# OATML-Markslab/ProteinGym

Measured on AMD Instinct MI355X. Metric: mutants scored/sec (ESM-1v 650M masked-marginal), higher is better.
Workload: dtype f16x3 (fp32 operands split into 2 fp16 planes, 3 fp16 MFMAs per product, fp32 accumulate)

## Files before the change

### include/pgmi.h

```cpp
#ifndef PGMI_H
#define PGMI_H

#include <stddef.h>
#include <stdint.h>

#ifdef __cplusplus
extern "C" {
#endif

#define PGMI_ABI_VERSION 6

#define PGMI_OK 0
#define PGMI_EINVAL (-1)
#define PGMI_ENOMEM (-2)
#define PGMI_EHIP (-3)
#define PGMI_ENODEV (-4)
#define PGMI_EPARSE (-5)
#define PGMI_EOVERFLOW (-6)

#define PGMI_ARCH_ESM1B 1
#define PGMI_ARCH_ESM2 2
#define PGMI_ARCH_TRANCEPTION 3
#define PGMI_ARCH_MSA 4
#define PGMI_ARCH_PROGEN2 5
// ... 43 lines not shown
typedef struct pgmi_pppl pgmi_pppl;

int pgmi_abi_version(void);
int pgmi_device_count(void);
const char* pgmi_last_error(void);

int64_t pgmi_weight_count(const pgmi_config* cfg);

int pgmi_model_create(const pgmi_config* cfg, const float* weights, int64_t n_weights,
                      int device, pgmi_model** out);
void pgmi_model_destroy(pgmi_model* m);
int pgmi_model_device(const pgmi_model* m);

int pgmi_token_logprobs(pgmi_model* m, const int32_t* tokens, int B, int T, float* out);

int pgmi_masked_logprobs(pgmi_model* m, const int32_t* tokens, const int32_t* mask_pos,
                         int B, int T, float* out);

int pgmi_assay_create(pgmi_model* m, const int32_t* wt_tokens, int n_tok,
                      const int32_t* positions, int P, int window,
                      const int32_t* sub_pos, const int32_t* sub_wt, const int32_t* sub_mt,
                      const int64_t* mut_off, int64_t n_mut, pgmi_assay** out);
int pgmi_assay_run(pgmi_model* m, pgmi_assay* a, double* scores_host, float* table_host,
                   double* scores_dev);
void pgmi_assay_destroy(pgmi_assay* a);

int pgmi_pppl_create(pgmi_model* m, const uint8_t* tokens, const int64_t* seq_off, int64_t n_seq, pgmi_pppl** out);
int pgmi_pppl_run(pgmi_model* m, pgmi_pppl* lib, int64_t first, int64_t count, double* scores_host,
                  float* terms_host, double* scores_dev);
int64_t pgmi_pppl_rows(const pgmi_pppl* lib, int64_t first, int64_t count);
int pgmi_pppl_stats(const pgmi_pppl* lib, int64_t* rows, int64_t* batches, int64_t* tokens, int64_t* padded_tokens);
void pgmi_pppl_destroy(pgmi_pppl* lib);

int pgmi_parse_mutants(const char* text, const int64_t* str_off, int64_t n_mut,
                       const char* sequence, int seq_len, int offset_idx,
                       int32_t* sub_pos, int32_t* sub_wt, int32_t* sub_mt,
                       int64_t* mut_off, int64_t* n_sub);

int pgmi_score_mutants(const float* table, int n_rows, int vocab, const int32_t* sub_pos, const int32_t* sub_wt,
                       const int32_t* sub_mt, const int64_t* mut_off, int64_t n_mut, double* scores);

void pgmi_optimal_window(int position, int seq_len_with_special, int model_window,
                         int* start, int* end);

#define PGMI_K_EMBED 0
#define PGMI_K_LAYERNORM 1
#define PGMI_K_GEMM_QKV 2
#define PGMI_K_ATTENTION 3
#define PGMI_K_GEMM_OUT 4
#define PGMI_K_GEMM_FC1 5
#define PGMI_K_GEMM_FC2 6
#define PGMI_K_HEAD 7
#define PGMI_K_SCORE 8
#define PGMI_K_KEPT_ROWS 9
#define PGMI_K_MOE_ROUTE 10
#define PGMI_K_GEOM 11
#define PGMI_K_CROSS_ATTENTION 12
#define PGMI_K_COUNT 13
int pgmi_profile_enable(pgmi_model* m, int on);
int pgmi_profile_get(pgmi_model* m, int kernel_class, double* ms, int64_t* launches,
                     double* flops, double* bytes);
int pgmi_profile_reset(pgmi_model* m);
int pgmi_synchronize(pgmi_model* m);

int pgmi_set_option(const char* name, int64_t value);

int pgmi_op_layernorm(int device, const float* x, const float* w, const float* b,
                      int rows, int D, float eps, float* y);
int pgmi_op_gemm(int device, int precision, const float* A, const float* W, const float* bias,
                 const float* residual, int M, int N, int K, int epilogue ,
                 float* C);
int pgmi_op_qkln_prep(int device, const float* qkv, const float* q_w, const float* k_w, int B, int T, int H, int iters, float* qk,
                      float* v, double* ms);
int pgmi_op_attention(int device, int precision, const float* qkv, const int32_t* kv_len,
                      int B, int T, int H, int rotary, float* ctx);
int pgmi_op_causal_attention(int device, int lanes, const float* X, const float* W, const float* bias, int K, const float* qkv,
                             const float* conv, const float* rot_cos, const float* rot_sin, const float* slopes, int B, int T,
                             int heads, float* ctx);
int pgmi_op_prefix_attention(int device, const float* qkv, const int32_t* seg_off, int n_seg, const float* prefix_kv, int P, int heads,
                             int split, float* ctx);
int pgmi_op_cross_attention(int device, const float* q, const int32_t* seg_off, int n_seg, const float* mem_kv, int S, int heads,
                            int split, float* ctx);
int pgmi_op_packed_chunks(const int32_t* lens, int B, int drop_last, int same_length, int max_rows, int32_t* out_b1, int32_t* out_n);
int pgmi_op_rmsnorm(int device, const float* x, const float* w, int rows, int D, float eps, float* y);
int pgmi_op_geom_attention(int device, const float* proj, const float* rot, const float* trans, const int32_t* frame_mask,
                           int per_row_frames, const float* w_rot, const float* w_dist, int B, int S, int H, float* out);
int pgmi_op_geom_key_tile(int S);
int pgmi_op_moe(int device, const float* h, const float* gate, const float* w1, const float* w3, const float* w2, int M, int D, int F,
                int E, int top_k, int gated, float* out, int32_t* ids, float* weights);
int pgmi_op_tied_row_attention(int device, const float* qkv, int R, int C, int H, int splits, float* ctx, float* probs);
int pgmi_op_tied_row_splits(int R, int C, int H);
int pgmi_op_column_attention(int device, const float* X, const float* W, const float* bias, int K, int R, int C, int H, float* ctx);
int pgmi_op_vocab_logsoftmax(int device, const float* h, const float* E, const float* bias, int rows, int D, int V, float* out,
                             int32_t* nonfinite);
int pgmi_op_wide_logsoftmax(int device, const float* logits, int ldl, int rows, int V, const int32_t* tgt, float* out, int32_t* nonfinite);
int pgmi_op_group_logsoftmax(int device, const float* h, const float* E, const float* bias, int rows, int D, int V, int first, int groups,
                             int width, float* full, float* group, int32_t* nonfinite);
int pgmi_op_seq_loglik(int device, const float* lp, const int32_t* tokens, int B, int T, int V, const int32_t* lens, const int32_t* seq_off,
                       const int32_t* seq_p, const int32_t* seq_root, int n_lp_rows, const float* prior, int n_prior_rows,
                       const int32_t* a0, const int32_t* row0, const int32_t* n, const int32_t* flip, float alpha, const float* eve,
                       float beta, int eve_fallback, float* out);

int pgmi_tr_token_logprobs(pgmi_model* m, const int32_t* tokens, int B, int T, float* out);
int pgmi_tr_sequence_loglik(pgmi_model* m, const int32_t* tokens, const int32_t* lens, int B, int T,
                            const float* log_prior, int P, const int32_t* prior_a0, const int32_t* prior_row0,
                            const int32_t* prior_n, const int32_t* prior_flip, float alpha, float* out);
int pgmi_tr_sequence_loglik_shared(pgmi_model* m, const int32_t* tokens, const int32_t* ref, int B, int T,
                                   const float* log_prior, int P, const int32_t* prior_a0, const int32_t* prior_row0,
                                   const int32_t* prior_n, const int32_t* prior_flip, float alpha, float* out,
                                   float* token_logprobs, int64_t* rows_forwarded);
int pgmi_tr_sequence_loglik_eve(pgmi_model* m, const int32_t* tokens, const int32_t* lens, int B, int T,
                                const float* log_prior, int P, const int32_t* prior_a0, const int32_t* prior_row0,
                                const int32_t* prior_n, const int32_t* prior_flip, float alpha, const float* eve_log_prior, float beta,
                                int eve_fallback, float* out);
int pgmi_tr_sequence_loglik_shared_eve(pgmi_model* m, const int32_t* tokens, const int32_t* ref, int B, int T,
                                       const float* log_prior, int P, const int32_t* prior_a0, const int32_t* prior_row0,
                                       const int32_t* prior_n, const int32_t* prior_flip, float alpha, const float* eve_log_prior,
                                       float beta, int eve_fallback, float* out, float* token_logprobs, int64_t* rows_forwarded);

int pgmi_bench_gemm(int device, int precision, int M, int N, int K, int epilogue, int split_out,
                    int variant, int iters, double* ms_per_launch);
int pgmi_bench_gemm_ab(int device, int precision, int M, int N, int K, int epilogue, int split_out,
                       const int* variants, int n_variants, int rounds, int iters, double* ms_out);

int pgmi_pg2_model_create(const pgmi_config* cfg, int rotary_dim, const float* weights, int64_t n_weights, int device, pgmi_model** out);
int pgmi_pg2_token_logprobs(pgmi_model* m, const int32_t* tokens, int B, int T, float* out);
int pgmi_pg2_sequence_loglik(pgmi_model* m, const int32_t* tokens, int B, int L, float* out, int32_t* n_kept);

int64_t pgmi_gpt_weight_count(const pgmi_config* cfg, int pos_kind);
int pgmi_gpt_model_create(const pgmi_config* cfg, int pos_kind, const float* weights, int64_t n_weights, int device, pgmi_model** out);
int pgmi_gpt_token_logprobs(pgmi_model* m, const int32_t* tokens, int B, int T, float* out);
int pgmi_gpt_sequence_loglik(pgmi_model* m, const int32_t* tokens, const int32_t* lens, int B, int T, double* sum, int32_t* n_targets);

typedef struct pgmi_pg3_params {
    int32_t kv_heads;
    int32_t n_experts;
    int32_t top_k;
    int32_t gated;
    float rope_theta;
    float clip_qkv;
} pgmi_pg3_params;
int64_t pgmi_pg3_weight_count(const pgmi_config* cfg, const pgmi_pg3_params* params);
int pgmi_pg3_model_create(const pgmi_config* cfg, const pgmi_pg3_params* params, const float* weights, int64_t n_weights, int device,
                          pgmi_model** out);
int pgmi_pg3_token_logprobs(pgmi_model* m, const int32_t* tokens, int B, int T, float* out);
int pgmi_pg3_sequence_loglik(pgmi_model* m, const int32_t* tokens, const int32_t* lens, int B, int T, double* sum, int32_t* n_targets);
int pgmi_pg3_routing(pgmi_model* m, int layer, int rows, int32_t* ids, float* weights);


int64_t pgmi_esm3_weight_count(const pgmi_config* cfg, int v_heads);
int pgmi_esm3_model_create(const pgmi_config* cfg, int v_heads, const float* weights, int64_t n_weights, int device, pgmi_model** out);
int pgmi_esm3_set_structure(pgmi_model* m, const int32_t* structure_tokens, const int32_t* plddt, const float* rot, const float* trans,
                            const int32_t* frame_mask, int T);

int pgmi_saprot_model_create(const pgmi_config* cfg, int mask_id, const float* weights, int64_t n_weights, int device, pgmi_model** out);
int pgmi_saprot_token_logprobs(pgmi_model* m, const int32_t* tokens, int B, int T, float* out);
int pgmi_saprot_group_logprobs(pgmi_model* m, const int32_t* wt_tokens, int T, const int32_t* set_off, const int32_t* set_pos,
                               int n_sets, float* out);

#define PGMI_POET_TOK_GAP 20
#define PGMI_POET_TOK_START 21
#define PGMI_POET_TOK_STOP 22
#define PGMI_POET_TOK_MASK 23
int64_t pgmi_poet_weight_count(const pgmi_config* cfg, int final_norm);
int pgmi_poet_model_create(const pgmi_config* cfg, int final_norm, const float* weights, int64_t n_weights, int device, pgmi_model** out);
int pgmi_poet_set_prompt(pgmi_model* m, const int32_t* tokens, const int32_t* seg_len, int n_seg);
// ... 128 lines not shown
```

### proteingym_amd/_lib.py

```python
from __future__ import annotations

import ctypes as C
import os

import numpy as np

HERE = os.path.dirname(os.path.abspath(__file__))
LIB_PATH = os.path.join(HERE, "libpgmi.so")

ABI_VERSION = 6
ARCH_ESM1B, ARCH_ESM2, ARCH_TRANCEPTION = 1, 2, 3
ARCH_PROGEN2 = 5
ARCH_GPT = 6
ARCH_ESMC = 7
ARCH_SAPROT = 8
ARCH_POET = 9
ARCH_PROGEN3 = 10
ARCH_ESM3 = 11
ARCH_ESMIF1 = 12
GPT_POS_ROTARY, GPT_POS_LEARNED = 0, 1
PREC_FP32, PREC_BF16, PREC_F16X3 = 0, 1, 2
PRECISIONS = {"fp32": PREC_FP32, "bf16": PREC_BF16, "f16x3": PREC_F16X3}
K_NAMES = ["embed", "layernorm", "gemm_qkv", "attention", "gemm_out", "gemm_fc1", "gemm_fc2",
           "head", "score", "kept_rows", "moe_route", "geom", "cross_attention"]


EINVAL, ENOMEM, EHIP, ENODEV, EPARSE, EOVERFLOW = -1, -2, -3, -4, -5, -6


class PgmiError(RuntimeError):

    def __init__(self, message, code=None):
        super().__init__(message)
        self.code = code


class Config(C.Structure):
    _fields_ = [(n, C.c_int32) for n in (
        "abi_version", "arch", "layers", "embed_dim", "heads", "ffn_dim", "vocab",
        "max_positions", "token_dropout", "emb_layer_norm_before", "precision", "max_rows")] + [("ln_eps", C.c_float)]


class Pg3Params(C.Structure):
    _fields_ = [(n, C.c_int32) for n in ("kv_heads", "n_experts", "top_k", "gated")] + [("rope_theta", C.c_float), ("clip_qkv", C.c_float)]


_lib = None

_i32p = C.POINTER(C.c_int32)
_i64p = C.POINTER(C.c_int64)
_f32p = C.POINTER(C.c_float)
_f64p = C.POINTER(C.c_double)
_u8p = C.POINTER(C.c_uint8)

SIGNATURES = [
    ("pgmi_abi_version", C.c_int, []),
    ("pgmi_device_count", C.c_int, []),
    ("pgmi_last_error", C.c_char_p, []),
    ("pgmi_weight_count", C.c_int64, [C.POINTER(Config)]),
    ("pgmi_model_create", C.c_int, [C.POINTER(Config), _f32p, C.c_int64, C.c_int, C.POINTER(C.c_void_p)]),
    ("pgmi_model_destroy", None, [C.c_void_p]),
    ("pgmi_model_device", C.c_int, [C.c_void_p]),
    ("pgmi_token_logprobs", C.c_int, [C.c_void_p, _i32p, C.c_int, C.c_int, _f32p]),
    ("pgmi_masked_logprobs", C.c_int, [C.c_void_p, _i32p, _i32p, C.c_int, C.c_int, _f32p]),
    ("pgmi_assay_create", C.c_int, [C.c_void_p, _i32p, C.c_int, _i32p, C.c_int, C.c_int,
                                    _i32p, _i32p, _i32p, _i64p, C.c_int64, C.POINTER(C.c_void_p)]),
    ("pgmi_assay_run", C.c_int, [C.c_void_p, C.c_void_p, _f64p, _f32p, C.c_void_p]),
    ("pgmi_assay_destroy", None, [C.c_void_p]),
    ("pgmi_pppl_create", C.c_int, [C.c_void_p, C.POINTER(C.c_uint8), _i64p, C.c_int64, C.POINTER(C.c_void_p)]),
    ("pgmi_pppl_run", C.c_int, [C.c_void_p, C.c_void_p, C.c_int64, C.c_int64, _f64p, _f32p, C.c_void_p]),
    ("pgmi_pppl_rows", C.c_int64, [C.c_void_p, C.c_int64, C.c_int64]),
    ("pgmi_pppl_stats", C.c_int, [C.c_void_p, _i64p, _i64p, _i64p, _i64p]),
    ("pgmi_pppl_destroy", None, [C.c_void_p]),
    ("pgmi_parse_mutants", C.c_int, [C.c_char_p, _i64p, C.c_int64, C.c_char_p, C.c_int, C.c_int,
                                     _i32p, _i32p, _i32p, _i64p, _i64p]),
    ("pgmi_score_mutants", C.c_int, [_f32p, C.c_int, C.c_int, _i32p, _i32p, _i32p, _i64p, C.c_int64, _f64p]),
    ("pgmi_optimal_window", None, [C.c_int, C.c_int, C.c_int, _i32p, _i32p]),
    ("pgmi_profile_enable", C.c_int, [C.c_void_p, C.c_int]),
    ("pgmi_profile_get", C.c_int, [C.c_void_p, C.c_int, _f64p, _i64p, _f64p, _f64p]),
    ("pgmi_profile_reset", C.c_int, [C.c_void_p]),
    ("pgmi_synchronize", C.c_int, [C.c_void_p]),
    ("pgmi_set_option", C.c_int, [C.c_char_p, C.c_int64]),
    ("pgmi_op_layernorm", C.c_int, [C.c_int, _f32p, _f32p, _f32p, C.c_int, C.c_int, C.c_float, _f32p]),
    ("pgmi_op_gemm", C.c_int, [C.c_int, C.c_int, _f32p, _f32p, _f32p, _f32p, C.c_int, C.c_int, C.c_int, C.c_int, _f32p]),
    ("pgmi_tr_token_logprobs", C.c_int, [C.c_void_p, _i32p, C.c_int, C.c_int, _f32p]),
    ("pgmi_tr_sequence_loglik", C.c_int, [C.c_void_p, _i32p, _i32p, C.c_int, C.c_int, _f32p, C.c_int,
                                          _i32p, _i32p, _i32p, _i32p, C.c_float, _f32p]),
    ("pgmi_tr_sequence_loglik_shared", C.c_int, [C.c_void_p, _i32p, _i32p, C.c_int, C.c_int, _f32p, C.c_int,
                                                 _i32p, _i32p, _i32p, _i32p, C.c_float, _f32p, _f32p, _i64p]),
    ("pgmi_tr_sequence_loglik_eve", C.c_int, [C.c_void_p, _i32p, _i32p, C.c_int, C.c_int, _f32p, C.c_int,
                                              _i32p, _i32p, _i32p, _i32p, C.c_float, _f32p, C.c_float, C.c_int, _f32p]),
    ("pgmi_tr_sequence_loglik_shared_eve", C.c_int, [C.c_void_p, _i32p, _i32p, C.c_int, C.c_int, _f32p, C.c_int,
                                                     _i32p, _i32p, _i32p, _i32p, C.c_float, _f32p, C.c_float, C.c_int, _f32p, _f32p,
                                                     _i64p]),
    ("pgmi_pg2_model_create", C.c_int, [C.POINTER(Config), C.c_int, _f32p, C.c_int64, C.c_int, C.POINTER(C.c_void_p)]),
    ("pgmi_pg2_token_logprobs", C.c_int, [C.c_void_p, _i32p, C.c_int, C.c_int, _f32p]),
    ("pgmi_pg2_sequence_loglik", C.c_int, [C.c_void_p, _i32p, C.c_int, C.c_int, _f32p, _i32p]),
    ("pgmi_gpt_weight_count", C.c_int64, [C.POINTER(Config), C.c_int]),
    ("pgmi_gpt_model_create", C.c_int, [C.POINTER(Config), C.c_int, _f32p, C.c_int64, C.c_int, C.POINTER(C.c_void_p)]),
    ("pgmi_gpt_token_logprobs", C.c_int, [C.c_void_p, _i32p, C.c_int, C.c_int, _f32p]),
    ("pgmi_gpt_sequence_loglik", C.c_int, [C.c_void_p, _i32p, _i32p, C.c_int, C.c_int, _f64p, _i32p]),
    ("pgmi_saprot_model_create", C.c_int, [C.POINTER(Config), C.c_int, _f32p, C.c_int64, C.c_int, C.POINTER(C.c_void_p)]),
    ("pgmi_saprot_token_logprobs", C.c_int, [C.c_void_p, _i32p, C.c_int, C.c_int, _f32p]),
    ("pgmi_saprot_group_logprobs", C.c_int, [C.c_void_p, _i32p, C.c_int, _i32p, _i32p, C.c_int, _f32p]),
    ("pgmi_poet_weight_count", C.c_int64, [C.POINTER(Config), C.c_int]),
    ("pgmi_poet_model_create", C.c_int, [C.POINTER(Config), C.c_int, _f32p, C.c_int64, C.c_int, C.POINTER(C.c_void_p)]),
    ("pgmi_poet_set_prompt", C.c_int, [C.c_void_p, _i32p, _i32p, C.c_int]),
    ("pgmi_poet_prompt_logprobs", C.c_int, [C.c_void_p, _f32p]),
    ("pgmi_poet_token_logprobs", C.c_int, [C.c_void_p, _i32p, _i32p, C.c_int, C.c_int, _f32p]),
    ("pgmi_poet_sequence_loglik", C.c_int, [C.c_void_p, _i32p, _i32p, C.c_int, C.c_int, _f64p]),
    ("pgmi_esmif1_weight_count", C.c_int64, [C.POINTER(Config), C.c_int]),
    ("pgmi_esmif1_model_create", C.c_int, [C.POINTER(Config), C.c_int, _f32p, C.c_int64, C.c_int, C.POINTER(C.c_void_p)]),
    ("pgmi_esmif1_set_memory", C.c_int, [C.c_void_p, _f32p, C.c_int]),
    ("pgmi_esmif1_token_logprobs", C.c_int, [C.c_void_p, _i32p, _i32p, C.c_int, C.c_int, _f32p]),
    ("pgmi_esmif1_sequence_loglik", C.c_int, [C.c_void_p, _i32p, _i32p, C.c_int, C.c_int, _f64p]),
    ("pgmi_pg3_weight_count", C.c_int64, [C.POINTER(Config), C.POINTER(Pg3Params)]),
    ("pgmi_pg3_model_create", C.c_int, [C.POINTER(Config), C.POINTER(Pg3Params), _f32p, C.c_int64, C.c_int, C.POINTER(C.c_void_p)]),
    ("pgmi_pg3_token_logprobs", C.c_int, [C.c_void_p, _i32p, C.c_int, C.c_int, _f32p]),
    ("pgmi_pg3_sequence_loglik", C.c_int, [C.c_void_p, _i32p, _i32p, C.c_int, C.c_int, _f64p, _i32p]),
    ("pgmi_pg3_routing", C.c_int, [C.c_void_p, C.c_int, C.c_int, _i32p, _f32p]),
    ("pgmi_esm3_weight_count", C.c_int64, [C.POINTER(Config), C.c_int]),
    ("pgmi_esm3_model_create", C.c_int, [C.POINTER(Config), C.c_int, _f32p, C.c_int64, C.c_int, C.POINTER(C.c_void_p)]),
    ("pgmi_esm3_set_structure", C.c_int, [C.c_void_p, _i32p, _i32p, _f32p, _f32p, _i32p, C.c_int]),
    ("pgmi_eve_weight_count", C.c_int64, [C.c_void_p]),
    ("pgmi_eve_create", C.c_int, [C.c_void_p, _f32p, C.c_int64, C.c_int, C.POINTER(C.c_void_p)]),
    ("pgmi_eve_destroy", None, [C.c_void_p]),
    ("pgmi_eve_profile_model", C.c_void_p, [C.c_void_p]),
    ("pgmi_eve_encode", C.c_int, [C.c_void_p, _u8p, C.c_int, _f32p, _f32p]),
    ("pgmi_eve_elbo", C.c_int, [C.c_void_p, _u8p, C.c_int, C.c_int64, C.c_uint64, C.c_int, C.c_void_p, _f32p, _f32p, _f32p]),
    ("pgmi_eve_noise_fill", C.c_int, [C.c_void_p, C.c_uint64, C.c_int, C.c_int64, C.c_int, C.c_void_p]),
    ("pgmi_eve_evol_indices", C.c_int, [C.c_void_p, _u8p, C.c_int, C.c_int, C.c_uint64, _f64p, _f64p]),
    ("pgmi_eve_log_prior", C.c_int, [C.c_void_p, _u8p, C.c_int, C.c_uint64, C.c_void_p, _f64p, _f64p]),
    ("pgmi_mpnn_weight_count", C.c_int64, [C.c_void_p]),
    ("pgmi_mpnn_create", C.c_int, [C.c_void_p, _f32p, C.c_int64, C.c_int, C.POINTER(C.c_void_p)]),
    ("pgmi_mpnn_destroy", None, [C.c_void_p]),
    ("pgmi_mpnn_profile_model", C.c_void_p, [C.c_void_p]),
    ("pgmi_mpnn_set_structure", C.c_int, [C.c_void_p, _f32p, _f32p, _i32p, _i32p, C.c_int]),
    ("pgmi_mpnn_graph", C.c_int, [C.c_void_p, _i32p, _f32p]),
    ("pgmi_mpnn_encoder", C.c_int, [C.c_void_p, _f32p, _f32p]),
    ("pgmi_mpnn_log_probs", C.c_int, [C.c_void_p, _u8p, _i32p, C.c_int, _f32p]),
    ("pgmi_mpnn_scores", C.c_int, [C.c_void_p, _u8p, _i32p, C.c_int, _f64p]),
    ("pgmi_s2f_weight_count", C.c_int64, [C.c_void_p]),
    ("pgmi_s2f_create", C.c_int, [C.c_void_p, _f32p, C.c_int64, C.c_void_p, C.c_int, C.POINTER(C.c_void_p)]),
    ("pgmi_s2f_destroy", None, [C.c_void_p]),
    ("pgmi_s2f_profile_model", C.c_void_p, [C.c_void_p]),
    ("pgmi_s2f_set_structure", C.c_int, [C.c_void_p, _f32p, _f32p, C.c_int]),
    ("pgmi_s2f_graph", C.c_int, [C.c_void_p, _i32p, _i32p, _i32p, _f32p, _f32p]),
    ("pgmi_s2f_gvp_forward", C.c_int, [C.c_void_p, _f32p, _f32p, C.c_int, _f32p, _f32p, _f32p]),
    ("pgmi_s2f_set_logprobs", C.c_int, [C.c_void_p, _i32p, C.c_int, _i32p, _i32p, _i32p, C.c_int, _f32p, _f32p]),
    ("pgmi_unirep_weight_count", C.c_int64, [C.c_void_p]),
    ("pgmi_unirep_model_create", C.c_int, [C.c_void_p, _f32p, C.c_int64, C.c_int, C.POINTER(C.c_void_p)]),
    ("pgmi_unirep_destroy", None, [C.c_void_p]),
    ("pgmi_unirep_profile_model", C.c_void_p, [C.c_void_p]),
    ("pgmi_unirep_set_target", C.c_int, [C.c_void_p, _i32p, C.c_int]),
    ("pgmi_unirep_sequence_nll", C.c_int, [C.c_void_p, _i32p, _i64p, C.c_int64, C.c_int, _f64p, _i64p]),
    ("pgmi_unirep_token_logprobs", C.c_int, [C.c_void_p, _i32p, C.c_int, _f32p]),
    ("pgmi_op_mlstm_step", C.c_int, [C.c_void_p, _f32p, _f32p, _i32p, C.c_int, _f32p, _f32p, _f32p]),
    ("pgmi_bench_gemm", C.c_int, [C.c_int] * 9 + [_f64p]),
    ("pgmi_bench_gemm_ab", C.c_int, [C.c_int] * 7 + [_i32p, C.c_int, C.c_int, C.c_int, _f64p]),
    ("pgmi_op_attention", C.c_int, [C.c_int, C.c_int, _f32p, _i32p, C.c_int, C.c_int, C.c_int, C.c_int, _f32p]),
    ("pgmi_op_qkln_prep", C.c_int, [C.c_int, _f32p, _f32p, _f32p, C.c_int, C.c_int, C.c_int, C.c_int, _f32p, _f32p, _f64p]),
    ("pgmi_op_causal_attention", C.c_int, [C.c_int, C.c_int, _f32p, _f32p, _f32p, C.c_int, _f32p, _f32p, _f32p, _f32p, _f32p,
                                           C.c_int, C.c_int, C.c_int, _f32p]),
    ("pgmi_op_prefix_attention", C.c_int, [C.c_int, _f32p, _i32p, C.c_int, _f32p, C.c_int, C.c_int, C.c_int, _f32p]),
    ("pgmi_op_cross_attention", C.c_int, [C.c_int, _f32p, _i32p, C.c_int, _f32p, C.c_int, C.c_int, C.c_int, _f32p]),
    ("pgmi_op_packed_chunks", C.c_int, [_i32p, C.c_int, C.c_int, C.c_int, C.c_int, _i32p, _i32p]),
    ("pgmi_op_rmsnorm", C.c_int, [C.c_int, _f32p, _f32p, C.c_int, C.c_int, C.c_float, _f32p]),
    ("pgmi_op_geom_attention", C.c_int, [C.c_int, _f32p, _f32p, _f32p, _i32p, C.c_int, _f32p, _f32p, C.c_int, C.c_int, C.c_int, _f32p]),
    ("pgmi_op_geom_key_tile", C.c_int, [C.c_int]),
    ("pgmi_op_moe", C.c_int, [C.c_int, _f32p, _f32p, _f32p, _f32p, _f32p, C.c_int, C.c_int, C.c_int, C.c_int, C.c_int, C.c_int, _f32p,
                              _i32p, _f32p]),
    ("pgmi_op_tied_row_attention", C.c_int, [C.c_int, _f32p, C.c_int, C.c_int, C.c_int, C.c_int, _f32p, _f32p]),
    ("pgmi_op_tied_row_splits", C.c_int, [C.c_int, C.c_int, C.c_int]),
    ("pgmi_op_column_attention", C.c_int, [C.c_int, _f32p, _f32p, _f32p, C.c_int, C.c_int, C.c_int, C.c_int, _f32p]),
    ("pgmi_op_vocab_logsoftmax", C.c_int, [C.c_int, _f32p, _f32p, _f32p, C.c_int, C.c_int, C.c_int, _f32p, _i32p]),
    ("pgmi_op_wide_logsoftmax", C.c_int, [C.c_int, _f32p, C.c_int, C.c_int, C.c_int, _i32p, _f32p, _i32p]),
    ("pgmi_op_group_logsoftmax", C.c_int, [C.c_int, _f32p, _f32p, _f32p, C.c_int, C.c_int, C.c_int, C.c_int, C.c_int, C.c_int, _f32p,
                                           _f32p, _i32p]),
    ("pgmi_op_seq_loglik", C.c_int, [C.c_int, _f32p, _i32p, C.c_int, C.c_int, C.c_int, _i32p, _i32p, _i32p, _i32p, C.c_int, _f32p, C.c_int,
                                     _i32p, _i32p, _i32p, _i32p, C.c_float, _f32p, C.c_float, C.c_int, _f32p]),
    ("pgmi_msa_token_logprobs", C.c_int, [C.c_void_p, _i32p, C.c_int, C.c_int, _f32p]),
    ("pgmi_msa_masked_logprobs", C.c_int, [C.c_void_p, _i32p, C.c_int, C.c_int, C.c_int, _i32p, _i32p, C.c_int, _f32p]),
    ("pgmi_msa_cluster_counts", C.c_int, [C.c_int, C.POINTER(C.c_int8), C.c_int64, C.c_int64, C.c_int, C.c_double, _i32p, _f64p]),
    ("pgmi_msa_neighbor_counts", C.c_int, [C.c_int, C.POINTER(C.c_int8), C.c_int64, C.c_int64, C.c_int, C.c_double, _i32p, _f64p]),
]


def load():
    global _lib
    if _lib is not None:
        return _lib
    if not os.path.exists(LIB_PATH):
        raise PgmiError(f"{LIB_PATH} not found: run `python -m proteingym_amd.build_native` "
                        "(hipcc, gfx950).  There is no CPU fallback.")
    lib = C.CDLL(LIB_PATH)
    for name, res, args in SIGNATURES:
        fn = getattr(lib, name)
        fn.restype = res
        fn.argtypes = args
    if lib.pgmi_abi_version() != ABI_VERSION:
        raise PgmiError("libpgmi ABI version mismatch; rebuild")
    _lib = lib
    return lib


def check(rc: int):
    if rc != 0:
        raise PgmiError(f"libpgmi error {rc}: {load().pgmi_last_error().decode(errors='replace')}", code=int(rc))


def ptr(a: np.ndarray, ty):
    return a.ctypes.data_as(ty) if a is not None else None


def as_i32(a):
    return np.ascontiguousarray(a, dtype=np.int32)


def as_f32(a):
    return np.ascontiguousarray(a, dtype=np.float32)


class ModelHandle:
    CREATE = "pgmi_model_create"

    def __init__(self, cfg: dict, weights: np.ndarray, device: int = 0, max_rows: int = 0, arch_arg=None,
                 precision: int = PREC_F16X3, **fields):
        lib = load()
        self.cfg = dict(cfg)
        self.device = device
        c = Config(abi_version=ABI_VERSION, layers=cfg["layers"], embed_dim=cfg["embed_dim"], heads=cfg["heads"],
                   ffn_dim=cfg["ffn_dim"], precision=precision, max_rows=max_rows, **fields)
        w = as_f32(weights)
        n = self._weight_count(lib, c, arch_arg)
        if w.size != n:
            raise PgmiError(f"weight blob has {w.size} elements, config needs {n}")
        h = C.c_void_p()
        head = (C.byref(c),) if arch_arg is None else (C.byref(c), arch_arg)
        check(getattr(lib, self.CREATE)(*head, ptr(w, _f32p), w.size, device, C.byref(h)))
        self._h = h

    @staticmethod
    def _weight_count(lib, c, arch_arg):
        return lib.pgmi_weight_count(C.byref(c))

    def close(self):
        if getattr(self, "_h", None):
            load().pgmi_model_destroy(self._h)
            self._h = None
# ... 7 lines not shown
```

### proteingym_amd/csrc/api_esm.hip

```cpp
#include "model.h"

namespace pgmi {

int create_esm(pgmi_model* m, const pgmi_config* cfg, const float* w, int64_t n_weights) {
    const size_t D = cfg->embed_dim, F = cfg->ffn_dim, V = cfg->vocab, dh = m->dh, Da = m->Da;
    BlobCursor c(m, w, n_weights);
    c.upload(&m->embed_tokens, V * D);
    if (cfg->arch == PGMI_ARCH_ESM1B) c.upload(&m->embed_positions, (size_t)(cfg->max_positions + 2) * D);
    if (cfg->emb_layer_norm_before) {
        c.upload(&m->lnb_w, D);
        c.upload(&m->lnb_b, D);
    }
    auto slot = [&](size_t col) -> size_t { return rotate_half_slot(col, dh); };
    const float qscale = 1.0f / sqrtf((float)dh);
    m->layers.resize(cfg->layers);
    std::vector<float> wq(3 * Da * D, 0.0f), bq(3 * Da, 0.0f), wo_r(D * Da, 0.0f);
    for (int l = 0; l < cfg->layers; ++l) {
        Layer& L = m->layers[l];
        c.upload(&L.ln1_w, D);
        c.upload(&L.ln1_b, D);
        pack_qkv_slots(c.take(3 * (D * D + D)), D, Da, slot, qscale, wq.data(), bq.data());
        c.linear(&L.wqkv, &L.wqkv16, wq.data(), wq.size(), D);
        c.upload(&L.bqkv, bq.data(), bq.size());
        pack_out_cols(c.take(D * D), D, Da, slot, wo_r.data());
        c.linear(&L.wo, &L.wo16, wo_r.data(), wo_r.size(), Da);
        c.upload(&L.bo, D);
        c.upload(&L.ln2_w, D);
        c.upload(&L.ln2_b, D);
        c.linear(&L.w1, &L.w116, F * D, D);
        c.upload(&L.b1, F);
        c.linear(&L.w2, &L.w216, D * F, F);
        c.upload(&L.b2, D);
    }
    c.upload(&m->lna_w, D);
    c.upload(&m->lna_b, D);
    c.linear(&m->hd_w, &m->hd16, D * D, D);
    c.upload(&m->hd_b, D);
    c.upload(&m->hln_w, D);
    c.upload(&m->hln_b, D);
    c.upload(&m->head_b, V);
    m->head_w = m->embed_tokens;
    return c.finish();
}

int ensure_rotary(pgmi_model* m, int T) {
    if ((!esm2_rotary(m->cfg.arch) && !esmc_blocks(m->cfg.arch)) || T <= m->rot_len) return PGMI_OK;
    return upload_rotate_half(m, std::max(T, 1026));
}

int upload_rotate_half(pgmi_model* m, int n) {
    const int rh = m->rot_halves;
    float inv[64];
    const int half = m->dh / 2;
    for (int i = 0; i < half; ++i) inv[i] = 1.0f / powf(10000.0f, (float)(2 * i) / (float)m->dh);
    return upload_rotary(m, n, rh, [&](int t, int g, int i) {
        const int j = (rh == 1) ? i : 32 * g + i;
        return j < half ? (float)t * inv[j] : 0.0f;
    });
}

int run_encoder(pgmi_model* m, int B, int T, const int32_t* keep, int n_keep, bool* compacted) {
    const pgmi_config& c = m->cfg;
    const int M = B * T, D = c.embed_dim, F = c.ffn_dim, N1 = m->fc1_cols, H = c.heads, Da = m->Da;
    hipStream_t s = m->stream;
    if (c.arch == PGMI_ARCH_ESM1B && T > c.max_positions) {
        set_error("Sequence length %d above maximum sequence length of %d", T, c.max_positions);
        return PGMI_EINVAL;
    }
    int rc = ensure_rotary(m, T);
    if (!rc) rc = reset_pad_keys(m, B, T);
    if (rc) return rc;
    {
        ProfScope p(m, PGMI_K_EMBED, 0, (double)M * D * 4);
        launch_seq_stats(m->tokens, B, T, m->embed_gather ? 0 : c.token_dropout, m->denom, m->pos_idx, m->kv_len, s, m->mask_id);
        if (c.arch == PGMI_ARCH_ESM3) { if ((rc = esm3_embed(m, B, T))) return rc; }
        else if (m->embed_gather) launch_gather_rows(m->embed_tokens, m->tokens, M, D, m->x, s);
        else launch_embed(m->tokens, m->denom, m->pos_idx, m->embed_tokens, m->embed_positions, c.token_dropout, M, T, D, m->x, s, m->mask_id);
        if (m->lnb_w) {
            launch_layernorm(m->x, m->lnb_w, m->lnb_b, M, D, 1e-5f, m->x, s);
            launch_zero_pad_rows(m->tokens, M, D, m->x, s);
        }
    }
    const double ln_bytes = 2.0 * M * D * 4;
    const int prec = c.precision;
    const int mode16 = (prec == PGMI_PREC_F16X3) ? 1 : 2;
    for (int l = 0; l < c.layers; ++l) {
        const Layer& L = m->layers[l];
        { ProfScope p(m, PGMI_K_LAYERNORM, 0, ln_bytes);
          if (prec == PGMI_PREC_FP32) launch_layernorm(m->x, L.ln1_w, L.ln1_b, M, D, 1e-5f, m->h, s);
          else launch_layernorm16(m->x, L.ln1_w, L.ln1_b, M, D, 1e-5f, m->h16, mode16, s); }
        const bool fused_qkv = prec != PGMI_PREC_FP32 && !L.q_ln;
        { ProfScope p(m, PGMI_K_GEMM_QKV, 2.0 * M * 3 * D * D, 0);
          if (fused_qkv) {
              GemmLaunch g = qkv_launch(m, L.wqkv16, L.bqkv, M, Da, D, T, m->Hs);
              g.bf = prec == PGMI_PREC_BF16;
              g.qkv.cos_t = m->rot_cos; g.qkv.sin_t = m->rot_sin; g.qkv.rotary = esm2_rotary(c.arch); g.qkv.rot_halves = m->rot_halves;
              rc = launch_gemm16(g);
          } else
              rc = linear(m, m->h, m->h16, L.wqkv, L.wqkv16, L.bqkv, nullptr, m->qkv, nullptr, M, 3 * Da, D, EPI_NONE);
          if (rc) return rc; }
        { ProfScope p(m, PGMI_K_ATTENTION, 4.0 * M * T * D, L.q_ln ? (double)M * D * 20 : 0);
          if (L.q_ln && (rc = launch_qkln_prep(m->qkv, L.q_ln, L.k_ln, 1e-5f, m->rot_cos, m->rot_sin, B, T, H, m->qk16, m->qk16_plane,
                                               m->vt16, m->vt16_plane, s)))
              return rc;
          const bool v2 = prec != PGMI_PREC_FP32;
          if (esm2_rotary(c.arch) && !v2) launch_rotary(m->qkv, m->rot_cos, m->rot_sin, M, T, m->Hs, s, m->rot_halves);
          if (v2) {
              AttLaunch a;
              a.qk16 = m->qk16, a.qk_plane = m->qk16_plane, a.vt16 = m->vt16, a.vt_plane = m->vt16_plane;
              a.B = B, a.T = T, a.H = H, a.head_dim = m->rot_halves * kHeadDim;
              a.kv_len = m->kv_len;
              a.out = prec == PGMI_PREC_F16X3 ? ATT_OUT_SPLIT : ATT_OUT_BF16;
              a.ctx16 = m->h16;
              a.stream = s;
              rc = launch_attention_f16x3_v2(a);
          } else {
              rc = launch_attention_f32(m->qkv, m->kv_len, B, T, H, m->h, s, m->rot_halves * kHeadDim);
          }
          if (rc) return rc; }
        if (keep && m->keep_rows && l == c.layers - 1 && !L.g_norm_w) {
            const int R = n_keep;
            ProfScope p(m, PGMI_K_KEPT_ROWS, 2.0 * R * D * (Da + N1 + F), 0);
            launch_gather_rows(m->x, keep, R, D, m->qkv, s);
            if (prec == PGMI_PREC_FP32) launch_gather_rows(m->h, keep, R, Da, m->g, s);
            else
                launch_gather_rows(reinterpret_cast<const float*>(m->h16), keep, R, prec == PGMI_PREC_F16X3 ? Da : Da / 2,
                                   reinterpret_cast<float*>(m->g16), s);
            rc = linear(m, m->g, m->g16, L.wo, L.wo16, L.bo, m->qkv, m->x, nullptr, R, D, Da, EPI_NONE);
            if (rc) return rc;
            if (prec == PGMI_PREC_FP32) launch_layernorm(m->x, L.ln2_w, L.ln2_b, R, D, 1e-5f, m->h, s);
            else launch_layernorm16(m->x, L.ln2_w, L.ln2_b, R, D, 1e-5f, m->h16, mode16, s);
            rc = linear(m, m->h, m->h16, L.w1, L.w116, L.b1, nullptr,
                        prec == PGMI_PREC_FP32 ? m->g : nullptr, prec == PGMI_PREC_FP32 ? nullptr : m->g16,
                        R, N1, D, m->fc1_epi);
            if (rc) return rc;
            rc = linear(m, m->g, m->g16, L.w2, L.w216, L.b2, m->x, m->x, nullptr, R, D, F, EPI_NONE);
            if (rc) return rc;
            if (compacted) *compacted = true;
            break;
        }
        { ProfScope p(m, PGMI_K_GEMM_OUT, 2.0 * M * D * D, 0);
          rc = linear(m, m->h, m->h16, L.wo, L.wo16, L.bo, m->x, m->x, nullptr, M, D, Da, EPI_NONE);
          if (rc) return rc; }
        if (L.g_norm_w && m->e3_framed && (rc = geom_branch(m, L, B, T))) return rc;
        { ProfScope p(m, PGMI_K_LAYERNORM, 0, ln_bytes);
          if (prec == PGMI_PREC_FP32) launch_layernorm(m->x, L.ln2_w, L.ln2_b, M, D, 1e-5f, m->h, s);
          else launch_layernorm16(m->x, L.ln2_w, L.ln2_b, M, D, 1e-5f, m->h16, mode16, s); }
        { ProfScope p(m, PGMI_K_GEMM_FC1, 2.0 * M * N1 * D, 0);
          rc = linear(m, m->h, m->h16, L.w1, L.w116, L.b1, nullptr,
                      prec == PGMI_PREC_FP32 ? m->g : nullptr, prec == PGMI_PREC_FP32 ? nullptr : m->g16,
                      M, N1, D, m->fc1_epi);
          if (rc) return rc; }
        { ProfScope p(m, PGMI_K_GEMM_FC2, 2.0 * M * F * D, 0);
          rc = linear(m, m->g, m->g16, L.w2, L.w216, L.b2, m->x, m->x, nullptr, M, D, F, EPI_NONE);
          if (rc) return rc; }
    }
    PGMI_HIP(hipGetLastError());
    return PGMI_OK;
}

int run_head(pgmi_model* m, int R, const int32_t* row_idx) {
    const pgmi_config& c = m->cfg;
    ProfScope p(m, PGMI_K_HEAD, 2.0 * R * c.embed_dim * (c.embed_dim + c.vocab), 0);
    int rc = head_hidden(m, R, row_idx);
    if (rc) return rc;
    launch_vocab_logsoftmax(m->g, m->head_w, m->head_b, R, c.embed_dim, c.vocab, m->lp, m->nonfinite, m->stream);
    PGMI_HIP(hipGetLastError());
    return PGMI_OK;
}

int head_hidden(pgmi_model* m, int R, const int32_t* row_idx) {
    const pgmi_config& c = m->cfg;
    const int D = c.embed_dim;
    hipStream_t s = m->stream;
    const int prec = c.precision;
    const float* src = m->x;
    if (row_idx) {
        launch_gather_rows(m->x, row_idx, R, D, m->h, s);
        src = m->h;
    }
    if (prec == PGMI_PREC_FP32) launch_layernorm(src, m->lna_w, m->lna_b, R, D, 1e-5f, m->h, s);
    else launch_layernorm16(src, m->lna_w, m->lna_b, R, D, 1e-5f, m->h16, prec == PGMI_PREC_F16X3 ? 1 : 2, s);
    int rc = linear(m, m->h, m->h16, m->hd_w, m->hd16, m->hd_b, nullptr, m->g, nullptr, R, D, D, EPI_GELU);
    if (rc) return rc;
    launch_layernorm(m->g, m->hln_w, m->hln_b, R, D, 1e-5f, m->g, s);
    return PGMI_OK;
}


int run_rows(pgmi_model* m, int B, int T, int R, const int32_t* row_idx) {
    bool compacted = false;
    int rc = run_encoder(m, B, T, row_idx, R, &compacted);
    if (rc) return rc;
    return run_head(m, R, compacted ? nullptr : row_idx);
}

}

extern "C" {

int pgmi_token_logprobs(pgmi_model* m, const int32_t* tokens, int B, int T, float* out) {
    if (!m || !tokens || !out || B <= 0 || T <= 0) { set_error("bad argument"); return PGMI_EINVAL; }
    if (m->cfg.arch == PGMI_ARCH_SAPROT) { set_error("SaProt models are scored with pgmi_saprot_token_logprobs / pgmi_saprot_group_logprobs"); return PGMI_EINVAL; }
    if (T + 31 > m->max_rows) { set_error("T=%d exceeds workspace rows %d", T, m->max_rows); return PGMI_EINVAL; }
    int rc = check_tokens(tokens, B, T);
    if (rc) return rc;
    PGMI_HIP(hipSetDevice(m->device));
    const int V = m->cfg.vocab;
    rc = for_each_chunk(m, B, T, [&](int b0, int bc) {
        PGMI_HIP(hipMemcpyAsync(m->tokens, tokens + (size_t)b0 * T, (size_t)bc * T * 4, hipMemcpyHostToDevice, m->stream));
        int rc = run_rows(m, bc, T, bc * T, nullptr);
        if (rc) return rc;
        PGMI_HIP(hipMemcpyAsync(out + (size_t)b0 * T * V, m->lp, (size_t)bc * T * V * 4, hipMemcpyDeviceToHost, m->stream));
        return PGMI_OK;
    });
    return rc ? rc : check_nonfinite(m);
}

int pgmi_masked_logprobs(pgmi_model* m, const int32_t* tokens, const int32_t* mask_pos, int B, int T, float* out) {
    if (!m || !tokens || !mask_pos || !out || B <= 0 || T <= 0) { set_error("bad argument"); return PGMI_EINVAL; }
    if (m->cfg.arch == PGMI_ARCH_SAPROT) { set_error("SaProt models are scored with pgmi_saprot_token_logprobs / pgmi_saprot_group_logprobs"); return PGMI_EINVAL; }
    if (esmc_blocks(m->cfg.arch) && T + 31 > m->max_rows) { set_error("T=%d exceeds workspace rows %d", T, m->max_rows); return PGMI_EINVAL; }
    if (T > m->max_rows) { set_error("T=%d exceeds workspace rows %d", T, m->max_rows); return PGMI_EINVAL; }
    int rc = check_tokens(tokens, B, T);
    if (rc) return rc;
    for (int b = 0; b < B; ++b)
        if (mask_pos[b] < 0 || mask_pos[b] >= T) { set_error("mask_pos[%d]=%d out of range", b, mask_pos[b]); return PGMI_EINVAL; }
    PGMI_HIP(hipSetDevice(m->device));
    const int V = m->cfg.vocab;
    std::vector<int32_t> ridx;
    rc = for_each_chunk(m, B, T, [&](int b0, int bc) {
        ridx.resize(bc);
        for (int b = 0; b < bc; ++b) ridx[b] = b * T + mask_pos[b0 + b];
        PGMI_HIP(hipMemcpyAsync(m->tokens, tokens + (size_t)b0 * T, (size_t)bc * T * 4, hipMemcpyHostToDevice, m->stream));
        PGMI_HIP(hipMemcpyAsync(m->aux_i, mask_pos + b0, (size_t)bc * 4, hipMemcpyHostToDevice, m->stream));
        PGMI_HIP(hipMemcpyAsync(m->row_idx, ridx.data(), (size_t)bc * 4, hipMemcpyHostToDevice, m->stream));
        launch_apply_mask(m->tokens, m->aux_i, bc, T, m->stream);
        int rc = run_rows(m, bc, T, bc, m->row_idx);
        if (rc) return rc;
        PGMI_HIP(hipMemcpyAsync(out + (size_t)b0 * V, m->lp, (size_t)bc * V * 4, hipMemcpyDeviceToHost, m->stream));
        return PGMI_OK;
    });
    return rc ? rc : check_nonfinite(m);
}

int pgmi_assay_create(pgmi_model* m, const int32_t* wt_tokens, int n_tok, const int32_t* positions, int P,
                      int window, const int32_t* sub_pos, const int32_t* sub_wt, const int32_t* sub_mt,
                      const int64_t* mut_off, int64_t n_mut, pgmi_assay** out) {
    if (!out) { set_error("null out"); return PGMI_EINVAL; }
    *out = nullptr;
    if (!m || !wt_tokens || n_tok <= 0 || P < 0 || (P > 0 && !positions) || window <= 0 || n_mut < 0) { set_error("bad argument"); return PGMI_EINVAL; }
    if (esmc_blocks(m->cfg.arch)) { set_error("ESM C / ESM3 assays run through pgmi_masked_logprobs (their window rule is not pgmi_optimal_window)"); return PGMI_EINVAL; }
    if (m->cfg.arch == PGMI_ARCH_SAPROT) { set_error("SaProt assays run through pgmi_saprot_group_logprobs (position sets, no window)"); return PGMI_EINVAL; }
    for (int i = 0; i < n_tok; ++i)
        if (wt_tokens[i] < 0 || wt_tokens[i] >= PGMI_VOCAB || wt_tokens[i] == PGMI_TOK_PAD) { set_error("wt token %d invalid at %d", wt_tokens[i], i); return PGMI_EINVAL; }
    const int T = std::min(n_tok, window);
    if (T > m->max_rows) { set_error("T=%d exceeds workspace rows %d", T, m->max_rows); return PGMI_EINVAL; }
    std::vector<int32_t> ws(P), mr(P);
    for (int i = 0; i < P; ++i) {
        if (positions[i] < 0 || positions[i] >= n_tok) { set_error("position %d out of range", positions[i]); return PGMI_EINVAL; }
        int s, e;
        pgmi_optimal_window(positions[i], n_tok, window, &s, &e);
        if (e - s != T) { set_error("internal: window length %d != %d", e - s, T); return PGMI_EINVAL; }
        ws[i] = s;
        mr[i] = positions[i] - s;
    }
    const int64_t n_sub = n_mut ? mut_off[n_mut] : 0;
    for (int64_t k = 0; k < n_sub; ++k)
        if (sub_pos[k] < 0 || sub_pos[k] >= n_tok || sub_wt[k] < 0 || sub_wt[k] >= PGMI_VOCAB || sub_mt[k] < 0 || sub_mt[k] >= PGMI_VOCAB) {
            set_error("substitution %lld out of range", (long long)k);
            return PGMI_EINVAL;
        }
    PGMI_HIP(hipSetDevice(m->device));
    pgmi_assay* a = new pgmi_assay();
    a->m = m; a->n_tok = n_tok; a->P = P; a->T = T; a->n_mut = n_mut; a->n_sub = n_sub;
    int rc = dev_upload(a->allocs, &a->wt, wt_tokens, (size_t)n_tok);
    if (!rc) rc = dev_upload(a->allocs, &a->positions, positions, (size_t)P);
    if (!rc) rc = dev_upload(a->allocs, &a->win_start, ws.data(), (size_t)P);
    if (!rc) rc = dev_upload(a->allocs, &a->mask_rel, mr.data(), (size_t)P);
    if (!rc) rc = dev_upload(a->allocs, &a->sub_pos, sub_pos, (size_t)n_sub);
    if (!rc) rc = dev_upload(a->allocs, &a->sub_wt, sub_wt, (size_t)n_sub);
    if (!rc) rc = dev_upload(a->allocs, &a->sub_mt, sub_mt, (size_t)n_sub);
    if (!rc) rc = dev_upload(a->allocs, &a->mut_off, mut_off, (size_t)(n_mut + 1));
    if (!rc) rc = dev_alloc(a->allocs, &a->table, (size_t)n_tok * PGMI_VOCAB);
    if (!rc) rc = dev_alloc(a->allocs, &a->scores, (size_t)n_mut);
    if (rc) { pgmi_assay_destroy(a); return rc; }
    m->assays.push_back(a);
    *out = a;
    return PGMI_OK;
}

void pgmi_assay_destroy(pgmi_assay* a) {
    if (!a) return;
    if (a->m) {
        hipSetDevice(a->m->device);
        hipStreamSynchronize(a->m->stream);
        auto& v = a->m->assays;
        v.erase(std::remove(v.begin(), v.end(), a), v.end());
    }
    for (void* p : a->allocs) hipFree(p);
    delete a;
}

int pgmi_assay_run(pgmi_model* m, pgmi_assay* a, double* scores_host, float* table_host, double* scores_dev) {
    if (!m || !a || a->m != m) { set_error("bad model/assay handle (assay belongs to another or a destroyed model)"); return PGMI_EINVAL; }
    PGMI_HIP(hipSetDevice(m->device));
    hipStream_t s = m->stream;
    const int T = a->T, V = m->cfg.vocab;
    const int per = rows_per_chunk(m, T);
    launch_fill_f32(a->table, (int64_t)a->n_tok * V, NAN, s);
    for (int p0 = 0; p0 < a->P; p0 += per) {
        const int bc = std::min(per, a->P - p0);
        launch_make_masked_windows(a->wt, a->win_start + p0, a->mask_rel + p0, bc, T, m->tokens, s);
        launch_row_index(a->mask_rel + p0, bc, T, m->row_idx, s);
        int rc = run_rows(m, bc, T, bc, m->row_idx);
        if (rc) return rc;
        launch_scatter_rows(m->lp, a->positions + p0, bc, V, a->table, s);
    }
    {
        ProfScope p(m, PGMI_K_SCORE, 0, (double)a->n_sub * 20);
        launch_score_mutants(a->table, V, a->sub_pos, a->sub_wt, a->sub_mt, a->mut_off, a->n_mut, a->scores, s);
    }
    PGMI_HIP(hipGetLastError());
    if (scores_dev && a->n_mut) PGMI_HIP(hipMemcpyAsync(scores_dev, a->scores, (size_t)a->n_mut * 8, hipMemcpyDeviceToDevice, s));
    if (scores_host && a->n_mut) PGMI_HIP(hipMemcpyAsync(scores_host, a->scores, (size_t)a->n_mut * 8, hipMemcpyDeviceToHost, s));
    if (table_host) PGMI_HIP(hipMemcpyAsync(table_host, a->table, (size_t)a->n_tok * V * 4, hipMemcpyDeviceToHost, s));
    PGMI_HIP(hipStreamSynchronize(s));
    return check_nonfinite(m);
}

int pgmi_pppl_create(pgmi_model* m, const uint8_t* tokens, const int64_t* seq_off, int64_t n_seq, pgmi_pppl** out) {
    if (!out) { set_error("null out"); return PGMI_EINVAL; }
    *out = nullptr;
    if (!m || !tokens || !seq_off || n_seq <= 0 || n_seq > 0x7fffffff) { set_error("bad argument"); return PGMI_EINVAL; }
    if (m->cfg.arch != PGMI_ARCH_ESM1B && m->cfg.arch != PGMI_ARCH_ESM2) { set_error("pseudo-ppl needs an ESM-1b/1v/ESM2 model"); return PGMI_EINVAL; }
    if (seq_off[0] != 0) { set_error("seq_off[0] must be 0"); return PGMI_EINVAL; }
    for (int64_t n = 0; n < n_seq; ++n) {
        const int64_t len = seq_off[n + 1] - seq_off[n];
        if (len < 2 || len > (1 << 24)) { set_error("sequence %lld has %lld tokens", (long long)n, (long long)len); return PGMI_EINVAL; }
        const uint8_t* t = tokens + seq_off[n];
        for (int64_t i = 0; i < len; ++i)
            if (t[i] >= PGMI_VOCAB || t[i] == PGMI_TOK_PAD) { set_error("token id %d invalid at sequence %lld, position %lld", (int)t[i], (long long)n, (long long)i); return PGMI_EINVAL; }
    }
    PGMI_HIP(hipSetDevice(m->device));
    pgmi_pppl* q = new pgmi_pppl();
    q->m = m;
    q->N = n_seq;
    q->off.assign(seq_off, seq_off + n_seq + 1);
    int rc = dev_upload(q->allocs, &q->tok8, tokens, (size_t)seq_off[n_seq]);
    if (!rc) rc = dev_upload(q->allocs, &q->off_dev, seq_off, (size_t)n_seq + 1);
    if (rc) { for (void* p : q->allocs) hipFree(p); delete q; return rc; }
    m->pppls.push_back(q);
    *out = q;
    return PGMI_OK;
}

void pgmi_pppl_destroy(pgmi_pppl* q) {
    if (!q) return;
    if (q->m) {
        hipSetDevice(q->m->device);
        hipStreamSynchronize(q->m->stream);
        auto& v = q->m->pppls;
        v.erase(std::remove(v.begin(), v.end(), q), v.end());
    }
    for (void* p : q->allocs) hipFree(p);
    delete q;
}

int64_t pgmi_pppl_rows(const pgmi_pppl* q, int64_t first, int64_t count) {
    if (!q || first < 0 || count < 0 || first + count > q->N) return -1;
    int64_t r = 0;
    for (int64_t n = first; n < first + count; ++n) r += std::max<int64_t>(0, q->off[n + 1] - q->off[n] - 4);
    return r;
}

int pgmi_pppl_run(pgmi_model* m, pgmi_pppl* q, int64_t first, int64_t count, double* scores_host, float* terms_host,
                  double* scores_dev) {
    if (!m || !q || q->m != m) { set_error("bad model/library handle (library belongs to another or a destroyed model)"); return PGMI_EINVAL; }
    if (first < 0 || count <= 0 || first + count > q->N) { set_error("sequence range [%lld, %lld) outside the library of %lld", (long long)first, (long long)(first + count), (long long)q->N); return PGMI_EINVAL; }
    PGMI_HIP(hipSetDevice(m->device));
    hipStream_t s = m->stream;
    const int J = (int)count, V = m->cfg.vocab;
    std::vector<int32_t> sid(J);
    for (int j = 0; j < J; ++j) sid[j] = (int32_t)(first + j);
    auto len_of = [&](int32_t n) { return q->off[n + 1] - q->off[n]; };
    std::stable_sort(sid.begin(), sid.end(), [&](int32_t a, int32_t b) { return len_of(a) > len_of(b); });
    std::vector<int64_t> rp((size_t)J + 1);
    rp[0] = 0;
    for (int j = 0; j < J; ++j) rp[j + 1] = rp[j] + std::max<int64_t>(0, len_of(sid[j]) - 4);
    const int64_t R = rp[J];
    const int64_t Tmax = len_of(sid[0]);
    if (R > 0 && Tmax + 31 > m->max_rows) { set_error("T=%lld exceeds workspace rows %d", (long long)Tmax, m->max_rows); return PGMI_EINVAL; }
    if (R > 0 && m->cfg.arch == PGMI_ARCH_ESM1B && Tmax > m->cfg.max_positions) {
        set_error("Sequence length %lld above maximum sequence length of %d", (long long)Tmax, m->cfg.max_positions);
        return PGMI_EINVAL;
    }
    std::vector<void*> pool;
    auto cleanup = [&]() { for (void* p : pool) hipFree(p); };
// ... 60 lines not shown
```

### proteingym_amd/csrc/api_model.hip

```cpp
#include "model.h"

namespace pgmi {

static thread_local char g_err[1024] = "";
void set_error(const char* fmt, ...) {
    va_list ap;
    va_start(ap, fmt);
    vsnprintf(g_err, sizeof(g_err), fmt, ap);
    va_end(ap);
}

int prof_drain(pgmi_model* m) {
    if (m->events_used == 0) return PGMI_OK;
    PGMI_HIP(hipStreamSynchronize(m->stream));
    for (size_t i = 0; i < m->events_used; ++i) {
        float ms = 0.f;
        PGMI_HIP(hipEventElapsedTime(&ms, m->events[i].start, m->events[i].stop));
        m->prof_ms[m->events[i].cls] += ms;
    }
    m->events_used = 0;
    return PGMI_OK;
}

int check_cfg(const pgmi_config* c) {
// ... 295 lines not shown
        const size_t planes = c.precision == PGMI_PREC_F16X3 ? 2 : 1;
        m->h16_plane = R * Dw;
        m->g16_plane = R * F;
        alloc(&m->h16, m->h16_plane * planes);
        alloc(&m->g16, m->g16_plane * planes);
    }
    alloc(&m->nonfinite, (size_t)1);
    if (!f32mode) {
        m->qk16_plane = R * 2 * Da;
        m->vt16_plane = R * Da;
        alloc(&m->qk16, m->qk16_plane * 2);
        alloc(&m->vt16, m->vt16_plane * 2);
    }
    if (c.arch == PGMI_ARCH_MSA) {
        alloc(&m->xt, R * D);
        alloc(&m->msa_kv_len, (size_t)2048);
    }
    alloc(&m->lp, ((c.arch == PGMI_ARCH_GPT || c.arch == PGMI_ARCH_PROGEN3) && V > kWave ? (size_t)m->gpt_head_rows : R) * V);
    alloc(&m->denom, R);
    alloc(&m->tokens, R);
    alloc(&m->pos_idx, R);
    alloc(&m->kv_len, R);
    alloc(&m->row_idx, R);
    alloc(&m->aux_i, R);
    if (rc) return rc;
    PGMI_HIP(hipMemset(m->nonfinite, 0, 4));
    if (m->vt16) PGMI_HIP(hipMemset(m->vt16, 0, m->vt16_plane * 2 * sizeof(unsigned short)));
    return PGMI_OK;
}

int model_create(const pgmi_config* cfg, const float* w, int64_t n_weights, int device, pgmi_model** out, int arch_arg,
                 const pgmi_pg3_params* pg3) {
    if (!out) { set_error("null out"); return PGMI_EINVAL; }
    *out = nullptr;
    int rc = check_cfg(cfg);
    if (rc) return rc;
    if (cfg->arch == PGMI_ARCH_PROGEN3 && (rc = pg3_check(cfg, pg3))) return rc;
    if (cfg->arch == PGMI_ARCH_ESM3 && (rc = esm3_check(cfg, arch_arg))) return rc;
    if (cfg->arch == PGMI_ARCH_ESMIF1 && (rc = if1_check(cfg, arch_arg))) return rc;
    const int64_t need = cfg->arch == PGMI_ARCH_GPT ? gpt_weight_count(cfg, arch_arg)
                         : cfg->arch == PGMI_ARCH_PROGEN3 ? pg3_weight_count(cfg, pg3)
                         : cfg->arch == PGMI_ARCH_POET ? poet_weight_count(cfg, arch_arg)
                         : cfg->arch == PGMI_ARCH_ESM3 ? esm3_weight_count(cfg, arch_arg)
                         : cfg->arch == PGMI_ARCH_ESMIF1 ? if1_weight_count(cfg, arch_arg) : pgmi_weight_count(cfg);
    if (need < 0) { set_error("causal decoder pos_kind %d: must be PGMI_GPT_POS_ROTARY or PGMI_GPT_POS_LEARNED", arch_arg); return PGMI_EINVAL; }
    if (!w || n_weights != need) {
        set_error("weight blob has %lld elements, config needs %lld", (long long)n_weights, (long long)need);
        return PGMI_EINVAL;
    }
    const int ndev = pgmi_device_count();
    if (ndev <= 0) { set_error("no HIP device visible (libpgmi has no CPU fallback)"); return PGMI_ENODEV; }
    if (device < 0 || device >= ndev) { set_error("device %d out of range (%d visible)", device, ndev); return PGMI_EINVAL; }
    PGMI_HIP(hipSetDevice(device));
    pgmi_model* m = new pgmi_model();
    m->cfg = *cfg;
    m->device = device;
    if (hipStreamCreateWithFlags(&m->stream, hipStreamNonBlocking) != hipSuccess) { set_error("hipStreamCreate failed"); delete m; return PGMI_EHIP; }
    m->dh = cfg->embed_dim / cfg->heads;
    m->rot_halves = m->dh > 2 * kHeadDim ? 4 : m->dh > kHeadDim ? 2 : 1;
    m->Hs = cfg->heads * m->rot_halves;
    m->Da = m->Hs * kHeadDim;
    m->ln_eps = cfg->ln_eps > 0.f ? cfg->ln_eps : 1e-5f;
    m->max_rows = std::max(cfg->max_rows > 0 ? cfg->max_rows : 98304, 2048);
    const size_t V = cfg->vocab;
    const std::vector<float> zeros(std::max({3 * (size_t)m->Da, (V + 63) / 64 * 64, (size_t)cfg->embed_dim, V, (size_t)cfg->heads}), 0.0f);
    rc = dev_upload(m->allocs, &m->zeros, zeros.data(), zeros.size());
    m->fc1_cols = cfg->ffn_dim;
    if (!rc) switch (cfg->arch) {
        case PGMI_ARCH_TRANCEPTION: rc = create_tranception(m, cfg, w, n_weights); break;
        case PGMI_ARCH_MSA: rc = create_msa(m, cfg, w, n_weights); break;
        case PGMI_ARCH_PROGEN2: rc = create_progen2(m, cfg, w, n_weights, arch_arg); break;
        case PGMI_ARCH_GPT: rc = create_gpt(m, cfg, w, n_weights, arch_arg); break;
        case PGMI_ARCH_ESMC: rc = create_esmc(m, cfg, w, n_weights); break;
        case PGMI_ARCH_SAPROT: rc = create_saprot(m, cfg, w, n_weights, arch_arg); break;
        case PGMI_ARCH_POET: rc = create_poet(m, cfg, w, n_weights, arch_arg); break;
        case PGMI_ARCH_PROGEN3: rc = create_progen3(m, cfg, w, n_weights, pg3); break;
        case PGMI_ARCH_ESM3: rc = create_esm3(m, cfg, w, n_weights, arch_arg); break;
        case PGMI_ARCH_ESMIF1: rc = create_esmif1(m, cfg, w, n_weights, arch_arg); break;
        default: rc = create_esm(m, cfg, w, n_weights);
    }
    if (!rc) rc = alloc_workspace(m);
    if (rc) { pgmi_model_destroy(m); return rc; }
    m->keep_rows = env_int("PGMI_KEEP_ROWS", 1);
    gemm_options_from_env();
    m->gemm_variant = env_int("PGMI_GEMM_VARIANT", 0);
    *out = m;
    return PGMI_OK;
}

}

extern "C" {

void pgmi_model_destroy(pgmi_model* m) {
    if (!m) return;
    hipSetDevice(m->device);
    if (m->stream) hipStreamSynchronize(m->stream);
    for (pgmi_assay* a : m->assays) {
        for (void* p : a->allocs) hipFree(p);
        a->allocs.clear();
        a->m = nullptr;
    }
    m->assays.clear();
    for (pgmi_pppl* q : m->pppls) {
        for (void* p : q->allocs) hipFree(p);
        q->allocs.clear();
        q->m = nullptr;
    }
    m->pppls.clear();
    for (auto& e : m->events) { hipEventDestroy(e.start); hipEventDestroy(e.stop); }
    if (m->moe.counts_host) hipHostFree(m->moe.counts_host);
    for (void* p : m->allocs) hipFree(p);
    if (m->stream) hipStreamDestroy(m->stream);
    delete m;
}

int pgmi_model_device(const pgmi_model* m) { return m ? m->device : -1; }

int pgmi_set_option(const char* name, int64_t value) {
    if (!name) { set_error("null option name"); return PGMI_EINVAL; }
    int rc = gemm_set_option(name, (long long)value);
    if (rc) rc = att_set_option(name, (long long)value);
    if (rc) rc = eve_set_option(name, (long long)value);
    if (rc) rc = mpnn_set_option(name, (long long)value);
    if (rc) rc = unirep_set_option(name, (long long)value);
    if (rc) rc = s2f_set_option(name, (long long)value);
    if (rc) set_error("unknown option '%s' (gemm_half_tail, gemm_max_rows, att_xcd_local, att_v3, eve_max_rows, eve_fixed_sample, eve_prior_batch, mpnn_max_rows, unirep_max_rows, s2f_max_rows)", name);
    return rc;
}

int pgmi_synchronize(pgmi_model* m) {
    if (!m) { set_error("null model"); return PGMI_EINVAL; }
    PGMI_HIP(hipStreamSynchronize(m->stream));
    return PGMI_OK;
}

int pgmi_profile_enable(pgmi_model* m, int on) {
    if (!m) { set_error("null model"); return PGMI_EINVAL; }
    int rc = prof_drain(m);
    m->prof = on != 0;
    return rc;
}

int pgmi_profile_reset(pgmi_model* m) {
    if (!m) { set_error("null model"); return PGMI_EINVAL; }
    int rc = prof_drain(m);
    for (int i = 0; i < PGMI_K_COUNT; ++i) { m->prof_ms[i] = 0; m->prof_n[i] = 0; m->prof_flops[i] = 0; m->prof_bytes[i] = 0; }
    return rc;
}

int pgmi_profile_get(pgmi_model* m, int k, double* ms, int64_t* launches, double* flops, double* bytes) {
    if (!m || k < 0 || k >= PGMI_K_COUNT) { set_error("bad argument"); return PGMI_EINVAL; }
    int rc = prof_drain(m);
    if (rc) return rc;
    if (ms) *ms = m->prof_ms[k];
    if (launches) *launches = m->prof_n[k];
    if (flops) *flops = m->prof_flops[k];
    if (bytes) *bytes = m->prof_bytes[k];
    return PGMI_OK;
}

}
```

### proteingym_amd/csrc/api_ops.hip

```cpp
#include "model.h"

static inline float rebuild_split(unsigned short h, unsigned short l) {
    _Float16 a, b;
    memcpy(&a, &h, 2); memcpy(&b, &l, 2);
    return (float)a + (float)b * (1.0f / kLoScale);
}

extern "C" {

int pgmi_op_layernorm(int device, const float* x, const float* w, const float* b, int rows, int D, float eps, float* y) {
    if (!x || !w || !b || !y || rows <= 0 || D <= 0 || D % 4) { set_error("bad argument"); return PGMI_EINVAL; }
    if (pgmi_device_count() <= 0) { set_error("no HIP device visible"); return PGMI_ENODEV; }
    PGMI_HIP(hipSetDevice(device));
    std::vector<void*> pool;
    float *dx, *dw, *db, *dy;
    int rc = 0;
    if ((rc = dev_upload(pool, &dx, x, (size_t)rows * D)) || (rc = dev_upload(pool, &dw, w, (size_t)D)) ||
        (rc = dev_upload(pool, &db, b, (size_t)D)) || (rc = dev_alloc(pool, &dy, (size_t)rows * D))) {
        for (void* p : pool) hipFree(p);
        return rc;
    }
    launch_layernorm(dx, dw, db, rows, D, eps, dy, nullptr);
    hipError_t e = hipMemcpy(y, dy, (size_t)rows * D * 4, hipMemcpyDeviceToHost);
    for (void* p : pool) hipFree(p);
// ... 497 lines not shown
                const size_t o = ki_off(m, (int)n, (int)Da);
                ctx[m * Da + n] = rebuild_split(h[o], h[o + 32]);
            }
    return PGMI_OK;
}

int pgmi_op_cross_attention(int device, const float* q, const int32_t* seg_off, int n_seg, const float* mem_kv, int S, int heads,
                            int split, float* ctx) {
    if (!q || !seg_off || !ctx || !mem_kv || n_seg <= 0 || heads <= 0 || S <= 0 || seg_off[0] != 0) { set_error("bad argument"); return PGMI_EINVAL; }
    std::vector<int32_t> ent_seg, ent_tile, pseg{0, S}, pent_seg, pent_tile;
    for (int b = 0; b < n_seg; ++b) {
        const int len = seg_off[b + 1] - seg_off[b];
        if (len <= 0) { set_error("segment %d is empty", b); return PGMI_EINVAL; }
        for (int j = 0; j * 32 < len; ++j) { ent_seg.push_back(b); ent_tile.push_back(j); }
    }
    for (int j = 0; j * 32 < S; ++j) { pent_seg.push_back(0); pent_tile.push_back(j); }
    if (pgmi_device_count() <= 0) { set_error("no HIP device visible"); return PGMI_ENODEV; }
    PGMI_HIP(hipSetDevice(device));
    const size_t R = (size_t)seg_off[n_seg], Da = (size_t)heads * kHeadDim, ppitch = pent_seg.size() * 32;
    std::vector<float> pq((size_t)S * 3 * Da, 0.0f);
    for (size_t t = 0; t < (size_t)S; ++t) memcpy(&pq[t * 3 * Da + Da], mem_kv + t * 2 * Da, 2 * Da * sizeof(float));
    std::vector<void*> pool;
    auto cleanup = [&]() { for (void* p : pool) hipFree(p); };
    float *dq = nullptr, *dpq = nullptr, *dctx = nullptr;
    int32_t *d_off = nullptr, *d_es = nullptr, *d_et = nullptr, *dp_off = nullptr, *dp_es = nullptr, *dp_et = nullptr;
    unsigned short *q16 = nullptr, *pq16 = nullptr, *pk16 = nullptr, *pvt16 = nullptr, *c16 = nullptr;
    int rc = 0;
    if ((rc = dev_upload(pool, &dq, q, R * Da)) || (rc = dev_upload(pool, &d_off, seg_off, (size_t)n_seg + 1)) ||
        (rc = dev_upload(pool, &d_es, ent_seg.data(), ent_seg.size())) || (rc = dev_upload(pool, &d_et, ent_tile.data(), ent_tile.size())) ||
        (rc = dev_alloc(pool, &q16, 2 * R * Da)) || (rc = dev_alloc(pool, &c16, 2 * R * Da)) || (rc = dev_alloc(pool, &dctx, R * Da)) ||
        (rc = dev_upload(pool, &dpq, pq.data(), pq.size())) || (rc = dev_upload(pool, &dp_off, pseg.data(), pseg.size())) ||
        (rc = dev_upload(pool, &dp_es, pent_seg.data(), pent_seg.size())) || (rc = dev_upload(pool, &dp_et, pent_tile.data(), pent_tile.size())) ||
        (rc = dev_alloc(pool, &pq16, 2 * (size_t)S * Da)) || (rc = dev_alloc(pool, &pk16, 2 * Da * ppitch)) ||
        (rc = dev_alloc(pool, &pvt16, 2 * Da * ppitch))) {
        cleanup();
        return rc;
    }
    hipError_t e = hipMemset(q16, 0xFF, 2 * R * Da * 2);
    if (e == hipSuccess) e = hipMemset(c16, 0xFF, 2 * R * Da * 2);
    if (e == hipSuccess) e = hipMemset(dctx, 0xFF, R * Da * 4);
    if (e == hipSuccess) e = hipMemset(pk16, 0xFF, 2 * Da * ppitch * 2);
    if (e == hipSuccess) e = hipMemset(pvt16, 0xFF, 2 * Da * ppitch * 2);
    if (e != hipSuccess) { cleanup(); set_error("cross attention op failed: %s", hipGetErrorString(e)); return PGMI_EHIP; }
    PrefixAttLaunch p;
    p.qkv = dpq; p.seg_off = dp_off; p.ent_seg = dp_es; p.ent_tile = dp_et; p.n_seg = 1; p.n_ent = (int)pent_seg.size(); p.H = heads;
    p.q16 = pq16; p.q_plane = (size_t)S * Da; p.k16 = pk16; p.vt16 = pvt16; p.pitch = ppitch;
    rc = launch_prefix_prep(p);
    PrefixAttLaunch a;
    a.seg_off = d_off; a.ent_seg = d_es; a.ent_tile = d_et; a.n_seg = n_seg; a.n_ent = (int)ent_seg.size(); a.H = heads;
    a.q16 = q16; a.q_plane = R * Da;
    a.pk16 = pk16; a.pvt16 = pvt16; a.ppitch = ppitch; a.P = S;
    a.out = split ? ATT_OUT_SPLIT : ATT_OUT_F32; a.ctx = dctx; a.ctx16 = c16;
    if (!rc) rc = launch_cross_q_prep(dq, R, heads, q16, R * Da, nullptr);
    if (!rc) rc = launch_cross_attention(a);
    std::vector<unsigned short> h(rc || !split ? 0 : R * Da * 2);
    e = hipDeviceSynchronize();
    if (!rc && e == hipSuccess) e = split ? hipMemcpy(h.data(), c16, h.size() * 2, hipMemcpyDeviceToHost) : hipMemcpy(ctx, dctx, R * Da * 4, hipMemcpyDeviceToHost);
    cleanup();
    if (rc) return rc;
    if (e != hipSuccess) { set_error("cross attention op failed: %s", hipGetErrorString(e)); return PGMI_EHIP; }
    if (split)
        for (size_t m = 0; m < R; ++m)
            for (size_t n = 0; n < Da; ++n) {
                const size_t o = ki_off(m, (int)n, (int)Da);
                ctx[m * Da + n] = rebuild_split(h[o], h[o + 32]);
            }
    return PGMI_OK;
}

int pgmi_op_packed_chunks(const int32_t* lens, int B, int drop_last, int same_length, int max_rows, int32_t* out_b1, int32_t* out_n) {
    if (!lens || !out_b1 || !out_n || B <= 0 || max_rows <= 0) { set_error("bad argument"); return PGMI_EINVAL; }
    const int lo = drop_last ? 2 : 1;
    for (int b = 0; b < B; ++b)
        if (lens[b] < lo) { set_error("row %d of this call: length %d below %d", b, lens[b], lo); return PGMI_EINVAL; }
    *out_n = 0;
    for (int b0 = 0; b0 < B;) {
        const PackedChunk ch = pack_chunk(lens, b0, B, drop_last != 0, same_length != 0, max_rows, own_pitch(max_rows));
        if (ch.b1 == b0) { set_error("row %d of this call: %d tokens exceed the workspace of %d rows", b0, lens[b0], max_rows); return PGMI_EINVAL; }
        out_b1[(*out_n)++] = b0 = ch.b1;
    }
    return PGMI_OK;
}

int pgmi_op_tied_row_splits(int R, int C, int H) {
    if (R <= 0 || C <= 0 || H <= 0) { set_error("bad argument"); return PGMI_EINVAL; }
    return tied_row_splits(R, C, H);
}

int pgmi_op_tied_row_attention(int device, const float* qkv, int R, int C, int H, int splits, float* ctx, float* probs) {
    if (!qkv || !ctx || R <= 0 || C <= 0 || H <= 0 || splits < 0) { set_error("bad argument"); return PGMI_EINVAL; }
    const int S = splits ? splits : tied_row_splits(R, C, H);
    int rc = tied_row_check(R, C, H, S);
    if (rc) return rc;
    if (pgmi_device_count() <= 0) { set_error("no HIP device visible"); return PGMI_ENODEV; }
    PGMI_HIP(hipSetDevice(device));
    const size_t M = (size_t)R * C, D = (size_t)H * kHeadDim, Kp = (size_t)tied_row_kp(C);
    const size_t n_part = (size_t)H * S * C * Kp, n_p = (size_t)H * C * Kp, n_vt = (size_t)H * R * kHeadDim * Kp;
    std::vector<void*> pool;
    auto cleanup = [&]() { for (void* p : pool) hipFree(p); };
    float *dq = nullptr, *part = nullptr, *pp = nullptr, *vt = nullptr;
    unsigned short *qctx16 = nullptr, *k16 = nullptr;
    if ((rc = dev_upload(pool, &dq, qkv, M * 3 * D)) || (rc = dev_alloc(pool, &qctx16, M * D * 2)) || (rc = dev_alloc(pool, &k16, M * D * 2)) ||
        (rc = dev_alloc(pool, &part, n_part)) || (rc = dev_alloc(pool, &pp, n_p)) || (rc = dev_alloc(pool, &vt, n_vt))) {
        cleanup();
        return rc;
    }
    hipError_t e = hipMemset(part, 0xFF, n_part * 4);
    if (e == hipSuccess) e = hipMemset(pp, 0xFF, n_p * 4);
    if (e == hipSuccess) e = hipMemset(vt, 0xFF, n_vt * 4);
    if (e == hipSuccess) e = hipMemset(qctx16, 0xFF, M * D * 2 * sizeof(unsigned short));
    if (e != hipSuccess) { cleanup(); set_error("tied row attention op failed: %s", hipGetErrorString(e)); return PGMI_EHIP; }
    TiedRowLaunch t;
    t.qkv = dq, t.R = R, t.C = C, t.H = H, t.S = S;
    t.qctx16 = qctx16, t.k16 = k16;
    t.part = part, t.p = pp, t.vt = vt;
    rc = launch_tied_row_attention(t);
    std::vector<unsigned short> h(rc ? 0 : M * D * 2), hp(rc || !probs ? 0 : n_p * 2);
    e = hipDeviceSynchronize();
    if (!rc && e == hipSuccess) e = hipMemcpy(h.data(), qctx16, h.size() * 2, hipMemcpyDeviceToHost);
    if (!rc && probs && e == hipSuccess) e = hipMemcpy(hp.data(), pp, hp.size() * 2, hipMemcpyDeviceToHost);
    cleanup();
    if (rc) return rc;
    if (e != hipSuccess) { set_error("tied row attention op failed: %s", hipGetErrorString(e)); return PGMI_EHIP; }
    for (size_t m = 0; m < M; ++m)
        for (size_t n = 0; n < D; ++n) {
            const size_t o = ki_off(m, (int)n, (int)D);
            ctx[m * D + n] = rebuild_split(h[o], h[o + 32]);
        }
    if (probs)
        for (size_t r = 0; r < (size_t)H * C; ++r)
            for (size_t j = 0; j < Kp; ++j) {
                const size_t o = ki_off(r, (int)j, (int)Kp);
                probs[r * Kp + j] = rebuild_split(hp[o], hp[o + 32]);
            }
    return PGMI_OK;
}

int pgmi_op_column_attention(int device, const float* X, const float* W, const float* bias, int K, int R, int C, int H, float* ctx) {
    if (!X || !W || !bias || !ctx || R <= 0 || C <= 0 || H <= 0) { set_error("bad argument"); return PGMI_EINVAL; }
    if (K <= 0 || K % 32) { set_error("column attention op: K = %d is not a positive multiple of 32", K); return PGMI_EINVAL; }
    if (pgmi_device_count() <= 0) { set_error("no HIP device visible"); return PGMI_ENODEV; }
    PGMI_HIP(hipSetDevice(device));
    gemm_options_from_env();
    const size_t M = (size_t)C * R, D = (size_t)H * kHeadDim, Tp = (size_t)(R + 31) / 32 * 32;
    const size_t qk_plane = M * 2 * D, vt_plane = (size_t)C * Tp * D;
    std::vector<void*> pool;
    auto cleanup = [&]() { for (void* p : pool) hipFree(p); };
    const std::vector<int32_t> kv((size_t)C, R);
    float *dx = nullptr, *db = nullptr;
    int32_t* dl = nullptr;
    unsigned short *a16 = nullptr, *qk16 = nullptr, *vt16 = nullptr, *c16 = nullptr;
    int rc = 0;
    if ((rc = dev_upload(pool, &dx, X, M * K)) || (rc = dev_upload(pool, &db, bias, 3 * D)) || (rc = dev_upload(pool, &dl, kv.data(), kv.size())) ||
        (rc = dev_alloc(pool, &a16, M * K * 2)) || (rc = dev_alloc(pool, &qk16, qk_plane * 2)) || (rc = dev_alloc(pool, &vt16, vt_plane * 2)) ||
        (rc = dev_alloc(pool, &c16, M * D * 2))) {
        cleanup();
        return rc;
    }
    hipError_t e = hipMemset(vt16, 0, vt_plane * 2 * sizeof(unsigned short));
    if (e == hipSuccess) e = hipMemset(c16, 0xFF, M * D * 2 * sizeof(unsigned short));
    if (e != hipSuccess) { cleanup(); set_error("column attention op failed: %s", hipGetErrorString(e)); return PGMI_EHIP; }
    W16 w16;
    rc = make_w16(pool, W, 3 * D * K, (size_t)K, PGMI_PREC_F16X3, nullptr, &w16);
    if (!rc) {
        launch_split16(dx, (int64_t)(M * K), 1.0f, 2, K, a16, nullptr);
        GemmLaunch g = op_gemm(a16, w16, db, (int)M, 3 * (int)D, K, env_int("PGMI_GEMM_VARIANT", 0));
// ... 225 lines not shown
```

### proteingym_amd/csrc/attention_f16.hip

```cpp
#include <stdlib.h>
#include <string.h>
#include <algorithm>

#include "attention_f16_common.h"

namespace pgmi {

template <int WPB, int OUT, int NSTG, int DH = 64, bool RAG = false, int DO = DH>
__global__ __launch_bounds__(WPB * 64) void attention_f16x3_v2_kernel(
    const unsigned short* __restrict__ qk16, size_t qk_plane, const unsigned short* __restrict__ vt16,
    size_t vt_plane, const int32_t* __restrict__ kv_len, const float* __restrict__ slopes, int T, int H,
    int Tp, float* __restrict__ ctx, unsigned short* __restrict__ ctx16, RagMap rag, int dense_nblk, int nseq) {
    constexpr float defer_thr = kAttDefer;
    constexpr int NT = WPB * 64;
    constexpr int KCPR = DH / 8;
    constexpr int KCH = AKT * KCPR, VCH = DO * 4;
    constexpr int NSL = DH / DO;
    static_assert(NSL == 1 || (OUT == ATT_OUT_SPLIT && !RAG), "sliced context: split-plane output of dense launches only");
    constexpr int STG_CH = 2 * KCH + 2 * VCH;
    constexpr int NWI = STG_CH / 64;
    static_assert(NWI % WPB == 0, "the wave-instructions of a stage divide evenly over the waves");
    constexpr int NDMA = NWI / WPB;
    constexpr int NS = DH / 16, ND = DO / 32;
    extern __shared__ __attribute__((aligned(16))) u32x4 lds[];
// ... 255 lines not shown
}
static const Att16v2Inst kAtt16v2[] = {
    att16v2_inst<1, ATT_OUT_F32, 3, 64>(),   att16v2_inst<2, ATT_OUT_F32, 3, 64>(),   att16v2_inst<4, ATT_OUT_F32, 3, 64>(),
    att16v2_inst<1, ATT_OUT_SPLIT, 3, 64>(), att16v2_inst<2, ATT_OUT_SPLIT, 3, 64>(), att16v2_inst<4, ATT_OUT_SPLIT, 3, 64>(),
    att16v2_inst<1, ATT_OUT_BF16, 3, 64>(),  att16v2_inst<2, ATT_OUT_BF16, 3, 64>(),  att16v2_inst<4, ATT_OUT_BF16, 3, 64>(),
    att16v2_inst<1, ATT_OUT_SPLIT, 3, 64, true>(), att16v2_inst<2, ATT_OUT_SPLIT, 3, 64, true>(), att16v2_inst<4, ATT_OUT_SPLIT, 3, 64, true>(),
    att16v2_inst<4, ATT_OUT_F32, 3, 128>(),  att16v2_inst<4, ATT_OUT_SPLIT, 3, 128>(), att16v2_inst<4, ATT_OUT_BF16, 3, 128>(),
    att16v2_inst<4, ATT_OUT_SPLIT, 2, 256, false, 128>(),
};

static int launch_att16v2(const AttLaunch& a, int wpb, dim3 grid, const RagMap* rag, int dense_nblk) {
    for (const Att16v2Inst& k : kAtt16v2) {
        if (k.wpb != wpb || k.out != a.out || k.head_dim != a.head_dim || k.rag != (rag != nullptr)) continue;
        if (k.lds_bytes > 65536) {
            hipError_t e = hipFuncSetAttribute(reinterpret_cast<const void*>(k.fn), hipFuncAttributeMaxDynamicSharedMemorySize, (int)k.lds_bytes);
            if (e != hipSuccess) { set_error("hipFuncSetAttribute: %s", hipGetErrorString(e)); return PGMI_EHIP; }
        }
        hipLaunchKernelGGL(k.fn, grid, dim3(wpb * 64), k.lds_bytes, a.stream, a.qk16, a.qk_plane, a.vt16, a.vt_plane, a.kv_len, a.slopes,
                           a.T, a.H, (a.T + 31) / 32 * 32, a.ctx, a.ctx16, rag ? *rag : RagMap{}, dense_nblk, a.B);
        PGMI_HIP(hipGetLastError());
        return PGMI_OK;
    }
    set_error("attention_f16x3_v2: no kernel for %d waves, output %d, head_dim %d%s", wpb, (int)a.out, a.head_dim, rag ? ", ragged" : "");
    return PGMI_EINVAL;
}

static int g_att_xcd_local = -1;
int att_set_option(const char* name, long long value) {
    if (!strcmp(name, "att_xcd_local")) { g_att_xcd_local = (int)value; return PGMI_OK; }
    if (!strcmp(name, "att_v3")) { att_v3_set_option((int)value); return PGMI_OK; }
    return PGMI_EINVAL;
}
static dim3 dense_grid(int nblk, int H, int B, int* dense_nblk) {
    if (g_att_xcd_local == 0 || (g_att_xcd_local < 0 && nblk < 2)) { *dense_nblk = 0; return dim3(nblk, H, B); }
    *dense_nblk = nblk;
    const long long pairs = (long long)H * B, groups = (pairs + 7) / 8;
    return dim3((unsigned)(groups * 8 * nblk), 1, 1);
}

int att16_waves_per_block(int T) {
    const int n32 = (T + 31) / 32, nblk = (n32 + 3) / 4;
    const int wpb = (n32 + nblk - 1) / nblk;
    return wpb == 3 ? 4 : wpb;
}

static int check_operand_range(const char* who, const AttLaunch& a) {
    const unsigned long long Tp = (unsigned long long)(a.T + 31) / 32 * 32;
    const unsigned long long seq_bytes = (unsigned long long)a.T * 2ull * (unsigned long long)a.H * (unsigned long long)a.head_dim * 2ull;
    const unsigned long long vt_bytes = (unsigned long long)a.head_dim * Tp * 2ull;
    if ((unsigned long long)a.qk_plane * 2ull + seq_bytes >= (1ull << 32) || (unsigned long long)a.vt_plane * 2ull + vt_bytes >= (1ull << 32)) {
        set_error("%s: operand planes of %zu / %zu halfs exceed the 32-bit offset range of the K / V^T DMA "
                  "(plane stride + one sequence must stay below 4 GiB: create the model with a smaller max_rows)", who, a.qk_plane, a.vt_plane);
        return PGMI_EINVAL;
    }
    return PGMI_OK;
}

int launch_attention_f16x3_v2(const AttLaunch& a) {
    const int B = a.B, T = a.T, H = a.H, head_dim = a.head_dim;
    if (B <= 0 || T <= 0 || H <= 0 || a.out < ATT_OUT_F32 || a.out > ATT_OUT_BF16 || (head_dim != 64 && head_dim != 128 && head_dim != 256)) {
        set_error("attention_f16x3_v2: bad arguments B=%d T=%d H=%d out=%d head_dim=%d", B, T, H, (int)a.out, head_dim);
        return PGMI_EINVAL;
    }
    const int n32 = (T + 31) / 32, Tp = n32 * 32;
    int rc = check_operand_range("attention_f16x3_v2", a);
    if (rc) return rc;
    int dn = 0;
    if (head_dim == 256) {
        if (a.qkv || a.conv || !a.slopes || a.out != ATT_OUT_SPLIT) { set_error("attention_f16x3_v2: head_dim 256 is the causal, fused-QKV, split-plane-output flavour only"); return PGMI_EINVAL; }
        const dim3 grid = dense_grid((n32 + 3) / 4, 2 * H, B, &dn);
        return launch_att16v2(a, 4, grid, nullptr, dn);
    }
    if (head_dim == 128) {
        if (a.qkv || a.conv) { set_error("attention_f16x3_v2: head_dim 128 needs operands from the fused QKV projection"); return PGMI_EINVAL; }
        const dim3 grid = dense_grid((n32 + 3) / 4, H, B, &dn);
        return launch_att16v2(a, 4, grid, nullptr, dn);
    }
    if (a.qkv && a.conv && a.rotary) { set_error("attention_f16x3_v2: depth-wise convolution and rotary together are not a model this library knows"); return PGMI_EINVAL; }
    if (a.qkv && a.conv && H % 4) { set_error("attention_f16x3_v2: the depth-wise convolution has four head groups, H = %d is not a multiple of 4", H); return PGMI_EINVAL; }
    if (a.qkv && a.conv)
        launch_qkv_prep_conv(dim3(n32, H, B), a.stream, a.qkv, a.conv, T, H, Tp, a.qk16, a.qk_plane, a.vt16, a.vt_plane, nullptr);
    else if (a.qkv)
        launch_qkv_prep(dim3(n32, H, B), a.stream, a.qkv, a.cos_t, a.sin_t, a.rotary, T, H, Tp, a.qk16, a.qk_plane, a.vt16, a.vt_plane);
    const int wpb = att16_waves_per_block(T);
    const dim3 grid = dense_grid((n32 + wpb - 1) / wpb, H, B, &dn);
    return att_v3_serves(a) ? launch_att16v3(a, wpb, grid, dn) : launch_att16v2(a, wpb, grid, nullptr, dn);
}

int launch_attention_tr_ragged(const AttLaunch& a, const AttRagged& rg) {
    const int T = a.T, H = a.H;
    if (T <= 0 || H <= 0 || !a.qkv || !a.conv || !a.slopes || a.head_dim != 64 || a.out != ATT_OUT_SPLIT || rg.n_tiles <= 0 || rg.n_blocks <= 0) {
        set_error("attention_tr_ragged: bad arguments T=%d H=%d tiles=%d blocks=%d", T, H, rg.n_tiles, rg.n_blocks);
        return PGMI_EINVAL;
    }
    const int rc = check_operand_range("attention_tr_ragged", a);
    if (rc) return rc;
    const RagMap tiles{rg.seq_off, rg.seq_p, rg.seq_q, rg.seq_root, rg.seq_vt, rg.tile_seq, rg.tile_j};
    launch_qkv_prep_conv(dim3(rg.n_tiles, H, 1), a.stream, a.qkv, a.conv, T, H, (T + 31) / 32 * 32, a.qk16, a.qk_plane, a.vt16, a.vt_plane, &tiles);
    const RagMap rag{rg.seq_off, rg.seq_p, rg.seq_q, rg.seq_root, rg.seq_vt, rg.blk_seq, rg.blk_j};
    return launch_att16v2(a, att16_waves_per_block(T), dim3(rg.n_blocks, H, 1), &rag, 0);
}

}
```

### proteingym_amd/csrc/attention_f16_common.h

```cpp
#pragma once
#include "common.h"

namespace pgmi {

typedef _Float16 h2 __attribute__((ext_vector_type(2)));
typedef _Float16 h8 __attribute__((ext_vector_type(8)));
typedef unsigned int u32x4 __attribute__((ext_vector_type(4)));
typedef unsigned int u32x2 __attribute__((ext_vector_type(2)));

constexpr int AKT = 32;
constexpr float kAttDefer = 4.0f;

__device__ __forceinline__ unsigned int pack_h2(_Float16 a, _Float16 b) {
    const h2 t = {a, b};
    return __builtin_bit_cast(unsigned int, t);
}
__device__ __forceinline__ f32x16 mfma_h(u32x4 a, u32x4 b, f32x16 c) {
    return __builtin_amdgcn_mfma_f32_32x32x16_f16(__builtin_bit_cast(h8, a), __builtin_bit_cast(h8, b), c, 0, 0, 0);
}


struct RagMap {
    const int32_t* seq_off;
    const int32_t* seq_p;
// ... 33 lines not shown
                first[k] = sw[0];
                second[k] = sw[1];
            }
            if (row_ok) *reinterpret_cast<u32x4*>(row_head + dt * 32 + 8 * (2 * gp + kh)) = u32x4{first[0], first[1], second[0], second[1]};
        }
}

template <int ND>
__device__ __forceinline__ void store_ctx_split(const f32x16 (&om)[ND], const f32x16 (&oc)[ND], float inv, float inv_lo, bool row_ok,
                                                unsigned short* rowp, int kh) {
#pragma unroll
    for (int dt = 0; dt < ND; ++dt)
#pragma unroll
        for (int gp = 0; gp < 2; ++gp) {
            unsigned int w[2][4];
#pragma unroll
            for (int gi = 0; gi < 2; ++gi) {
                const int g = 2 * gp + gi;
                _Float16 hh[4], ll[4];
#pragma unroll
                for (int e = 0; e < 4; ++e) split_act(fmaf(oc[dt][4 * g + e], inv_lo, om[dt][4 * g + e]) * inv, hh[e], ll[e]);
                w[gi][0] = pack_h2(hh[0], hh[1]); w[gi][1] = pack_h2(hh[2], hh[3]);
                w[gi][2] = pack_h2(ll[0], ll[1]); w[gi][3] = pack_h2(ll[2], ll[3]);
            }
            unsigned int first[4], second[4];
#pragma unroll
            for (int k = 0; k < 4; ++k) {
                const auto sw = __builtin_amdgcn_permlane32_swap(w[0][k], w[1][k], false, false);
                first[k] = sw[0];
                second[k] = sw[1];
            }
            if (row_ok) {
                unsigned short* dst = rowp + dt * 64 + 8 * (2 * gp + kh);
                *reinterpret_cast<u32x4*>(dst) = u32x4{first[0], first[1], second[0], second[1]};
                *reinterpret_cast<u32x4*>(dst + 32) = u32x4{first[2], first[3], second[2], second[3]};
            }
        }
}

template <int ND>
__device__ __forceinline__ void store_ctx_f32(const f32x16 (&om)[ND], const f32x16 (&oc)[ND], float inv, float inv_lo, float* dst) {
#pragma unroll
    for (int dt = 0; dt < ND; ++dt)
#pragma unroll
        for (int g = 0; g < 4; ++g) {
            float val[4];
#pragma unroll
            for (int e = 0; e < 4; ++e) val[e] = fmaf(oc[dt][4 * g + e], inv_lo, om[dt][4 * g + e]) * inv;
            *reinterpret_cast<f32x4*>(dst + dt * 32 + 8 * g) = f32x4{val[0], val[1], val[2], val[3]};
        }
}

__device__ __forceinline__ int xcd_local_pair(int dense_nblk, int& qblk) {
    const int within = (int)blockIdx.x % (8 * dense_nblk);
    qblk = within >> 3;
    return ((int)blockIdx.x / (8 * dense_nblk)) * 8 + (within & 7);
}

__device__ __forceinline__ __amdgpu_buffer_rsrc_t operand_rsrc(const unsigned short* base, unsigned long long bytes) {
    return __builtin_amdgcn_make_buffer_rsrc(const_cast<unsigned short*>(base), 0, (int)(unsigned int)bytes, 0x00020000);
}

template <int DH>
__device__ __forceinline__ int k_swizzle(int row) { return DH == 64 ? ((row >> 1) & 7) : (row & 15); }
__device__ __forceinline__ int v_chunk(int d, int m, int kh) { return d * 4 + ((2 * m + kh) ^ ((d >> 2) & 3)); }

__device__ __forceinline__ u32x2 split_p(float p0, float p1) {
    typedef __fp16 fp16x2 __attribute__((ext_vector_type(2)));
    typedef float f32x2 __attribute__((ext_vector_type(2)));
    const fp16x2 hi2 = __builtin_amdgcn_cvt_pkrtz(p0, p1);
    const f32x2 ps = f32x2{p0, p1} * f32x2{kLoScale, kLoScale};
    const float l0 = fmaf((float)hi2[0], -kLoScale, ps[0]), l1 = fmaf((float)hi2[1], -kLoScale, ps[1]);
    const fp16x2 lo2 = __builtin_amdgcn_cvt_pkrtz(l0, l1);
    return u32x2{__builtin_bit_cast(unsigned int, hi2), __builtin_bit_cast(unsigned int, lo2)};
}

void launch_qkv_prep(dim3 grid, hipStream_t s, const float* qkv, const float* cos_t, const float* sin_t, int rotary, int T, int H, int Tp,
                     unsigned short* qk16, size_t qk_plane, unsigned short* vt16, size_t vt_plane);
void launch_qkv_prep_conv(dim3 grid, hipStream_t s, const float* qkv, const float* conv, int T, int H, int Tp, unsigned short* qk16, size_t qk_plane,
                          unsigned short* vt16, size_t vt_plane, const RagMap* rag);
bool att_v3_serves(const AttLaunch& a);
void att_v3_set_option(int value);
int launch_att16v3(const AttLaunch& a, int wpb, dim3 grid, int dense_nblk);

}
```

### proteingym_amd/csrc/attention_f16_prep.hip

```cpp
#include <stdlib.h>
#include <string.h>
#include <algorithm>

#include "attention_f16_common.h"

namespace pgmi {

__global__ __launch_bounds__(256) void qkv_prep_kernel(
    const float* __restrict__ qkv, const float* __restrict__ cos_t, const float* __restrict__ sin_t,
    int rotary, int T, int H, int Tp, unsigned short* __restrict__ qk16,
    size_t qk_plane, unsigned short* __restrict__ vt16, size_t vt_plane) {
    const int b = blockIdx.z, h = blockIdx.y, t0 = blockIdx.x * 32;
    const int tid = threadIdx.x;
    const int D = H * kHeadDim;
    const size_t RS = (size_t)3 * D;
#pragma unroll
    for (int it = 0; it < 2; ++it) {
        const int u = tid + 256 * it;
        const int which = u >> 8, tok = (u >> 3) & 31, c = u & 7;
        const int t = t0 + tok;
        if (t < T) {
            const float* src = qkv + ((size_t)b * T + t) * RS + (size_t)which * D + h * kHeadDim + 4 * c;
            f32x4 x1 = *reinterpret_cast<const f32x4*>(src);
            f32x4 x2 = *reinterpret_cast<const f32x4*>(src + 32);
// ... 184 lines not shown
        float q = 0.f;
#pragma unroll
        for (int i = 0; i < NV; ++i) {
            const int c = lane + 64 * i;
            if (c < nv) {
#pragma unroll
                for (int k = 0; k < 4; ++k) {
                    const float d = v[i][k] - mean;
                    q += d * d;
                }
            }
        }
#pragma unroll
        for (int o = 32; o > 0; o >>= 1) q += __shfl_xor(q, o);
        const float rstd = 1.0f / sqrtf(q / (float)D + eps);
        const f32x4* wr = reinterpret_cast<const f32x4*>(which ? k_w : q_w);
        const int j4 = 4 * (lane & 15);
        const f32x4 cs = *reinterpret_cast<const f32x4*>(cos_t + (size_t)t * 64 + j4);
        const f32x4 sn = *reinterpret_cast<const f32x4*>(sin_t + (size_t)t * 64 + j4);
        const bool first_half = (lane & 8) == 0;
#pragma unroll
        for (int i = 0; i < NV; ++i) {
            const int c = lane + 64 * i;
            f32x4 o;
            const f32x4 wv = (c < nv) ? wr[c] : f32x4{0.f, 0.f, 0.f, 0.f};
#pragma unroll
            for (int k = 0; k < 4; ++k) o[k] = (v[i][k] - mean) * rstd * wv[k];
            f32x4 p;
#pragma unroll
            for (int k = 0; k < 4; ++k) p[k] = __shfl_xor(o[k], 8);
            if (c < nv) {
                f32x4 y;
#pragma unroll
                for (int k = 0; k < 4; ++k) y[k] = first_half ? o[k] * cs[k] + (-p[k]) * sn[k] : o[k] * cs[k] + p[k] * sn[k];
                if (which == 0) {
#pragma unroll
                    for (int k = 0; k < 4; ++k) y[k] *= kQLog2e;
                }
                _Float16 hh[4], ll[4];
#pragma unroll
                for (int k = 0; k < 4; ++k) split_act(y[k], hh[k], ll[k]);
                unsigned short* dst = qk16 + ((size_t)b * T + t) * (2 * D) + (size_t)which * D + 4 * c;
                *reinterpret_cast<u32x2*>(dst) = u32x2{pack_h2(hh[0], hh[1]), pack_h2(hh[2], hh[3])};
                *reinterpret_cast<u32x2*>(dst + qk_plane) = u32x2{pack_h2(ll[0], ll[1]), pack_h2(ll[2], ll[3])};
            }
        }
    }
    const int d = tid & 63, kq = tid >> 6;
    for (int h = 0; h < H; ++h) {
        _Float16 hh[8], ll[8];
        const float* vsrc = qkv + ((size_t)b * T) * RS + 2 * D + h * kHeadDim + d;
#pragma unroll
        for (int e = 0; e < 8; ++e) {
            const int t = t0 + 8 * kq + e;
            const float x = (t < T) ? vsrc[(size_t)t * RS] : 0.0f;
            split_act(x, hh[e], ll[e]);
        }
        unsigned short* row = vt16 + (((size_t)b * H + h) * kHeadDim + d) * Tp + t0 + 16 * (kq >> 1) + 4 * (kq & 1);
        *reinterpret_cast<u32x2*>(row) = u32x2{pack_h2(hh[0], hh[1]), pack_h2(hh[2], hh[3])};
        *reinterpret_cast<u32x2*>(row + 8) = u32x2{pack_h2(hh[4], hh[5]), pack_h2(hh[6], hh[7])};
        *reinterpret_cast<u32x2*>(row + vt_plane) = u32x2{pack_h2(ll[0], ll[1]), pack_h2(ll[2], ll[3])};
        *reinterpret_cast<u32x2*>(row + vt_plane + 8) = u32x2{pack_h2(ll[4], ll[5]), pack_h2(ll[6], ll[7])};
    }
}

int launch_qkln_prep(const float* qkv, const float* q_w, const float* k_w, float eps, const float* cos_t, const float* sin_t, int B,
                     int T, int H, unsigned short* qk16, size_t qk_plane, unsigned short* vt16, size_t vt_plane, hipStream_t s) {
    const int nv = H * kHeadDim / 4, Tp = (T + 31) / 32 * 32;
    if (B <= 0 || T <= 0 || H <= 0 || nv > 512) { set_error("qkln_prep: bad shape B=%d T=%d H=%d (D = 64 H <= 2048)", B, T, H); return PGMI_EINVAL; }
    const dim3 grid((T + 31) / 32, B);
#define PGMI_QKLN(NV_) hipLaunchKernelGGL(qkln_prep_kernel<NV_>, grid, dim3(256), 0, s, qkv, q_w, k_w, eps, cos_t, sin_t, T, H, Tp, \
                                          qk16, qk_plane, vt16, vt_plane)
    if (nv <= 64) PGMI_QKLN(1);
    else if (nv <= 128) PGMI_QKLN(2);
    else if (nv <= 192) PGMI_QKLN(3);
    else if (nv <= 256) PGMI_QKLN(4);
    else if (nv <= 320) PGMI_QKLN(5);
    else PGMI_QKLN(8);
#undef PGMI_QKLN
    PGMI_HIP(hipGetLastError());
    return PGMI_OK;
}

void launch_qkv_prep(dim3 grid, hipStream_t s, const float* qkv, const float* cos_t, const float* sin_t, int rotary, int T, int H, int Tp,
                     unsigned short* qk16, size_t qk_plane, unsigned short* vt16, size_t vt_plane) {
    hipLaunchKernelGGL(qkv_prep_kernel, grid, dim3(256), 0, s, qkv, cos_t, sin_t, rotary, T, H, Tp, qk16, qk_plane, vt16, vt_plane);
}
void launch_qkv_prep_conv(dim3 grid, hipStream_t s, const float* qkv, const float* conv, int T, int H, int Tp, unsigned short* qk16, size_t qk_plane,
                          unsigned short* vt16, size_t vt_plane, const RagMap* rag) {
    if (rag)
        hipLaunchKernelGGL(qkv_prep_conv_kernel<true>, grid, dim3(256), 0, s, qkv, conv, T, H, Tp, qk16, qk_plane, vt16, vt_plane,
                           rag->seq_off, rag->seq_p, rag->seq_q, rag->seq_root, rag->seq_vt, rag->ent_seq, rag->ent_j);
    else
        hipLaunchKernelGGL(qkv_prep_conv_kernel<false>, grid, dim3(256), 0, s, qkv, conv, T, H, Tp, qk16, qk_plane, vt16, vt_plane,
                           nullptr, nullptr, nullptr, nullptr, nullptr, nullptr, nullptr);
}

}
```

### proteingym_amd/csrc/attention_f16_v3.hip

```cpp
#include <stdlib.h>
#include <string.h>
#include <algorithm>

#include "attention_f16_common.h"

namespace pgmi {

template <int WPB, int OUT>
__global__ __launch_bounds__(WPB * 64, 2) void attention_f16x3_v3_kernel(
    const unsigned short* __restrict__ qk16, size_t qk_plane, const unsigned short* __restrict__ vt16, size_t vt_plane,
    const int32_t* __restrict__ kv_len, int T, int H, int Tp, float* __restrict__ ctx, unsigned short* __restrict__ ctx16,
    int dense_nblk, int nseq) {
    constexpr float defer_thr = kAttDefer;
    constexpr int DH = 64, NSTG = 3, KCPR = 8, KCH = AKT * KCPR, VCH = DH * 4, STG_CH = 2 * KCH + 2 * VCH;
    constexpr int NWI = STG_CH / 64, NDMA = (NWI + WPB - 1) / WPB, NS = 4, ND = 2;
    extern __shared__ __attribute__((aligned(16))) u32x4 lds[];
    int b, h, qblk;
    if (dense_nblk > 0) {
        const int pair = xcd_local_pair(dense_nblk, qblk);
        if (pair >= nseq * H) return;
        b = pair / H;
        h = pair - b * H;
    } else {
        b = blockIdx.z;
        h = blockIdx.y;
        qblk = blockIdx.x;
    }
    const int tid = threadIdx.x, lane = tid & 63;
    const int wave = __builtin_amdgcn_readfirstlane(tid >> 6);
    const int r = lane & 31, kh = lane >> 5;
    const int D = H * DH;
    const int Tk = kv_len ? kv_len[b] : T;
    const int q0 = (qblk * WPB + wave) * 32;
    const bool active = q0 < T;
    const int nkt = (Tk + AKT - 1) / AKT;
    const size_t seq_halfs = (size_t)T * (2 * D), vt_halfs = (size_t)DH * Tp;
    const unsigned long long qk_bytes = std::min<unsigned long long>(0xFFFFFFFFull, (unsigned long long)qk_plane * 2ull + seq_halfs * 2ull);
    const unsigned long long vt_bytes = std::min<unsigned long long>(0xFFFFFFFFull, (unsigned long long)vt_plane * 2ull + vt_halfs * 2ull);
    const __amdgpu_buffer_rsrc_t rsQK = operand_rsrc(qk16 + (size_t)b * seq_halfs, qk_bytes);
    const __amdgpu_buffer_rsrc_t rsVT = operand_rsrc(vt16 + ((size_t)b * H + h) * vt_halfs, vt_bytes);

    static_assert(WPB == 1 || WPB == 2 || WPB == 4, "the DMA map needs WPB to divide 8");
    constexpr int NK = 8 / WPB;
    int kvoff[NK], krow[NK], vvoff[NDMA - NK];
#pragma unroll
    for (int i = 0; i < NK; ++i) {
        const int q4 = (wave + WPB * i) & 3;
        const int key = q4 * 8 + (lane >> 3);
        krow[i] = key;
        kvoff[i] = ((lane & 7) ^ k_swizzle<DH>(key)) * 16;
    }
#pragma unroll
    for (int i = 0; i < NDMA - NK; ++i) {
        const int q4 = (wave + WPB * (i + NK)) & 3;
        const int g = q4 * 64 + lane, d = g >> 2, c = (g & 3) ^ ((d >> 2) & 3);
        vvoff[i] = d * Tp * 2 + c * 16;
    }
    auto issue_piece = [&](int i, int m, int stage, bool on) {
        u32x4* base = lds + stage * STG_CH;
        const int kk = min(m, nkt - 1), vv = min(max(m - 2, 0), nkt - 1);
        if (i < NK) {
            const int wi = wave + WPB * i, p = (WPB * i) >> 2;
            const int kr = krow[i < NK ? i : 0], ko = kvoff[i < NK ? i : 0];
            const int vo = on ? min(kk * AKT + kr, T - 1) * (2 * D) * 2 + ko : -16;
            const int so = (int)((unsigned int)p * (unsigned int)qk_plane * 2u + (unsigned int)(D + h * DH) * 2u);
            __builtin_amdgcn_raw_ptr_buffer_load_lds(rsQK, (__attribute__((address_space(3))) void*)(base + wi * 64), 16, vo, so, 0, 0);
        } else {
            const int wi = wave + WPB * i, p = (WPB * i - 8) >> 2;
            const int so = (int)((unsigned int)p * (unsigned int)vt_plane * 2u) + vv * ((AKT / 8) * 16);
            const int vv0 = vvoff[i >= NK ? i - NK : 0];
            const int vo = on ? vv0 : -16;
            __builtin_amdgcn_raw_ptr_buffer_load_lds(rsVT, (__attribute__((address_space(3))) void*)(base + wi * 64), 16, vo, so, 0, 0);
        }
    };
    auto issue_bundle = [&](int m, int stage, bool on) {
#pragma unroll
        for (int i = 0; i < NDMA; ++i) issue_piece(i, m, stage, on);
    };
    const int last_bundle = nkt + 1;

    issue_bundle(0, 0, true);
    u32x4 qh[NS], ql[NS];
    {
        u32x4* qbase = lds + STG_CH + wave * (2 * KCH);
        if (active) {
            constexpr int NQ = 2 * KCH / 64;
#pragma unroll
            for (int i = 0; i < NQ; ++i) {
                const int f = i * 64 + lane, pq = f / KCH, row = (f % KCH) / KCPR;
                const int c = (f % KCPR) ^ k_swizzle<DH>(row);
                const int vo = (int)(((unsigned int)min(q0 + row, T - 1) * (unsigned int)(2 * D) + (unsigned int)(h * DH)) * 2u + (unsigned int)c * 16u);
                const int so = (int)((unsigned int)pq * (unsigned int)qk_plane * 2u);
                __builtin_amdgcn_raw_ptr_buffer_load_lds(rsQK, (__attribute__((address_space(3))) void*)(qbase + i * 64), 16, vo, so, 0, 0);
            }
        }
        asm volatile("s_waitcnt vmcnt(0)" ::: "memory");
        if (active) {
#pragma unroll
            for (int s = 0; s < NS; ++s) {
                const int ci = r * KCPR + ((2 * s + kh) ^ k_swizzle<DH>(r));
                qh[s] = qbase[ci];
// ... 187 lines not shown
        PGMI_SLOT();
        sm = mfma_h(k1h, qh[3], sm);
        dma_slot(5);
#undef PGMI_SLOT
    };
    auto closing_pv = [&](const u32x4* stage) {
        apply_pending();
        const u32x4* Vb = stage + 2 * KCH;
        u32x4 va_h[ND], va_l[ND], vb_h[ND], vb_l[ND];
        vfrag(Vb, 0, va_h, va_l);
        vfrag(Vb, 1, vb_h, vb_l);
        pv(0, va_h, va_l);
        pv(1, vb_h, vb_l);
    };
    using T1 = std::integral_constant<bool, true>;
    using T0 = std::integral_constant<bool, false>;

    if (active && nkt > 0) {
#pragma unroll
        for (int s = 0; s < NS; ++s) {
            const int ci = r * KCPR + ((2 * s + kh) ^ k_swizzle<DH>(r));
            const u32x4 kfh = lds[ci], kfl = lds[KCH + ci];
            sc = mfma_h(kfh, ql[s], s == 0 ? zero16 : sc);
            sc = mfma_h(kfl, qh[s], sc);
            sm = mfma_h(kfh, qh[s], s == 0 ? zero16 : sm);
        }
    }
    auto wait_bundle = [&](int younger) {
        if (younger >= 1) asm volatile("s_waitcnt vmcnt(%0)" ::"n"(NDMA) : "memory");
        else asm volatile("s_waitcnt vmcnt(0)" ::: "memory");
    };
    int cur = 1;
    auto step_head = [&](int kt) {
        wait_bundle(1);
        __builtin_amdgcn_s_barrier();
        asm volatile("" ::: "memory");
    };
    auto idle_dma = [&](int kt) {
        issue_bundle(kt + 3, cur == 0 ? NSTG - 1 : cur - 1, kt + 3 <= last_bundle);
    };
    for (int kt = 0; kt < nkt - 1; ++kt) {
        step_head(kt);
        if (active) step(T0{}, kt, lds + cur * STG_CH, cur == 0 ? NSTG - 1 : cur - 1);
        else idle_dma(kt);
        cur = (cur == NSTG - 1) ? 0 : cur + 1;
    }
    step_head(nkt - 1);
    if (active) step(T1{}, nkt - 1, lds + cur * STG_CH, cur == 0 ? NSTG - 1 : cur - 1);
    else idle_dma(nkt - 1);
    cur = (cur == NSTG - 1) ? 0 : cur + 1;
    asm volatile("s_waitcnt vmcnt(0)" ::: "memory");
    __builtin_amdgcn_s_barrier();
    asm volatile("" ::: "memory");
    if (active) closing_pv(lds + cur * STG_CH);

    if (active) {
        const float l_tot = l_run + __shfl_xor(l_run, 32);
        const float inv = 1.0f / l_tot;
        const bool row_ok = q0 + r < T;
        const size_t orow = (size_t)(b * T + min(q0 + r, T - 1));
        if (OUT == ATT_OUT_BF16) store_ctx_bf16<ND>(om, oc, inv, kInvLo, row_ok, ctx16 + orow * (size_t)D + (size_t)h * DH, kh);
        else if (OUT == ATT_OUT_SPLIT) store_ctx_split<ND>(om, oc, inv, kInvLo, row_ok, ctx16 + orow * (size_t)(2 * D) + (size_t)(ND * h) * 64, kh);
        else if (row_ok) store_ctx_f32<ND>(om, oc, inv, kInvLo, ctx + (size_t)(b * T + q0 + r) * D + (size_t)h * DH + 4 * kh);
    }
}

static int g_att_v3 = -1;
void att_v3_set_option(int value) { g_att_v3 = value; }
bool att_v3_serves(const AttLaunch& a) {
    if (g_att_v3 == 0 || a.conv || a.slopes || a.head_dim != 64) return false;
    return g_att_v3 > 0 || (a.T + 31) / 32 >= 7;
}

using Att16v3Kernel = decltype(&attention_f16x3_v3_kernel<4, ATT_OUT_F32>);
struct Att16v3Inst { int wpb, out; Att16v3Kernel fn; };
template <int WPB, int OUT>
static constexpr Att16v3Inst att16v3_inst() { return {WPB, OUT, attention_f16x3_v3_kernel<WPB, OUT>}; }
static const Att16v3Inst kAtt16v3[] = {
    att16v3_inst<1, ATT_OUT_F32>(),   att16v3_inst<2, ATT_OUT_F32>(),   att16v3_inst<4, ATT_OUT_F32>(),
    att16v3_inst<1, ATT_OUT_SPLIT>(), att16v3_inst<2, ATT_OUT_SPLIT>(), att16v3_inst<4, ATT_OUT_SPLIT>(),
    att16v3_inst<1, ATT_OUT_BF16>(),  att16v3_inst<2, ATT_OUT_BF16>(),  att16v3_inst<4, ATT_OUT_BF16>(),
};

int launch_att16v3(const AttLaunch& a, int wpb, dim3 grid, int dense_nblk) {
    constexpr size_t lds_bytes = (size_t)3 * (2 * AKT * 8 + 2 * 64 * 4) * 16;
    for (const Att16v3Inst& k : kAtt16v3) {
        if (k.wpb != wpb || k.out != a.out) continue;
        hipLaunchKernelGGL(k.fn, grid, dim3(wpb * 64), lds_bytes, a.stream, a.qk16, a.qk_plane, a.vt16, a.vt_plane, a.kv_len, a.T, a.H, (a.T + 31) / 32 * 32,
                           a.ctx, a.ctx16, dense_nblk, a.B);
        PGMI_HIP(hipGetLastError());
        return PGMI_OK;
    }
    set_error("attention_f16x3_v3: no kernel for %d waves, output %d", wpb, (int)a.out);
    return PGMI_EINVAL;
}

}
```

### proteingym_amd/csrc/common.h

```cpp
#pragma once
#include <hip/hip_runtime.h>
#include <stdint.h>
#include <stddef.h>

#include "../../include/pgmi.h"

namespace pgmi {

void set_error(const char* fmt, ...);

#define PGMI_HIP(expr)                                                                   \
    do {                                                                                 \
        hipError_t _e = (expr);                                                          \
        if (_e != hipSuccess) {                                                          \
            pgmi::set_error("%s failed: %s (%s:%d)", #expr, hipGetErrorString(_e),       \
                            __FILE__, __LINE__);                                         \
            return PGMI_EHIP;                                                            \
        }                                                                                \
    } while (0)

typedef float f32x4 __attribute__((ext_vector_type(4)));
typedef float f32x16 __attribute__((ext_vector_type(16)));

constexpr int kWave = 64;
constexpr int kHeadDim = 64;

enum Epilogue { EPI_NONE = 0, EPI_GELU = 1, EPI_SQRELU = 2, EPI_GELU_TANH = 3,
                EPI_SWIGLU = 4,
                EPI_RELU = 5 };

constexpr float kLoScale = 2048.0f;
constexpr float kQLog2e = 1.4426950408889634f;

__host__ __device__ __forceinline__ size_t ki_off(size_t row, int k, int K) {
    return row * (size_t)(2 * K) + (size_t)(k >> 5) * 64 + (size_t)(k & 31);
}
#if defined(__HIPCC__)
__device__ __forceinline__ void split_act(float x, _Float16& hi, _Float16& lo) {
    hi = (fabsf(x) < 6.103515625e-05f) ? (_Float16)0.0f : (_Float16)x;
    lo = (_Float16)((x - (float)hi) * kLoScale);
}
typedef _Float16 f16x4 __attribute__((ext_vector_type(4)));
__device__ __forceinline__ void split_act4(f32x4 x, f16x4& hi, f16x4& lo) {
    f32x4 xz, lo32;
#pragma unroll
    for (int e = 0; e < 4; ++e) xz[e] = (fabsf(x[e]) < 6.103515625e-05f) ? 0.0f : x[e];
    hi = __builtin_convertvector(xz, f16x4);
    const f32x4 xs = x * f32x4{kLoScale, kLoScale, kLoScale, kLoScale};
#pragma unroll
    for (int e = 0; e < 4; ++e) lo32[e] = __builtin_fmaf((float)hi[e], -kLoScale, xs[e]);
    lo = __builtin_convertvector(lo32, f16x4);
}
__device__ __forceinline__ void split_act4_prod(f32x4 a, f32x4 b, f16x4& hi, f16x4& lo) {
    const f32x4 x = a * b;
    f32x4 xz, lo32;
#pragma unroll
    for (int e = 0; e < 4; ++e) xz[e] = (fabsf(x[e]) < 6.103515625e-05f) ? 0.0f : x[e];
    hi = __builtin_convertvector(xz, f16x4);
#pragma unroll
    for (int e = 0; e < 4; ++e) lo32[e] = __builtin_fmaf(a[e], b[e], -(float)hi[e]);
    lo = __builtin_convertvector(lo32 * f32x4{kLoScale, kLoScale, kLoScale, kLoScale}, f16x4);
}
__device__ __forceinline__ void store_split4(f32x4 o, unsigned short* y16, size_t row, int c, int lane, int D) {
    typedef _Float16 h4 __attribute__((ext_vector_type(4)));
    typedef unsigned int u32x2 __attribute__((ext_vector_type(2)));
    typedef unsigned int u32x4 __attribute__((ext_vector_type(4)));
    h4 hi, lo;
#pragma unroll
    for (int k = 0; k < 4; ++k) {
        _Float16 a, b;
        split_act(o[k], a, b);
        hi[k] = a;
        lo[k] = b;
    }
    const u32x2 H = __builtin_bit_cast(u32x2, hi), L = __builtin_bit_cast(u32x2, lo);
    const bool odd = lane & 1;
    const unsigned int s0 = odd ? H[0] : L[0], s1 = odd ? H[1] : L[1];
    const unsigned int r0 = __shfl_xor(s0, 1), r1 = __shfl_xor(s1, 1);
    const u32x4 out = odd ? u32x4{r0, r1, L[0], L[1]} : u32x4{H[0], H[1], r0, r1};
    *reinterpret_cast<u32x4*>(y16 + ki_off(row, 4 * (c & ~1), D) + (odd ? 32 : 0)) = out;
}
#endif

void launch_make_masked_windows(const int32_t* wt, const int32_t* win_start, const int32_t* mask_rel,
                                int B, int T, int32_t* tokens_out, hipStream_t s);
void launch_apply_mask(int32_t* tokens, const int32_t* mask_pos, int B, int T, hipStream_t s);
void launch_seq_stats(const int32_t* tokens, int B, int T, int token_dropout, float* scale,
                      int32_t* pos_idx, int32_t* kv_len, hipStream_t s, int mask_id = PGMI_TOK_MASK);
void launch_zero_pad_rows(const int32_t* tokens, int rows, int D, float* x, hipStream_t s);
void launch_embed(const int32_t* tokens, const float* scale, const int32_t* pos_idx,
                  const float* embed_tokens, const float* embed_positions, int token_dropout,
                  int rows, int T, int D, float* x, hipStream_t s, int mask_id = PGMI_TOK_MASK);
void launch_layernorm(const float* x, const float* w, const float* b, int rows, int D, float eps,
                      float* y, hipStream_t s);
void launch_gather_rows(const float* x, const int32_t* row_idx, int n, int D, float* y, hipStream_t s);
void launch_strided_index(int first, int stride, int n, int32_t* idx, hipStream_t s);
void launch_vocab_logsoftmax(const float* h, const float* E, const float* bias, int rows, int D,
                             int V, float* out, int32_t* nonfinite, hipStream_t s);
void launch_layernorm16(const float* x, const float* w, const float* b, int rows, int D, float eps,
                        unsigned short* y16, int mode, hipStream_t s);
int launch_rmsnorm16(const float* x, const float* w, int rows, int D, float eps, unsigned short* y16, hipStream_t s);
void launch_scatter_rows(const float* src, const int32_t* dst_row, int n, int V, float* table,
                         hipStream_t s);
void launch_row_index(const int32_t* mask_rel, int B, int T, int32_t* out, hipStream_t s);
void launch_fill_f32(float* p, int64_t n, float v, hipStream_t s);
void launch_seq_loglik(const float* lp, const int32_t* tokens, const int32_t* lens, int B, int T, int V,
                       const float* prior, const int32_t* a0, const int32_t* row0, const int32_t* n,
                       const int32_t* flip, float alpha, const float* eve, float beta, int eve_fallback, float* out, hipStream_t s);
void launch_seq_loglik_ragged(const float* lp, const int32_t* tokens, const int32_t* seq_off, const int32_t* seq_p,
                              const int32_t* seq_root, int B, int T, int V, const float* prior, const int32_t* a0,
                              const int32_t* row0, const int32_t* n, const int32_t* flip, float alpha, const float* eve, float beta,
                              int eve_fallback, float* out, hipStream_t s);
void launch_pg2_seq_loglik(const float* lp, const int32_t* col, const int32_t* n_kept, int B, int T, int V, float* out, hipStream_t s);
void launch_embed_learned(const int32_t* tokens, const float* E, const float* P, int rows, int T, int D, float* x, hipStream_t s);
void launch_embed_scaled_pos(const int32_t* tokens, const int32_t* pos, const float* E, const float* P, float scale, int rows, int D,
                             float* x, hipStream_t s);
void launch_wide_logsoftmax(const float* logits, int ldl, int rows, int V, const int32_t* tgt, float* out, int32_t* nonfinite,
                            hipStream_t s);
// ... 98 lines not shown
void launch_s2f_pick_logits(const float* lp, const int32_t* cols, int L, int T, int V, int64_t rows, float* out, hipStream_t s);
int s2f_set_option(const char* name, long long value);

void launch_mlstm_m(const float* g1, const float* Tmx, const int32_t* tok, int tok_stride, int rows, int Hp, unsigned short* m16,
                    float* m32, hipStream_t s);
struct MlstmGate {
    const float* z = nullptr;
    const float* Tx = nullptr;
    const int32_t* tok = nullptr;
    int tok_stride = 0;
    float* c = nullptr;
    unsigned short* h16 = nullptr;
    float* h32 = nullptr;
    float* hwin = nullptr;
    float* z_out = nullptr;
    int rows = 0, Hp = 0;
};
void launch_mlstm_gate(const MlstmGate& a, hipStream_t s);
void launch_mlstm_init(const float* ctab, const uint32_t* htab, const float* tlp, const int32_t* tgt, const int32_t* join, int rows,
                       int Hp, int Lc, float* c, uint32_t* h, float* terms, hipStream_t s);
void launch_mlstm_head(const float* hwin, size_t slot_stride, int W, const float* Wd, const float* bd, const int32_t* tgt,
                       const int32_t* join, int Lc, int t0, int nw, int rows, int Hp, float* terms, float* lp, hipStream_t s);
void launch_mlstm_score(const float* terms, const int32_t* tgt, int rows, int Lc, double* out, hipStream_t s);
int unirep_set_option(const char* name, long long value);

void launch_msa_window_tokens(const int32_t* full, int R, int Tfull, int start, int Tw, int mask_col, int32_t* out, hipStream_t s);
void launch_add_row_embedding(float* x, const float* pe, int R, int C, int D, hipStream_t s);
void launch_permute_rows(const float* src, float* dst, int A, int B, int D, hipStream_t s);
void launch_tied_prep_qk(const float* qkv, int64_t M, int D, unsigned short* q16, unsigned short* k16, hipStream_t s);
void launch_pack_vt16(const float* qkv, int R, int C, int Kp, int H, unsigned short* Vt, hipStream_t s);
int launch_tied_softmax16(const float* part, int H, int S, int C, int Kp, float scale, unsigned short* P, hipStream_t s);
float tied_w_scale();
struct TiedRowLaunch {
    const float* qkv = nullptr;
    int R = 0, C = 0, H = 0;
    int S = 0;
    unsigned short* qctx16 = nullptr;
    unsigned short* k16 = nullptr;
    float* part = nullptr;
    float* p = nullptr;
    float* vt = nullptr;
    hipStream_t stream = nullptr;
};
int tied_row_kp(int C);
int tied_row_splits(int R, int C, int H);
int tied_row_check(int R, int C, int H, int S);
int launch_tied_row_attention(const TiedRowLaunch& t);

int launch_gemm_f32(const float* A, const float* W, const float* bias, const float* residual,
                    float* C, int M, int N, int K, int epilogue, hipStream_t s);

void gemm_options_from_env();
int gemm_set_option(const char* name, long long value);
struct GemmLaunch {
    const unsigned short* A = nullptr;
    const unsigned short* W = nullptr;
    float out_scale = 1.0f;
    const float* bias = nullptr;
    const float* residual = nullptr;
    float* out32 = nullptr;
    unsigned short* out16 = nullptr;
    int M = 0, N = 0, K = 0;
    int epilogue = EPI_NONE;
    bool bf = false;
    int variant = 0;
    hipStream_t stream = nullptr;
    struct Qkv {
        unsigned short* vt16 = nullptr;
        size_t vt_plane = 0, qk_plane = 0;
        const float* cos_t = nullptr;
        const float* sin_t = nullptr;
        int rotary = 0, T = 0, H = 0, rot_halves = 1;
    } qkv;
};
int launch_gemm16(const GemmLaunch& g);
struct XMap;
int launch_gemm16_ex(const unsigned short* A, const unsigned short* W, float* Cf, unsigned short* Ch, int M, int N, int K,
                     float out_scale, XMap xm, int nbatch, hipStream_t s);
void launch_split16(const float* x, int64_t n, float scale, int mode, int K, unsigned short* out, hipStream_t s);

int launch_qkln_prep(const float* qkv, const float* q_w, const float* k_w, float eps, const float* cos_t, const float* sin_t, int B,
                     int T, int H, unsigned short* qk16, size_t qk_plane, unsigned short* vt16, size_t vt_plane, hipStream_t s);

struct GeomAttLaunch {
    const float* proj = nullptr;
    int pitch = 0;
    const float *rot = nullptr, *trans = nullptr;
    const int32_t* mask = nullptr;
    bool per_row_frames = false;
    const float *w_rot = nullptr, *w_dist = nullptr;
    int B = 0, S = 0, H = 0;
    float* out = nullptr;
    int opitch = 0;
    hipStream_t stream = nullptr;
};
int launch_geom_attention(const GeomAttLaunch& g);
int geom_key_tile(int S);
void launch_esm3_embed(const int32_t* tokens, const int32_t* stok, const int32_t* plddt, const float* seq_embed, const float* struct_embed,
                       const float* cst, int rows, int T, int D, float* x, hipStream_t s);

int launch_attention_f32(const float* qkv, const int32_t* kv_len, int B, int T, int H, float* ctx, hipStream_t s,
                         int head_dim = 64);

enum AttOut {
    ATT_OUT_F32 = 0,
    ATT_OUT_SPLIT = 1,
    ATT_OUT_BF16 = 2
};
struct AttLaunch {
    unsigned short* qk16 = nullptr;
    size_t qk_plane = 0;
    unsigned short* vt16 = nullptr;
    size_t vt_plane = 0;
    int B = 1, T = 0, H = 0;
    int head_dim = 64;
    const int32_t* kv_len = nullptr;
    const float* slopes = nullptr;
    AttOut out = ATT_OUT_F32;
    float* ctx = nullptr;
    unsigned short* ctx16 = nullptr;
    hipStream_t stream = nullptr;
    const float* qkv = nullptr;
    const float* conv = nullptr;
    const float* cos_t = nullptr;
    const float* sin_t = nullptr;
    int rotary = 0;
};
int launch_attention_f16x3_v2(const AttLaunch& a);

struct AttRagged {
    const int32_t* seq_off;
    const int32_t* seq_p;
    const int32_t* seq_q;
    const int32_t* seq_root;
    const uint32_t* seq_vt;
    const int32_t* tile_seq;
    const int32_t* tile_j;
    const int32_t* blk_seq;
    const int32_t* blk_j;
    int n_tiles, n_blocks;
};
struct PrefixAttLaunch {
    const float* qkv = nullptr;
    const int32_t* pos = nullptr;
    const float* cos_t = nullptr;
    const float* sin_t = nullptr;
    const int32_t* seg_off = nullptr;
    const int32_t* ent_seg = nullptr;
    const int32_t* ent_tile = nullptr;
    int n_seg = 0, n_ent = 0, H = 0;
    unsigned short* q16 = nullptr;
    size_t q_plane = 0;
    unsigned short* k16 = nullptr;
    unsigned short* vt16 = nullptr;
    size_t pitch = 0;
    const unsigned short* pk16 = nullptr;
    const unsigned short* pvt16 = nullptr;
    size_t ppitch = 0;
    int P = 0;
    AttOut out = ATT_OUT_SPLIT;
    float* ctx = nullptr;
    unsigned short* ctx16 = nullptr;
    hipStream_t stream = nullptr;
};
int launch_prefix_prep(const PrefixAttLaunch& p);
int launch_prefix_attention(const PrefixAttLaunch& p);
int launch_cross_q_prep(const float* q, size_t rows, int H, unsigned short* q16, size_t q_plane, hipStream_t s);
int launch_cross_attention(const PrefixAttLaunch& p);

int att16_waves_per_block(int T);
int att_set_option(const char* name, long long value);
int launch_attention_tr_ragged(const AttLaunch& a, const AttRagged& rg);

}
```

### proteingym_amd/csrc/gemm16x_kernel.h

```cpp
#pragma once
#include <type_traits>

#include "common.h"

namespace pgmi {

typedef _Float16 h8 __attribute__((ext_vector_type(8)));
typedef _Float16 h4 __attribute__((ext_vector_type(4)));
typedef __bf16 b8 __attribute__((ext_vector_type(8)));
typedef unsigned int u32x4 __attribute__((ext_vector_type(4)));
typedef unsigned int u32x2 __attribute__((ext_vector_type(2)));

__device__ __forceinline__ f32x4 gelu_erf16(f32x4 x) {
    auto all = [](float v) { return f32x4{v, v, v, v}; };
    const f32x4 b = __builtin_elementwise_max(-__builtin_elementwise_abs(x), all(-6.0f));
    f32x4 q = __builtin_elementwise_fma(x, all(0.0f), all(3.309269596e-05f));
    q = __builtin_elementwise_fma(q, b, all(7.692188374e-04f));
    q = __builtin_elementwise_fma(q, b, all(8.080714382e-03f));
    q = __builtin_elementwise_fma(q, b, all(5.341210216e-02f));
    q = __builtin_elementwise_fma(q, b, all(-4.587709904e-01f));
    q = __builtin_elementwise_fma(q, b, all(1.151201725e+00f));
    q = __builtin_elementwise_fma(q, b, all(-9.999930859e-01f));
    const f32x4 e = {__builtin_amdgcn_exp2f(q[0]), __builtin_amdgcn_exp2f(q[1]), __builtin_amdgcn_exp2f(q[2]), __builtin_amdgcn_exp2f(q[3])};
    return __builtin_elementwise_fma(b, e, __builtin_elementwise_max(x, all(0.0f)));
// ... 280 lines not shown
        item += gridDim.x;
        const bool more = item < n_items;
        if (more) {
            decode(item);
            issue_tile(0, 0);
        }

        if constexpr (OUT == 2) {
            const int Dm = N / 3;
            const int nb = en0 + wn * 64;
            if (nb < N) {
            const int which = nb / Dm, hcol = nb - which * Dm, hh = hcol >> 6;
            constexpr int SPQ = 144;
            unsigned char* patch_q = patches + wave * (2 * 32 * SPQ);
            const bool staged_q = which < 2;
            f32x4 bq0[2], bq1[2];
#pragma unroll
            for (int g = 0; g < 2; ++g) {
                bq0[g] = *reinterpret_cast<const f32x4*>(bias + nb + 16 * g + 4 * kq);
                bq1[g] = *reinterpret_cast<const f32x4*>(bias + nb + 32 + 16 * g + 4 * kq);
            }
#pragma unroll
            for (int g = 0; g < 2; ++g) asm volatile("" :: "v"(bq0[g]), "v"(bq1[g]));
            auto emit = [&](auto interior_c) {
            constexpr bool INT = decltype(interior_c)::value;
            unsigned char* const lane_cell = patch_q + r * SPQ + kq * 8;
            unsigned short* const int_dst = !INT ? nullptr : Ch + (size_t)(em0 + wm * TM * 16 + (lane >> 3)) * (2 * Dm) + (size_t)which * Dm + hcol + (lane & 7) * 8;
#pragma unroll
            for (int ib = 0; ib < TM / 2; ++ib) {
#pragma unroll
            for (int s = 0; s < 2; ++s) {
                const int i = 2 * ib + s;
                const int m = em0 + (wm * TM + i) * 16 + r;
                const bool row_ok = m < M;
                if (!INT && !row_ok) continue;
                int bb = 0, t = 0;
                if (!INT || qo.rotary) {
                    bb = m / qo.T;
                    t = m - bb * qo.T;
                }
                f32x4 rc[2], rs[2];
                if ((INT || which < 2) && qo.rotary) {
                    const int tr = (min(t, qo.T - 1) * qo.rot_halves + (hh % qo.rot_halves)) * 64;
#pragma unroll
                    for (int g = 0; g < 2; ++g) {
                        rc[g] = *reinterpret_cast<const f32x4*>(qo.cos_t + tr + 16 * g + 4 * kq);
                        rs[g] = *reinterpret_cast<const f32x4*>(qo.sin_t + tr + 16 * g + 4 * kq);
                    }
                }
#pragma unroll
                for (int g = 0; g < 2; ++g) {
                    const int d0 = 16 * g + 4 * kq;
                    const f32x4 b0 = bq0[g], b1 = bq1[g];
                    float x0[4], x1[4];
#pragma unroll
                    for (int e = 0; e < 4; ++e) {
                        x0[e] = fmaf(acc[g][i][e], out_scale, b0[e]);
                        x1[e] = fmaf(acc[g + 2][i][e], out_scale, b1[e]);
                    }
                    if (which == 0) {
#pragma unroll
                        for (int e = 0; e < 4; ++e) { x0[e] *= kQLog2e; x1[e] *= kQLog2e; }
                    }
                    if (INT || which < 2) {
                        if (qo.rotary) {
                            const f32x4 c1 = rc[g], s1 = rs[g], c2 = rc[g], s2 = rs[g];
#pragma unroll
                            for (int e = 0; e < 4; ++e) {
                                const float y0 = fmaf(x0[e], c1[e], (-x1[e]) * s1[e]);
                                const float y1 = fmaf(x1[e], c2[e], x0[e] * s2[e]);
                                x0[e] = y0;
                                x1[e] = y1;
                            }
                        }
                        h4 hi0, lo0, hi1, lo1;
                        split_act4(f32x4{x0[0], x0[1], x0[2], x0[3]}, hi0, lo0);
                        split_act4(f32x4{x1[0], x1[1], x1[2], x1[3]}, hi1, lo1);
                        unsigned char* cell = lane_cell + (16 * s) * SPQ + 32 * g;
                        lds_put(cell, hi0);
                        lds_put(cell + 32 * SPQ, lo0);
                        lds_put(cell + 64, hi1);
                        lds_put(cell + 32 * SPQ + 64, lo1);
                    } else {
                        const int tk = t & 31;
                        const int pos = (t & ~31) + ((tk & 0x13) | ((tk & 4) << 1) | ((tk & 8) >> 1));
                        unsigned short* col = qo.vt16 + (((size_t)bb * qo.H + hh) * kHeadDim + d0) * qo.Tp + pos;
#pragma unroll
                        for (int e = 0; e < 4; ++e) {
                            _Float16 a0, l0, a1, l1;
                            split_act(x0[e], a0, l0);
                            split_act(x1[e], a1, l1);
                            unsigned short* c0 = col + (size_t)e * qo.Tp;
                            unsigned short* c1p = c0 + (size_t)32 * qo.Tp;
                            c0[0] = __builtin_bit_cast(unsigned short, a0);
                            c0[qo.vt_plane] = __builtin_bit_cast(unsigned short, l0);
                            c1p[0] = __builtin_bit_cast(unsigned short, a1);
                            c1p[qo.vt_plane] = __builtin_bit_cast(unsigned short, l1);
                        }
                    }
                }
            }
                if (INT || staged_q) {
                    __builtin_amdgcn_wave_barrier();
                    const int m_base = em0 + (wm * TM + 2 * ib) * 16;
#pragma unroll
                    for (int k = 0; k < 4; ++k) {
                        const int q = lane + 64 * k, row = q >> 3, cc = q & 7;
                        const u32x4 vh = *reinterpret_cast<const u32x4*>(patch_q + row * SPQ + cc * 16);
                        const u32x4 vl = *reinterpret_cast<const u32x4*>(patch_q + (32 + row) * SPQ + cc * 16);
                        if (INT || m_base + row < M) {
                            unsigned short* dst = INT ? int_dst + (size_t)(32 * ib + 8 * k) * (size_t)(2 * Dm)
                                                      : Ch + (size_t)(m_base + row) * (2 * Dm) + (size_t)which * Dm + hcol + cc * 8;
                            *reinterpret_cast<u32x4*>(dst) = vh;
                            *reinterpret_cast<u32x4*>(dst + c_plane) = vl;
                        }
                    }
                    __builtin_amdgcn_wave_barrier();
                }
            }
            };
            if (staged_q && em0 + (wm + 1) * (TM * 16) <= M) emit(std::true_type{});
            else emit(std::false_type{});
            }
        } else if constexpr (OUT == 0) {
            unsigned char* patch = patches + wave * (32 * 128);
            const int cc = lane & 7, rq = lane >> 3;
            const unsigned int kOob = 0x80000000u;
            const unsigned int ldc = xm.ldc ? (unsigned int)xm.ldc : (unsigned int)N;
            const long long cb = xm.tiles_per_batch ? (long long)(eb % xm.batch_inner) * xm.c_b0 + (long long)(eb / xm.batch_inner) * xm.c_b1 : 0;
            const __amdgpu_buffer_rsrc_t rsC = __builtin_amdgcn_make_buffer_rsrc(Cf + cb, 0, (int)((unsigned int)M * ldc * 4u), 0x00020000);
            const __amdgpu_buffer_rsrc_t rsR = __builtin_amdgcn_make_buffer_rsrc(const_cast<float*>(residual ? residual : Cf) + cb, 0, (int)((unsigned int)M * ldc * 4u), 0x00020000);
            constexpr int NB = TN / 2;
            unsigned int coff[NB];
            f32x4 bv[NB];
#pragma unroll
            for (int j = 0; j < NB; ++j) {
                const int n = en0 + wn * 64 + j * 32 + cc * 4;
                coff[j] = n < N ? (unsigned int)n * 4u : kOob;
                bv[j] = (bias && n < N) ? *reinterpret_cast<const f32x4*>(bias + n) : f32x4{0.f, 0.f, 0.f, 0.f};
            }
#pragma unroll
            for (int j = 0; j < NB; ++j) asm volatile("" :: "v"(bv[j]));
            auto c_off = [&](int m, int j) -> int {
                return (int)((m < M && coff[j] != kOob) ? (unsigned int)m * ldc * 4u + coff[j] : kOob);
            };
            u32x4 rv[2][NB][4];
            auto load_residual = [&](int i, u32x4 (&dst)[NB][4]) {
                const int m_base = em0 + (wm * TM + 2 * i) * 16;
#pragma unroll
                for (int j = 0; j < NB; ++j)
#pragma unroll
                    for (int k = 0; k < 4; ++k)
                        dst[j][k] = __builtin_bit_cast(u32x4, __builtin_amdgcn_raw_buffer_load_b128(rsR, c_off(m_base + rq + 8 * k, j), 0, 0));
            };
            if (residual) load_residual(0, rv[0]);
#pragma unroll
            for (int i = 0; i < TM / 2; ++i) {
                const int m_base = em0 + (wm * TM + 2 * i) * 16;
                if (residual && i + 1 < TM / 2) load_residual(i + 1, rv[(i + 1) & 1]);
#pragma unroll
                for (int j = 0; j < NB; ++j) {
#pragma unroll
                    for (int s = 0; s < 2; ++s)
#pragma unroll
                        for (int u = 0; u < 2; ++u) {
                            const int prow = 16 * s + r;
                            *reinterpret_cast<f32x4*>(patch + prow * 128 + (((4 * u + kq) ^ (prow & 7)) << 4)) = acc[2 * j + u][2 * i + s];
                        }
// ... 232 lines not shown
```

### proteingym_amd/csrc/model.h

```cpp
#pragma once
#include <math.h>
#include <stdlib.h>
#include <cmath>
#include <algorithm>
#include <stdarg.h>
#include <stdio.h>
#include <string.h>

#include <string>
#include <vector>

#include "common.h"
#include "gemm16x_kernel.h"
#include "packed_chunks.h"

namespace pgmi {

struct W16 {
    unsigned short* p = nullptr;
    float out_scale = 1.0f;
};

struct Layer {
    float *ln1_w, *ln1_b, *wqkv, *bqkv, *wo, *bo, *ln2_w, *ln2_b, *w1, *b1, *w2, *b2;
    W16 wqkv16, wo16, w116, w216;
    float* conv = nullptr;
    float *c_ln_w = nullptr, *c_ln_b = nullptr, *c_bqkv = nullptr, *c_bo = nullptr;
    W16 c_wqkv16, c_wo16;
    float* c_bq = nullptr;
    W16 c_wq16;
    float *q_ln = nullptr, *k_ln = nullptr;
    float* gate = nullptr;
    std::vector<W16> ew1, ew2;
    float *g_norm_w = nullptr, *g_wrot = nullptr, *g_wdist = nullptr;
    W16 g_proj16, g_out16;
};

struct ProfEvent {
    hipEvent_t start, stop;
    int cls;
};

struct PrefixCache {
    unsigned short* planes = nullptr;
    size_t pitch = 0, plane = 0, cap = 0;
    int rows = 0;
    int32_t* meta = nullptr;
    static size_t plan_ints(size_t cap) { return 3 * cap + 2; }
    static size_t meta_ints(size_t cap) { return 2 * plan_ints(cap) + cap + 4; }
    unsigned short* k(int l) const { return planes ? planes + (size_t)l * 4 * plane : nullptr; }
    unsigned short* vt(int l) const { return planes ? k(l) + 2 * plane : nullptr; }
    int32_t* plan(int slot) const { return meta + (size_t)slot * plan_ints(cap); }
    int32_t* seq_off() const { return plan(2); }
};

}

using namespace pgmi;

struct pgmi_assay;
struct pgmi_pppl;

struct pgmi_model {
    pgmi_config cfg;
    int device = 0;
    hipStream_t stream = nullptr;
    std::vector<void*> allocs;
    std::vector<pgmi_assay*> assays;
    std::vector<pgmi_pppl*> pppls;
    float *embed_tokens = nullptr, *embed_positions = nullptr;
    float *lnb_w = nullptr, *lnb_b = nullptr, *lna_w = nullptr, *lna_b = nullptr;
    float *hd_w = nullptr, *hd_b = nullptr, *hln_w = nullptr, *hln_b = nullptr;
    float *head_w = nullptr, *head_b = nullptr;
    std::vector<Layer> layers;
    W16 hd16;
    int fc1_epi = EPI_GELU, fc1_cols = 0;
    bool embed_gather = false;
    int mask_id = PGMI_TOK_MASK, n_token_ids = PGMI_VOCAB;
    float* slopes = nullptr;
    float* tr_prior = nullptr;
    size_t tr_prior_cap = 0;
    int32_t* tr_meta = nullptr;
    size_t tr_meta_cap = 0;
    int pg2_rotary = 0;
    float *pg2_aa_w = nullptr, *pg2_aa_b = nullptr;
    int gpt_Vp = 0, gpt_head_rows = 0;
    bool parallel_residual = false;
    float* gpt_logits = nullptr;
    W16 gpt_head16;
    double* gpt_sum = nullptr;
    bool rms_norm = false;
    int pg3_E = 0, pg3_k = 0, pg3_gated = 0;
    struct MoeWs {
        int32_t *ids = nullptr, *slot = nullptr, *blk_cnt = nullptr, *blk_base = nullptr, *counts_seg = nullptr;
        float *wts = nullptr, *y = nullptr, *t32 = nullptr;
        unsigned short *a16 = nullptr, *g16 = nullptr;
        int32_t* counts_host = nullptr;
        size_t layer_stride = 0;
    } moe;
    float* msa_pe = nullptr;
    float* xt = nullptr;
    int32_t *msa_full = nullptr, *msa_kv_len = nullptr;
    size_t msa_full_cap = 0;
    float *tied_part = nullptr, *tied_p = nullptr, *tied_vt = nullptr;
    size_t tied_part_cap = 0, tied_p_cap = 0, tied_vt_cap = 0;
    int msa_kv_R = 0, msa_kv_C = 0;
    float ln_eps = 1e-5f;
    bool final_norm = false;
    PrefixCache pfx;
    std::vector<float> poet_prompt_lp;
    int if1_enc = 0, if1_pos_len = 0;
    float *if1_mem = nullptr, *if1_pos = nullptr;
    unsigned short* if1_mem16 = nullptr;
    int e3_vheads = 0, e3_Kp = 0;
    float *e3_struct_embed = nullptr, *e3_const = nullptr;
    int32_t *e3_stok = nullptr, *e3_plddt = nullptr, *e3_mask = nullptr;
    float *e3_rot = nullptr, *e3_trans = nullptr;
    size_t e3_cap = 0;
    int e3_T = 0;
    bool e3_framed = false;
    unsigned short *h16 = nullptr, *g16 = nullptr;
    size_t h16_plane = 0, g16_plane = 0;
    unsigned short *qk16 = nullptr, *vt16 = nullptr;
    size_t qk16_plane = 0, vt16_plane = 0;
    int32_t* nonfinite = nullptr;
    int gemm_variant = 0;
    int keep_rows = 1;
    int last_B = 0, last_T = 0;
    int dh = kHeadDim;
    int rot_halves = 1;
    int Hs = 0;
    int Da = 0;
    float *rot_cos = nullptr, *rot_sin = nullptr;
    int rot_len = 0;
    float* zeros = nullptr;
    int max_rows = 0;
    float *x = nullptr, *h = nullptr, *qkv = nullptr, *g = nullptr, *lp = nullptr, *denom = nullptr;
    int32_t *tokens = nullptr, *pos_idx = nullptr, *kv_len = nullptr, *row_idx = nullptr, *aux_i = nullptr;
    bool prof = false;
    std::vector<ProfEvent> events;
    size_t events_used = 0;
    double prof_ms[PGMI_K_COUNT] = {0};
    int64_t prof_n[PGMI_K_COUNT] = {0};
    double prof_flops[PGMI_K_COUNT] = {0};
    double prof_bytes[PGMI_K_COUNT] = {0};
};

struct pgmi_assay {
    pgmi_model* m = nullptr;
    int n_tok = 0, P = 0, T = 0;
    int64_t n_mut = 0, n_sub = 0;
    std::vector<void*> allocs;
    int32_t *wt = nullptr, *positions = nullptr, *win_start = nullptr, *mask_rel = nullptr;
    int32_t *sub_pos = nullptr, *sub_wt = nullptr, *sub_mt = nullptr;
    int64_t* mut_off = nullptr;
    float* table = nullptr;
    double* scores = nullptr;
};

struct pgmi_pppl {
    pgmi_model* m = nullptr;
    int64_t N = 0;
    std::vector<int64_t> off;
    std::vector<void*> allocs;
    uint8_t* tok8 = nullptr;
    int64_t* off_dev = nullptr;
    int64_t last_rows = 0, last_chunks = 0, last_tokens = 0, last_padded = 0;
};

namespace pgmi {

template <typename T>
int dev_alloc(std::vector<void*>& pool, T** p, size_t n) {
    void* q = nullptr;
    if (n == 0) n = 1;
    hipError_t e = hipMalloc(&q, n * sizeof(T));
    if (e != hipSuccess) {
        set_error("hipMalloc(%zu bytes) failed: %s", n * sizeof(T), hipGetErrorString(e));
        return PGMI_ENOMEM;
    }
    pool.push_back(q);
    *p = static_cast<T*>(q);
    return PGMI_OK;
}

template <typename T>
int dev_upload(std::vector<void*>& pool, T** p, const T* host, size_t n) {
    int rc = dev_alloc(pool, p, n);
    if (rc) return rc;
    if (n) PGMI_HIP(hipMemcpy(*p, host, n * sizeof(T), hipMemcpyHostToDevice));
    return PGMI_OK;
}

struct ProfScope {
    pgmi_model* m;
    ProfEvent* ev = nullptr;
    ProfScope(pgmi_model* m_, int cls, double flops, double bytes) : m(m_) {
        if (!m->prof) return;
        if (m->events_used == m->events.size()) {
            ProfEvent e;
            if (hipEventCreate(&e.start) != hipSuccess || hipEventCreate(&e.stop) != hipSuccess) return;
            m->events.push_back(e);
        }
        ev = &m->events[m->events_used++];
        ev->cls = cls;
        m->prof_n[cls] += 1;
        m->prof_flops[cls] += flops;
        m->prof_bytes[cls] += bytes;
        hipEventRecord(ev->start, m->stream);
    }
    ~ProfScope() {
        if (ev) hipEventRecord(ev->stop, m->stream);
    }
};

template <typename T>
int ensure_cap(pgmi_model* m, T** p, size_t* cap, size_t need) {
    if (need <= *cap) return PGMI_OK;
    T* q = nullptr;
    int rc = dev_alloc(m->allocs, &q, need);
    if (rc) return rc;
    *p = q;
    *cap = need;
    return PGMI_OK;
}

int prof_drain(pgmi_model* m);
int check_cfg(const pgmi_config* c);
int check_tokens(const int32_t* tokens, int B, int T, int n_ids = PGMI_VOCAB);
int check_vocab(const int32_t* tokens, int B, int T, int V);
int env_int(const char* name, int dflt);
int make_w16(std::vector<void*>& pool, const float* host, size_t n, size_t K, int precision, hipStream_t s, W16* out);
int linear(pgmi_model* m, const float* in32, const unsigned short* in16, const float* W32, const W16& w16, const float* bias,
           const float* residual, float* out32, unsigned short* out16, int M, int N, int K, int epi);
GemmLaunch qkv_launch(pgmi_model* m, const W16& w16, const float* bias, int M, int Da, int K, int T, int H);
PrefixAttLaunch prefix_launch(pgmi_model* m, const SegPlan& pl);
int alloc_prefix_cache(pgmi_model* m);
int check_nonfinite(pgmi_model* m);
int reset_pad_keys(pgmi_model* m, int B, int T);
int model_create(const pgmi_config* cfg, const float* w, int64_t n_weights, int device, pgmi_model** out, int arch_arg,
                 const pgmi_pg3_params* pg3 = nullptr);
int create_esm(pgmi_model* m, const pgmi_config* cfg, const float* w, int64_t n_weights);
int ensure_rotary(pgmi_model* m, int T);
int upload_rotate_half(pgmi_model* m, int n);
int run_encoder(pgmi_model* m, int B, int T, const int32_t* keep = nullptr, int n_keep = 0, bool* compacted = nullptr);
int head_hidden(pgmi_model* m, int R, const int32_t* row_idx);
int run_head(pgmi_model* m, int R, const int32_t* row_idx);
int run_rows(pgmi_model* m, int B, int T, int R, const int32_t* row_idx);
int create_tranception(pgmi_model* m, const pgmi_config* cfg, const float* w, int64_t n_weights);
int create_progen2(pgmi_model* m, const pgmi_config* cfg, const float* w, int64_t n_weights, int rotary_dim);
int create_gpt(pgmi_model* m, const pgmi_config* cfg, const float* w, int64_t n_weights, int pos_kind);
int64_t gpt_weight_count(const pgmi_config* c, int pos_kind);
int decoder_check(pgmi_model* m, int arch, int T);
int run_decoder(pgmi_model* m, int B, int T, const AttRagged* rg = nullptr, int rows = 0, double att_flops = 0);
int self_attention(pgmi_model* m, const Layer& L, int B, int T, const AttRagged* rg = nullptr, int rows = 0, double att_flops = 0);
int out_proj(pgmi_model* m, const W16& wo16, const float* bo, int M);
int ffn(pgmi_model* m, const Layer& L, int M);
int narrow_head(pgmi_model* m, const float* src, int n);
int loglik_tail(pgmi_model* m, const int32_t* row_idx, int R, const int32_t* d_off, int bc, double* sum);
int decoder_token_logprobs(pgmi_model* m, int arch, const int32_t* tokens, int B, int T, float* out);
int decoder_sequence_loglik(pgmi_model* m, int arch, const int32_t* tokens, const int32_t* lens, int B, int T, double* sum, int32_t* n_targets);
int pg3_check(const pgmi_config* c, const pgmi_pg3_params* p);
int64_t pg3_weight_count(const pgmi_config* c, const pgmi_pg3_params* p);
int create_progen3(pgmi_model* m, const pgmi_config* cfg, const float* w, int64_t n_weights, const pgmi_pg3_params* p);
void pack_swiglu(const float* w1, const float* w3, size_t F, size_t D, float* dst);
int moe_ws_alloc(std::vector<void*>& pool, pgmi_model::MoeWs* ws, size_t rows, size_t layers, int D, int F, int E, int top_k, int gated);
int dense_ffn(pgmi_model* m, const pgmi_model::MoeWs& ws, const W16& w1, const W16& w2, const unsigned short* h16, unsigned short* g16,
              int M, int D, int F, int gated, float* x);
int pg3_ffn(pgmi_model* m, const Layer& L, int layer, int M);
int moe_ffn(pgmi_model* m, const pgmi_model::MoeWs& ws, const std::vector<W16>& ew1, const std::vector<W16>& ew2,
            const unsigned short* h16, const int32_t* ids, const float* wts, int M, int D, int F, int E, int top_k, int gated, float* x);
int64_t poet_weight_count(const pgmi_config* c, int final_norm);
int create_poet(pgmi_model* m, const pgmi_config* cfg, const float* w, int64_t n_weights, int final_norm);
struct PackedScorer {
    int (*forward)(pgmi_model* m, int bc, int R, const SegPlan& pl);
    int pos_len;
    const char* pos_what;
    const char* not_ready;
    bool same_length;
    bool vocab_per_row;
    int skip_target;
    bool mean;
};
int score_packed(pgmi_model* m, const PackedScorer& e, const int32_t* tokens, const int32_t* lens, int B, int T, bool loglik, float* out,
                 double* sum);
int if1_check(const pgmi_config* c, int enc_dim);
int64_t if1_weight_count(const pgmi_config* c, int enc_dim);
int create_esmif1(pgmi_model* m, const pgmi_config* cfg, const float* w, int64_t n_weights, int enc_dim);
int64_t esmc_weight_count(const pgmi_config* c);
int create_esmc(pgmi_model* m, const pgmi_config* cfg, const float* w, int64_t n_weights);
int esm3_check(const pgmi_config* c, int v_heads);
int64_t esm3_weight_count(const pgmi_config* c, int v_heads);
int create_esm3(pgmi_model* m, const pgmi_config* cfg, const float* w, int64_t n_weights, int v_heads);
int esm3_embed(pgmi_model* m, int B, int T);
int geom_branch(pgmi_model* m, const Layer& L, int B, int T);
int create_saprot(pgmi_model* m, const pgmi_config* cfg, const float* w, int64_t n_weights, int mask_id);
int create_msa(pgmi_model* m, const pgmi_config* cfg, const float* w, int64_t n_weights);
int run_msa(pgmi_model* m, int R, int C, int keep_col = -1, bool* compacted = nullptr);

inline bool esm2_rotary(int arch) { return arch == PGMI_ARCH_ESM2 || arch == PGMI_ARCH_SAPROT; }
inline bool esmc_blocks(int arch) { return arch == PGMI_ARCH_ESMC || arch == PGMI_ARCH_ESM3; }

struct BlobCursor {
    pgmi_model* m;
    const float *p, *end;
    int rc = PGMI_OK;
    BlobCursor(pgmi_model* m_, const float* w, int64_t n_weights) : m(m_), p(w), end(w + n_weights) {}
    const float* take(size_t n) { p += n; return p - n; }
    void upload(float** dst, const float* host, size_t n) { if (!rc) rc = dev_upload(m->allocs, dst, host, n); }
    void upload(float** dst, size_t n) { upload(dst, take(n), n); }
    void w16(W16* dst, const float* host, size_t n, size_t K) { if (!rc) rc = make_w16(m->allocs, host, n, K, m->cfg.precision, m->stream, dst); }
    void w16(W16* dst, size_t n, size_t K) { w16(dst, take(n), n, K); }
    void linear(float** w32, W16* w16_, const float* host, size_t n, size_t K) {
        if (m->cfg.precision == PGMI_PREC_FP32) upload(w32, host, n); else w16(w16_, host, n, K);
    }
    void linear(float** w32, W16* w16_, size_t n, size_t K) { linear(w32, w16_, take(n), n, K); }
    int finish() {
        if (!rc && p != end) { set_error("internal: blob walk mismatch"); rc = PGMI_EINVAL; }
        return rc;
    }
};

inline size_t rotate_half_slot(size_t col, size_t dh) {
    const size_t h = col / dh, j = col % dh;
    if (dh > 64) return (2 * h + ((j >> 5) & 1)) * 64 + ((j >> 6) << 5) + (j & 31);
    return h * 64 + (j < dh / 2 ? j : 32 + (j - dh / 2));
}

template <typename Slot>
void pack_qkv_slots(const float* src, size_t D, size_t Da, Slot slot, float qscale, float* wq, float* bq = nullptr) {
    for (size_t k = 0; k < 3; ++k) {
// ... 62 lines not shown
```

Baseline: 18550.

## Share layer-0 QKV across masked copies and restrict last-layer attention to masked query tile

For masked-marginal chunks where every copy is the same window with one masked position, layer 0's layernorm and QKV GEMM run on only two prototype rows per position instead of B*T. An expand kernel then builds each copy's q/k/V^T from the unmasked prototype, using the masked prototype at that copy's mask position. In the last layer, when only masked rows are kept, attention runs just the query tile containing the mask position through a new QSEL variant of the v3 kernel. This removes most layer-0 GEMM work and most final-layer attention work, at the cost of an extra expand kernel, a memset and host-side planning at assay creation.

```diff
diff --git a/include/pgmi.h b/include/pgmi.h
--- a/include/pgmi.h
+++ b/include/pgmi.h
@@ -149,6 +149,9 @@
 int pgmi_op_cross_attention(int device, const float* q, const int32_t* seg_off, int n_seg, const float* mem_kv, int S, int heads,
                             int split, float* ctx);
 int pgmi_op_packed_chunks(const int32_t* lens, int B, int drop_last, int same_length, int max_rows, int32_t* out_b1, int32_t* out_n);
+int pgmi_op_layer0_plan(const int32_t* win_start, const int32_t* mask_rel, int bc, int T, int32_t* src);
+int pgmi_op_expand_layer0(int device, const uint16_t* proto_qk, const uint16_t* proto_vt, const int32_t* mask_rel, int B, int T, int H,
+                          uint16_t* qk, uint16_t* vt);
 int pgmi_op_rmsnorm(int device, const float* x, const float* w, int rows, int D, float eps, float* y);
 int pgmi_op_geom_attention(int device, const float* proj, const float* rot, const float* trans, const int32_t* frame_mask,
                            int per_row_frames, const float* w_rot, const float* w_dist, int B, int S, int H, float* out);
diff --git a/proteingym_amd/_lib.py b/proteingym_amd/_lib.py
--- a/proteingym_amd/_lib.py
+++ b/proteingym_amd/_lib.py
@@ -52,6 +52,7 @@
 _f32p = C.POINTER(C.c_float)
 _f64p = C.POINTER(C.c_double)
 _u8p = C.POINTER(C.c_uint8)
+_u16p = C.POINTER(C.c_uint16)
 
 SIGNATURES = [
     ("pgmi_abi_version", C.c_int, []),
@@ -165,6 +166,8 @@
     ("pgmi_op_prefix_attention", C.c_int, [C.c_int, _f32p, _i32p, C.c_int, _f32p, C.c_int, C.c_int, C.c_int, _f32p]),
     ("pgmi_op_cross_attention", C.c_int, [C.c_int, _f32p, _i32p, C.c_int, _f32p, C.c_int, C.c_int, C.c_int, _f32p]),
     ("pgmi_op_packed_chunks", C.c_int, [_i32p, C.c_int, C.c_int, C.c_int, C.c_int, _i32p, _i32p]),
+    ("pgmi_op_layer0_plan", C.c_int, [_i32p, _i32p, C.c_int, C.c_int, _i32p]),
+    ("pgmi_op_expand_layer0", C.c_int, [C.c_int, _u16p, _u16p, _i32p, C.c_int, C.c_int, C.c_int, _u16p, _u16p]),
     ("pgmi_op_rmsnorm", C.c_int, [C.c_int, _f32p, _f32p, C.c_int, C.c_int, C.c_float, _f32p]),
     ("pgmi_op_geom_attention", C.c_int, [C.c_int, _f32p, _f32p, _f32p, _i32p, C.c_int, _f32p, _f32p, C.c_int, C.c_int, C.c_int, _f32p]),
     ("pgmi_op_geom_key_tile", C.c_int, [C.c_int]),
diff --git a/proteingym_amd/csrc/api_esm.hip b/proteingym_amd/csrc/api_esm.hip
--- a/proteingym_amd/csrc/api_esm.hip
+++ b/proteingym_amd/csrc/api_esm.hip
@@ -59,7 +59,47 @@
     });
 }
 
-int run_encoder(pgmi_model* m, int B, int T, const int32_t* keep, int n_keep, bool* compacted) {
+static GemmLaunch layer_qkv_launch(pgmi_model* m, const Layer& L, int M, int T) {
+    const pgmi_config& c = m->cfg;
+    GemmLaunch g = qkv_launch(m, L.wqkv16, L.bqkv, M, m->Da, c.embed_dim, T, m->Hs);
+    g.bf = c.precision == PGMI_PREC_BF16;
+    g.qkv.cos_t = m->rot_cos; g.qkv.sin_t = m->rot_sin; g.qkv.rotary = esm2_rotary(c.arch); g.qkv.rot_halves = m->rot_halves;
+    return g;
+}
+
+static bool layer0_shared_serves(const pgmi_model* m, const Layer& L, int B, int T, const MaskedCopies* cp) {
+    const pgmi_config& c = m->cfg;
+    return cp && cp->l0_src && cp->mask_rel && m->share_layer0 && B >= 2 && T >= 2 && (c.arch == PGMI_ARCH_ESM1B || c.arch == PGMI_ARCH_ESM2) &&
+           c.precision != PGMI_PREC_FP32 && !L.q_ln && (size_t)2 * ((T + 31) / 32 * 32) <= (size_t)m->max_rows;
+}
+static int layer0_shared(pgmi_model* m, const Layer& L, int B, int T, const MaskedCopies& cp) {
+    const pgmi_config& c = m->cfg;
+    const size_t D = c.embed_dim, Da = m->Da, P = (size_t)2 * T, Tp = ((size_t)T + 31) / 32 * 32;
+    hipStream_t s = m->stream;
+    ExpandLayer0 e;
+    e.pqk_plane = P * 2 * Da;
+    e.pvt_plane = 2 * Da * Tp;
+    unsigned short* pqk = reinterpret_cast<unsigned short*>(m->qkv);
+    unsigned short* pvt = pqk + 2 * e.pqk_plane;
+    { ProfScope p(m, PGMI_K_LAYERNORM, 0, 4.0 * P * D * 4);
+      launch_gather_rows(m->x, cp.l0_src, (int)P, (int)D, m->g, s);
+      launch_layernorm16(m->g, L.ln1_w, L.ln1_b, (int)P, (int)D, 1e-5f, m->h16, c.precision == PGMI_PREC_F16X3 ? 1 : 2, s); }
+    const double out_bytes = 2.0 * 2 * ((double)B * T * 2 * Da + (double)B * Da * Tp);
+    ProfScope p(m, PGMI_K_GEMM_QKV, 2.0 * P * 3 * D * D, out_bytes + 2.0 * 2 * (e.pqk_plane + e.pvt_plane));
+    PGMI_HIP(hipMemsetAsync(pvt, 0, 2 * e.pvt_plane * sizeof(unsigned short), s));
+    GemmLaunch g = layer_qkv_launch(m, L, (int)P, T);
+    g.out16 = pqk; g.qkv.qk_plane = e.pqk_plane;
+    g.qkv.vt16 = pvt; g.qkv.vt_plane = e.pvt_plane;
+    int rc = launch_gemm16(g);
+    if (rc) return rc;
+    e.pqk = pqk; e.pvt = pvt; e.mask_rel = cp.mask_rel;
+    e.B = B; e.T = T; e.H = m->Hs;
+    e.qk16 = m->qk16; e.qk_plane = m->qk16_plane; e.vt16 = m->vt16; e.vt_plane = m->vt16_plane;
+    e.stream = s;
+    return launch_expand_layer0(e);
+}
+
+int run_encoder(pgmi_model* m, int B, int T, const int32_t* keep, int n_keep, bool* compacted, const MaskedCopies* copies) {
     const pgmi_config& c = m->cfg;
     const int M = B * T, D = c.embed_dim, F = c.ffn_dim, N1 = m->fc1_cols, H = c.heads, Da = m->Da;
     hipStream_t s = m->stream;
@@ -86,19 +126,19 @@
     const int mode16 = (prec == PGMI_PREC_F16X3) ? 1 : 2;
     for (int l = 0; l < c.layers; ++l) {
         const Layer& L = m->layers[l];
-        { ProfScope p(m, PGMI_K_LAYERNORM, 0, ln_bytes);
-          if (prec == PGMI_PREC_FP32) launch_layernorm(m->x, L.ln1_w, L.ln1_b, M, D, 1e-5f, m->h, s);
-          else launch_layernorm16(m->x, L.ln1_w, L.ln1_b, M, D, 1e-5f, m->h16, mode16, s); }
         const bool fused_qkv = prec != PGMI_PREC_FP32 && !L.q_ln;
-        { ProfScope p(m, PGMI_K_GEMM_QKV, 2.0 * M * 3 * D * D, 0);
-          if (fused_qkv) {
-              GemmLaunch g = qkv_launch(m, L.wqkv16, L.bqkv, M, Da, D, T, m->Hs);
-              g.bf = prec == PGMI_PREC_BF16;
-              g.qkv.cos_t = m->rot_cos; g.qkv.sin_t = m->rot_sin; g.qkv.rotary = esm2_rotary(c.arch); g.qkv.rot_halves = m->rot_halves;
-              rc = launch_gemm16(g);
-          } else
-              rc = linear(m, m->h, m->h16, L.wqkv, L.wqkv16, L.bqkv, nullptr, m->qkv, nullptr, M, 3 * Da, D, EPI_NONE);
-          if (rc) return rc; }
+        const bool kept_rows = keep && m->keep_rows && l == c.layers - 1 && !L.g_norm_w;
+        if (l == 0 && layer0_shared_serves(m, L, B, T, copies)) {
+            if ((rc = layer0_shared(m, L, B, T, *copies))) return rc;
+        } else {
+            { ProfScope p(m, PGMI_K_LAYERNORM, 0, ln_bytes);
+              if (prec == PGMI_PREC_FP32) launch_layernorm(m->x, L.ln1_w, L.ln1_b, M, D, 1e-5f, m->h, s);
+              else launch_layernorm16(m->x, L.ln1_w, L.ln1_b, M, D, 1e-5f, m->h16, mode16, s); }
+            { ProfScope p(m, PGMI_K_GEMM_QKV, 2.0 * M * 3 * D * D, 0);
+              if (fused_qkv) rc = launch_gemm16(layer_qkv_launch(m, L, M, T));
+              else rc = linear(m, m->h, m->h16, L.wqkv, L.wqkv16, L.bqkv, nullptr, m->qkv, nullptr, M, 3 * Da, D, EPI_NONE);
+              if (rc) return rc; }
+        }
         { ProfScope p(m, PGMI_K_ATTENTION, 4.0 * M * T * D, L.q_ln ? (double)M * D * 20 : 0);
           if (L.q_ln && (rc = launch_qkln_prep(m->qkv, L.q_ln, L.k_ln, 1e-5f, m->rot_cos, m->rot_sin, B, T, H, m->qk16, m->qk16_plane,
                                                m->vt16, m->vt16_plane, s)))
@@ -110,6 +150,7 @@
               a.qk16 = m->qk16, a.qk_plane = m->qk16_plane, a.vt16 = m->vt16, a.vt_plane = m->vt16_plane;
               a.B = B, a.T = T, a.H = H, a.head_dim = m->rot_halves * kHeadDim;
               a.kv_len = m->kv_len;
+              if (kept_rows && copies) a.q_sel = copies->mask_rel;
               a.out = prec == PGMI_PREC_F16X3 ? ATT_OUT_SPLIT : ATT_OUT_BF16;
               a.ctx16 = m->h16;
               a.stream = s;
@@ -118,7 +159,7 @@
               rc = launch_attention_f32(m->qkv, m->kv_len, B, T, H, m->h, s, m->rot_halves * kHeadDim);
           }
           if (rc) return rc; }
-        if (keep && m->keep_rows && l == c.layers - 1 && !L.g_norm_w) {
+        if (kept_rows) {
             const int R = n_keep;
             ProfScope p(m, PGMI_K_KEPT_ROWS, 2.0 * R * D * (Da + N1 + F), 0);
             launch_gather_rows(m->x, keep, R, D, m->qkv, s);
@@ -188,9 +229,9 @@
 }
 
 
-int run_rows(pgmi_model* m, int B, int T, int R, const int32_t* row_idx) {
+int run_rows(pgmi_model* m, int B, int T, int R, const int32_t* row_idx, const MaskedCopies* copies) {
     bool compacted = false;
-    int rc = run_encoder(m, B, T, row_idx, R, &compacted);
+    int rc = run_encoder(m, B, T, row_idx, R, &compacted, copies);
     if (rc) return rc;
     return run_head(m, R, compacted ? nullptr : row_idx);
 }
@@ -236,7 +277,9 @@
         PGMI_HIP(hipMemcpyAsync(m->aux_i, mask_pos + b0, (size_t)bc * 4, hipMemcpyHostToDevice, m->stream));
         PGMI_HIP(hipMemcpyAsync(m->row_idx, ridx.data(), (size_t)bc * 4, hipMemcpyHostToDevice, m->stream));
         launch_apply_mask(m->tokens, m->aux_i, bc, T, m->stream);
-        int rc = run_rows(m, bc, T, bc, m->row_idx);
+        MaskedCopies cp;
+        cp.mask_rel = m->aux_i;
+        int rc = run_rows(m, bc, T, bc, m->row_idx, &cp);
         if (rc) return rc;
         PGMI_HIP(hipMemcpyAsync(out + (size_t)b0 * V, m->lp, (size_t)bc * V * 4, hipMemcpyDeviceToHost, m->stream));
         return PGMI_OK;
@@ -284,6 +327,16 @@
     if (!rc) rc = dev_upload(a->allocs, &a->mut_off, mut_off, (size_t)(n_mut + 1));
     if (!rc) rc = dev_alloc(a->allocs, &a->table, (size_t)n_tok * PGMI_VOCAB);
     if (!rc) rc = dev_alloc(a->allocs, &a->scores, (size_t)n_mut);
+    a->l0_per = rows_per_chunk(m, T);
+    std::vector<int32_t> src;
+    for (int p0 = 0; p0 < P; p0 += a->l0_per) {
+        const int bc = std::min(a->l0_per, P - p0);
+        src.resize(src.size() + (size_t)2 * T, 0);
+        a->l0_ok.push_back(layer0_plan(ws.data() + p0, mr.data() + p0, bc, T, src.data() + src.size() - (size_t)2 * T));
+    }
+    if (!rc) rc = dev_upload(a->allocs, &a->l0_src, src.data(), src.size());
+    a->h_win_start = std::move(ws);
+    a->h_mask_rel = std::move(mr);
     if (rc) { pgmi_assay_destroy(a); return rc; }
     m->assays.push_back(a);
     *out = a;
@@ -313,7 +366,11 @@
         const int bc = std::min(per, a->P - p0);
         launch_make_masked_windows(a->wt, a->win_start + p0, a->mask_rel + p0, bc, T, m->tokens, s);
         launch_row_index(a->mask_rel + p0, bc, T, m->row_idx, s);
-        int rc = run_rows(m, bc, T, bc, m->row_idx);
+        const size_t chunk = (size_t)(p0 / per);
+        MaskedCopies cp;
+        cp.mask_rel = a->mask_rel + p0;
+        if (per == a->l0_per && a->l0_ok[chunk]) cp.l0_src = a->l0_src + chunk * 2 * T;
+        int rc = run_rows(m, bc, T, bc, m->row_idx, &cp);
         if (rc) return rc;
         launch_scatter_rows(m->lp, a->positions + p0, bc, V, a->table, s);
     }
diff --git a/proteingym_amd/csrc/api_model.hip b/proteingym_amd/csrc/api_model.hip
--- a/proteingym_amd/csrc/api_model.hip
+++ b/proteingym_amd/csrc/api_model.hip
@@ -401,6 +401,7 @@
     if (!rc) rc = alloc_workspace(m);
     if (rc) { pgmi_model_destroy(m); return rc; }
     m->keep_rows = env_int("PGMI_KEEP_ROWS", 1);
+    m->share_layer0 = env_int("PGMI_SHARE_LAYER0", 1);
     gemm_options_from_env();
     m->gemm_variant = env_int("PGMI_GEMM_VARIANT", 0);
     *out = m;
diff --git a/proteingym_amd/csrc/api_ops.hip b/proteingym_amd/csrc/api_ops.hip
--- a/proteingym_amd/csrc/api_ops.hip
+++ b/proteingym_amd/csrc/api_ops.hip
@@ -603,6 +603,59 @@
     return PGMI_OK;
 }
 
+int pgmi_op_layer0_plan(const int32_t* win_start, const int32_t* mask_rel, int bc, int T, int32_t* src) {
+    if (!win_start || !mask_rel || !src) { set_error("bad argument"); return PGMI_EINVAL; }
+    if (!layer0_plan(win_start, mask_rel, bc, T, src)) {
+        set_error("layer0 plan: a chunk of %d copies of %d tokens does not qualify (two or more copies of one window of two or more tokens, masks inside it)", bc, T);
+        return PGMI_EINVAL;
+    }
+    return PGMI_OK;
+}
+
+int pgmi_op_expand_layer0(int device, const uint16_t* proto_qk, const uint16_t* proto_vt, const int32_t* mask_rel, int B, int T, int H,
+                          uint16_t* qk, uint16_t* vt) {
+    if (!proto_qk || !proto_vt || !mask_rel || !qk || !vt || B <= 0 || T <= 0 || H <= 0) { set_error("bad argument"); return PGMI_EINVAL; }
+    for (int b = 0; b < B; ++b)
+        if (mask_rel[b] < 0 || mask_rel[b] >= T) { set_error("mask_rel[%d]=%d out of range", b, mask_rel[b]); return PGMI_EINVAL; }
+    if (pgmi_device_count() <= 0) { set_error("no HIP device visible"); return PGMI_ENODEV; }
+    PGMI_HIP(hipSetDevice(device));
+    constexpr size_t spare = 64;
+    const size_t Da = (size_t)H * kHeadDim, Tp = ((size_t)T + 31) / 32 * 32;
+    ExpandLayer0 e;
+    e.pqk_plane = (size_t)2 * T * 2 * Da; e.pvt_plane = 2 * Da * Tp;
+    e.qk_plane = (size_t)B * T * 2 * Da; e.vt_plane = (size_t)B * Da * Tp;
+    e.B = B; e.T = T; e.H = H;
+    std::vector<void*> pool;
+    auto cleanup = [&]() { for (void* p : pool) hipFree(p); };
+    unsigned short *dpqk = nullptr, *dpvt = nullptr, *dqk = nullptr, *dvt = nullptr;
+    int32_t* dmask = nullptr;
+    int rc = 0;
+    if ((rc = dev_upload(pool, &dpqk, reinterpret_cast<const unsigned short*>(proto_qk), 2 * e.pqk_plane)) ||
+        (rc = dev_upload(pool, &dpvt, reinterpret_cast<const unsigned short*>(proto_vt), 2 * e.pvt_plane)) ||
+        (rc = dev_upload(pool, &dmask, mask_rel, (size_t)B)) || (rc = dev_alloc(pool, &dqk, 2 * e.qk_plane + spare)) ||
+        (rc = dev_alloc(pool, &dvt, 2 * e.vt_plane + spare))) {
+        cleanup();
+        return rc;
+    }
+    hipError_t err = hipMemset(dqk, 0xFF, (2 * e.qk_plane + spare) * 2);
+    if (err == hipSuccess) err = hipMemset(dvt, 0xFF, (2 * e.vt_plane + spare) * 2);
+    if (err != hipSuccess) { cleanup(); set_error("expand layer0 op failed: %s", hipGetErrorString(err)); return PGMI_EHIP; }
+    e.pqk = dpqk; e.pvt = dpvt; e.mask_rel = dmask; e.qk16 = dqk; e.vt16 = dvt;
+    rc = launch_expand_layer0(e);
+    err = hipDeviceSynchronize();
+    unsigned short tail[2 * spare];
+    if (!rc && err == hipSuccess) err = hipMemcpy(qk, dqk, 2 * e.qk_plane * 2, hipMemcpyDeviceToHost);
+    if (!rc && err == hipSuccess) err = hipMemcpy(vt, dvt, 2 * e.vt_plane * 2, hipMemcpyDeviceToHost);
+    if (!rc && err == hipSuccess) err = hipMemcpy(tail, dqk + 2 * e.qk_plane, spare * 2, hipMemcpyDeviceToHost);
+    if (!rc && err == hipSuccess) err = hipMemcpy(tail + spare, dvt + 2 * e.vt_plane, spare * 2, hipMemcpyDeviceToHost);
+    cleanup();
+    if (rc) return rc;
+    if (err != hipSuccess) { set_error("expand layer0 op failed: %s", hipGetErrorString(err)); return PGMI_EHIP; }
+    for (size_t i = 0; i < 2 * spare; ++i)
+        if (tail[i] != 0xFFFFu) { set_error("expand layer0 op: the kernel wrote past the end of its %s output", i < spare ? "q | k" : "V^T"); return PGMI_EHIP; }
+    return PGMI_OK;
+}
+
 int pgmi_op_tied_row_splits(int R, int C, int H) {
     if (R <= 0 || C <= 0 || H <= 0) { set_error("bad argument"); return PGMI_EINVAL; }
     return tied_row_splits(R, C, H);
diff --git a/proteingym_amd/csrc/attention_f16.hip b/proteingym_amd/csrc/attention_f16.hip
--- a/proteingym_amd/csrc/attention_f16.hip
+++ b/proteingym_amd/csrc/attention_f16.hip
@@ -361,6 +361,7 @@
         launch_qkv_prep_conv(dim3(n32, H, B), a.stream, a.qkv, a.conv, T, H, Tp, a.qk16, a.qk_plane, a.vt16, a.vt_plane, nullptr);
     else if (a.qkv)
         launch_qkv_prep(dim3(n32, H, B), a.stream, a.qkv, a.cos_t, a.sin_t, a.rotary, T, H, Tp, a.qk16, a.qk_plane, a.vt16, a.vt_plane);
+    if (att_v3_sel_serves(a)) return launch_att16v3_sel(a);
     const int wpb = att16_waves_per_block(T);
     const dim3 grid = dense_grid((n32 + wpb - 1) / wpb, H, B, &dn);
     return att_v3_serves(a) ? launch_att16v3(a, wpb, grid, dn) : launch_att16v2(a, wpb, grid, nullptr, dn);
diff --git a/proteingym_amd/csrc/attention_f16_common.h b/proteingym_amd/csrc/attention_f16_common.h
--- a/proteingym_amd/csrc/attention_f16_common.h
+++ b/proteingym_amd/csrc/attention_f16_common.h
@@ -139,5 +139,7 @@
 bool att_v3_serves(const AttLaunch& a);
 void att_v3_set_option(int value);
 int launch_att16v3(const AttLaunch& a, int wpb, dim3 grid, int dense_nblk);
+bool att_v3_sel_serves(const AttLaunch& a);
+int launch_att16v3_sel(const AttLaunch& a);
 
 }
diff --git a/proteingym_amd/csrc/attention_f16_prep.hip b/proteingym_amd/csrc/attention_f16_prep.hip
--- a/proteingym_amd/csrc/attention_f16_prep.hip
+++ b/proteingym_amd/csrc/attention_f16_prep.hip
@@ -290,6 +290,82 @@
     return PGMI_OK;
 }
 
+constexpr int kExpandPerThread = 8, kExpandBlock = 256 * kExpandPerThread;
+__global__ __launch_bounds__(256) void expand_layer0_kernel(
+    const u32x4* __restrict__ pqk, size_t pqk_plane, const u32x4* __restrict__ pvt, size_t pvt_plane, const int32_t* __restrict__ mask_rel,
+    unsigned int nq, unsigned int row_pieces, unsigned int nv, unsigned int W, unsigned int bq, unsigned int bv,
+    u32x4* __restrict__ qk16, size_t qk_plane, u32x4* __restrict__ vt16, size_t vt_plane) {
+    const unsigned int b = blockIdx.y, tid = threadIdx.x;
+    const unsigned int mask = (unsigned int)mask_rel[b];
+    unsigned int blk = blockIdx.x;
+    u32x4 v[kExpandPerThread];
+    if (blk < 2 * bq) {
+        const unsigned int plane = blk >= bq;
+        blk -= plane * bq;
+        const u32x4* src = pqk + plane * pqk_plane;
+        u32x4* dst = qk16 + plane * qk_plane + (size_t)b * nq;
+        const unsigned int j0 = blk * kExpandBlock + tid, lo = mask * row_pieces, hi = lo + row_pieces;
+#pragma unroll
+        for (int u = 0; u < kExpandPerThread; ++u) {
+            const unsigned int j = min(j0 + 256u * u, nq - 1);
+            v[u] = src[(size_t)j + ((j >= lo && j < hi) ? nq : 0u)];
+        }
+#pragma unroll
+        for (int u = 0; u < kExpandPerThread; ++u) {
+            const unsigned int j = j0 + 256u * u;
+            if (j < nq) dst[j] = v[u];
+        }
+    } else {
+        blk -= 2 * bq;
+        const unsigned int plane = blk >= bv;
+        blk -= plane * bv;
+        const u32x4* src = pvt + plane * pvt_plane;
+        u32x4* dst = vt16 + plane * vt_plane + (size_t)b * nv;
+        const unsigned int j0 = blk * kExpandBlock + tid;
+        const unsigned int pos = (unsigned int)vt_key_pos((int)mask), pc = pos >> 3, pe = (pos >> 1) & 3u;
+        const unsigned int keep = (pos & 1u) ? 0x0000FFFFu : 0xFFFF0000u;
+        const unsigned int cstep = 256u % W;
+        unsigned int c = j0 % W;
+#pragma unroll
+        for (int u = 0; u < kExpandPerThread; ++u) {
+            const unsigned int j = min(j0 + 256u * u, nv - 1);
+            v[u] = src[j];
+            if (c == pc && j0 + 256u * u < nv) {
+                const u32x4 k = src[(size_t)j + nv];
+#pragma unroll
+                for (int e = 0; e < 4; ++e)
+                    if ((unsigned int)e == pe) v[u][e] = (v[u][e] & keep) | (k[e] & ~keep);
+            }
+            c += cstep;
+            if (c >= W) c -= W;
+        }
+#pragma unroll
+        for (int u = 0; u < kExpandPerThread; ++u) {
+            const unsigned int j = j0 + 256u * u;
+            if (j < nv) dst[j] = v[u];
+        }
+    }
+}
+
+int launch_expand_layer0(const ExpandLayer0& e) {
+    const size_t Da = (size_t)e.H * kHeadDim, Tp = ((size_t)e.T + 31) / 32 * 32;
+    const size_t nq = (size_t)e.T * (Da / 4), nv = Da * (Tp / 8);
+    auto odd = [](const void* p, size_t plane) { return ((uintptr_t)p & 15) != 0 || (plane & 7) != 0; };
+    if (e.B <= 0 || e.B > 65535 || e.T <= 0 || e.H <= 0 || !e.mask_rel || !e.pqk || !e.pvt || !e.qk16 || !e.vt16 ||
+        nq + nv >= (1ull << 31) || odd(e.pqk, e.pqk_plane) || odd(e.pvt, e.pvt_plane) || odd(e.qk16, e.qk_plane) || odd(e.vt16, e.vt_plane) ||
+        e.pqk_plane < 2 * nq * 8 || e.pvt_plane < 2 * nv * 8 || e.qk_plane < (size_t)e.B * nq * 8 || e.vt_plane < (size_t)e.B * nv * 8) {
+        set_error("expand_layer0: bad shape or planes B=%d T=%d H=%d", e.B, e.T, e.H);
+        return PGMI_EINVAL;
+    }
+    const unsigned int bq = (unsigned int)((nq + kExpandBlock - 1) / kExpandBlock), bv = (unsigned int)((nv + kExpandBlock - 1) / kExpandBlock);
+    hipLaunchKernelGGL(expand_layer0_kernel, dim3(2 * bq + 2 * bv, e.B), dim3(256), 0, e.stream,
+                       reinterpret_cast<const u32x4*>(e.pqk), e.pqk_plane / 8, reinterpret_cast<const u32x4*>(e.pvt), e.pvt_plane / 8, e.mask_rel,
+                       (unsigned int)nq, (unsigned int)(Da / 4), (unsigned int)nv, (unsigned int)(Tp / 8), bq, bv,
+                       reinterpret_cast<u32x4*>(e.qk16), e.qk_plane / 8, reinterpret_cast<u32x4*>(e.vt16), e.vt_plane / 8);
+    PGMI_HIP(hipGetLastError());
+    return PGMI_OK;
+}
+
 void launch_qkv_prep(dim3 grid, hipStream_t s, const float* qkv, const float* cos_t, const float* sin_t, int rotary, int T, int H, int Tp,
                      unsigned short* qk16, size_t qk_plane, unsigned short* vt16, size_t vt_plane) {
     hipLaunchKernelGGL(qkv_prep_kernel, grid, dim3(256), 0, s, qkv, cos_t, sin_t, rotary, T, H, Tp, qk16, qk_plane, vt16, vt_plane);
diff --git a/proteingym_amd/csrc/attention_f16_v3.hip b/proteingym_amd/csrc/attention_f16_v3.hip
--- a/proteingym_amd/csrc/attention_f16_v3.hip
+++ b/proteingym_amd/csrc/attention_f16_v3.hip
@@ -6,17 +6,22 @@
 
 namespace pgmi {
 
-template <int WPB, int OUT>
+template <int WPB, int OUT, bool QSEL = false>
 __global__ __launch_bounds__(WPB * 64, 2) void attention_f16x3_v3_kernel(
     const unsigned short* __restrict__ qk16, size_t qk_plane, const unsigned short* __restrict__ vt16, size_t vt_plane,
     const int32_t* __restrict__ kv_len, int T, int H, int Tp, float* __restrict__ ctx, unsigned short* __restrict__ ctx16,
-    int dense_nblk, int nseq) {
+    int dense_nblk, int nseq, const int32_t* __restrict__ q_sel) {
     constexpr float defer_thr = kAttDefer;
     constexpr int DH = 64, NSTG = 3, KCPR = 8, KCH = AKT * KCPR, VCH = DH * 4, STG_CH = 2 * KCH + 2 * VCH;
     constexpr int NWI = STG_CH / 64, NDMA = (NWI + WPB - 1) / WPB, NS = 4, ND = 2;
     extern __shared__ __attribute__((aligned(16))) u32x4 lds[];
+    static_assert(!QSEL || WPB == 1, "one query tile per block");
     int b, h, qblk;
-    if (dense_nblk > 0) {
+    if constexpr (QSEL) {
+        b = blockIdx.z;
+        h = blockIdx.y;
+        qblk = min(max(q_sel[b], 0), T - 1) >> 5;
+    } else if (dense_nblk > 0) {
         const int pair = xcd_local_pair(dense_nblk, qblk);
         if (pair >= nseq * H) return;
         b = pair / H;
@@ -370,17 +375,29 @@
     att16v3_inst<1, ATT_OUT_BF16>(),  att16v3_inst<2, ATT_OUT_BF16>(),  att16v3_inst<4, ATT_OUT_BF16>(),
 };
 
-int launch_att16v3(const AttLaunch& a, int wpb, dim3 grid, int dense_nblk) {
+static const Att16v3Inst kAtt16v3Sel[] = {
+    {1, ATT_OUT_F32, attention_f16x3_v3_kernel<1, ATT_OUT_F32, true>}, {1, ATT_OUT_SPLIT, attention_f16x3_v3_kernel<1, ATT_OUT_SPLIT, true>},
+    {1, ATT_OUT_BF16, attention_f16x3_v3_kernel<1, ATT_OUT_BF16, true>},
+};
+bool att_v3_sel_serves(const AttLaunch& a) { return a.q_sel && g_att_v3 != 0 && !a.conv && !a.slopes && a.head_dim == 64; }
+
+static int launch_att16v3_inst(const Att16v3Inst* first, const Att16v3Inst* last, const AttLaunch& a, int wpb, dim3 grid, int dense_nblk, const int32_t* q_sel) {
     constexpr size_t lds_bytes = (size_t)3 * (2 * AKT * 8 + 2 * 64 * 4) * 16;
-    for (const Att16v3Inst& k : kAtt16v3) {
-        if (k.wpb != wpb || k.out != a.out) continue;
-        hipLaunchKernelGGL(k.fn, grid, dim3(wpb * 64), lds_bytes, a.stream, a.qk16, a.qk_plane, a.vt16, a.vt_plane, a.kv_len, a.T, a.H, (a.T + 31) / 32 * 32,
-                           a.ctx, a.ctx16, dense_nblk, a.B);
+    for (const Att16v3Inst* k = first; k != last; ++k) {
+        if (k->wpb != wpb || k->out != a.out) continue;
+        hipLaunchKernelGGL(k->fn, grid, dim3(wpb * 64), lds_bytes, a.stream, a.qk16, a.qk_plane, a.vt16, a.vt_plane, a.kv_len, a.T, a.H, (a.T + 31) / 32 * 32,
+                           a.ctx, a.ctx16, dense_nblk, a.B, q_sel);
         PGMI_HIP(hipGetLastError());
         return PGMI_OK;
     }
     set_error("attention_f16x3_v3: no kernel for %d waves, output %d", wpb, (int)a.out);
     return PGMI_EINVAL;
 }
-
-}
+int launch_att16v3(const AttLaunch& a, int wpb, dim3 grid, int dense_nblk) {
+    return launch_att16v3_inst(std::begin(kAtt16v3), std::end(kAtt16v3), a, wpb, grid, dense_nblk, nullptr);
+}
+int launch_att16v3_sel(const AttLaunch& a) {
+    return launch_att16v3_inst(std::begin(kAtt16v3Sel), std::end(kAtt16v3Sel), a, 1, dim3(1, a.H, a.B), 0, a.q_sel);
+}
+
+}
diff --git a/proteingym_amd/csrc/common.h b/proteingym_amd/csrc/common.h
--- a/proteingym_amd/csrc/common.h
+++ b/proteingym_amd/csrc/common.h
@@ -34,6 +34,10 @@
 
 __host__ __device__ __forceinline__ size_t ki_off(size_t row, int k, int K) {
     return row * (size_t)(2 * K) + (size_t)(k >> 5) * 64 + (size_t)(k & 31);
+}
+__host__ __device__ __forceinline__ int vt_key_pos(int t) {
+    const int tk = t & 31;
+    return (t & ~31) + ((tk & 0x13) | ((tk & 4) << 1) | ((tk & 8) >> 1));
 }
 #if defined(__HIPCC__)
 __device__ __forceinline__ void split_act(float x, _Float16& hi, _Float16& lo) {
@@ -298,6 +302,21 @@
 int launch_qkln_prep(const float* qkv, const float* q_w, const float* k_w, float eps, const float* cos_t, const float* sin_t, int B,
                      int T, int H, unsigned short* qk16, size_t qk_plane, unsigned short* vt16, size_t vt_plane, hipStream_t s);
 
+struct ExpandLayer0 {
+    const unsigned short* pqk = nullptr;
+    size_t pqk_plane = 0;
+    const unsigned short* pvt = nullptr;
+    size_t pvt_plane = 0;
+    const int32_t* mask_rel = nullptr;
+    int B = 0, T = 0, H = 0;
+    unsigned short* qk16 = nullptr;
+    size_t qk_plane = 0;
+    unsigned short* vt16 = nullptr;
+    size_t vt_plane = 0;
+    hipStream_t stream = nullptr;
+};
+int launch_expand_layer0(const ExpandLayer0& e);
+
 struct GeomAttLaunch {
     const float* proj = nullptr;
     int pitch = 0;
@@ -331,6 +350,7 @@
     int B = 1, T = 0, H = 0;
     int head_dim = 64;
     const int32_t* kv_len = nullptr;
+    const int32_t* q_sel = nullptr;
     const float* slopes = nullptr;
     AttOut out = ATT_OUT_F32;
     float* ctx = nullptr;
diff --git a/proteingym_amd/csrc/gemm16x_kernel.h b/proteingym_amd/csrc/gemm16x_kernel.h
--- a/proteingym_amd/csrc/gemm16x_kernel.h
+++ b/proteingym_amd/csrc/gemm16x_kernel.h
@@ -386,8 +386,7 @@
                         lds_put(cell + 64, hi1);
                         lds_put(cell + 32 * SPQ + 64, lo1);
                     } else {
-                        const int tk = t & 31;
-                        const int pos = (t & ~31) + ((tk & 0x13) | ((tk & 4) << 1) | ((tk & 8) >> 1));
+                        const int pos = vt_key_pos(t);
                         unsigned short* col = qo.vt16 + (((size_t)bb * qo.H + hh) * kHeadDim + d0) * qo.Tp + pos;
 #pragma unroll
                         for (int e = 0; e < 4; ++e) {
diff --git a/proteingym_amd/csrc/layer0_plan.h b/proteingym_amd/csrc/layer0_plan.h
--- /dev/null
+++ b/proteingym_amd/csrc/layer0_plan.h
@@ -0,0 +1,24 @@
+#pragma once
+#include <stdint.h>
+
+#include <vector>
+
+namespace pgmi {
+
+inline bool layer0_plan(const int32_t* win_start, const int32_t* mask_rel, int bc, int T, int32_t* src) {
+    if (!win_start || !mask_rel || !src || bc < 2 || T < 2) return false;
+    for (int b = 0; b < bc; ++b)
+        if (win_start[b] != win_start[0] || mask_rel[b] < 0 || mask_rel[b] >= T) return false;
+    int other = 0;
+    for (int b = 1; b < bc && !other; ++b)
+        if (mask_rel[b] != mask_rel[0]) other = b;
+    std::vector<int32_t> first(T, -1);
+    for (int b = bc - 1; b >= 0; --b) first[mask_rel[b]] = b;
+    for (int t = 0; t < T; ++t) {
+        src[t] = (t == mask_rel[0] ? other : 0) * T + t;
+        src[T + t] = first[t] >= 0 ? first[t] * T + t : src[t];
+    }
+    return true;
+}
+
+}
diff --git a/proteingym_amd/csrc/model.h b/proteingym_amd/csrc/model.h
--- a/proteingym_amd/csrc/model.h
+++ b/proteingym_amd/csrc/model.h
@@ -13,6 +13,7 @@
 #include "common.h"
 #include "gemm16x_kernel.h"
 #include "packed_chunks.h"
+#include "layer0_plan.h"
 
 namespace pgmi {
 
@@ -126,6 +127,7 @@
     int32_t* nonfinite = nullptr;
     int gemm_variant = 0;
     int keep_rows = 1;
+    int share_layer0 = 1;
     int last_B = 0, last_T = 0;
     int dh = kHeadDim;
     int rot_halves = 1;
@@ -156,6 +158,10 @@
     int64_t* mut_off = nullptr;
     float* table = nullptr;
     double* scores = nullptr;
+    std::vector<int32_t> h_win_start, h_mask_rel;
+    int l0_per = 0;
+    int32_t* l0_src = nullptr;
+    std::vector<char> l0_ok;
 };
 
 struct pgmi_pppl {
@@ -243,10 +249,15 @@
 int create_esm(pgmi_model* m, const pgmi_config* cfg, const float* w, int64_t n_weights);
 int ensure_rotary(pgmi_model* m, int T);
 int upload_rotate_half(pgmi_model* m, int n);
-int run_encoder(pgmi_model* m, int B, int T, const int32_t* keep = nullptr, int n_keep = 0, bool* compacted = nullptr);
+struct MaskedCopies {
+    const int32_t* l0_src = nullptr;
+    const int32_t* mask_rel = nullptr;
+};
+int run_encoder(pgmi_model* m, int B, int T, const int32_t* keep = nullptr, int n_keep = 0, bool* compacted = nullptr,
+                const MaskedCopies* copies = nullptr);
 int head_hidden(pgmi_model* m, int R, const int32_t* row_idx);
 int run_head(pgmi_model* m, int R, const int32_t* row_idx);
-int run_rows(pgmi_model* m, int B, int T, int R, const int32_t* row_idx);
+int run_rows(pgmi_model* m, int B, int T, int R, const int32_t* row_idx, const MaskedCopies* copies = nullptr);
 int create_tranception(pgmi_model* m, const pgmi_config* cfg, const float* w, int64_t n_weights);
 int create_progen2(pgmi_model* m, const pgmi_config* cfg, const float* w, int64_t n_weights, int rotary_dim);
 int create_gpt(pgmi_model* m, const pgmi_config* cfg, const float* w, int64_t n_weights, int pos_kind);
```

Result: no change. 18690, median of 6 (+0.7%).
